# ritobanrc/firework

Measured on AMD Instinct MI355X. Metric: Mrays/s, cornell_box 512x512 @1024spp (scene resident in HBM; whole frame incl. tile gather), higher is better.
Workload: dtype f32; 1 GPU; C2_cornell_box 512x512 @1024spp; use_bvh=False, tiles=16x16, dealt diagonally over ranks, collective=none, rng=counter (pcg4d) keyed by (seed,pixel,sample,dimension), seed=0

## Files before the change

firework_amd/csrc/fw_device.h:

```cpp
#pragma once
#include <hip/hip_runtime.h>
#include <stdint.h>

#ifndef FW_AB
#define FW_AB 0
#endif

namespace fw {

constexpr int OBJ_Q = 6;

enum : uint32_t {
    OF_ROTATED = 1u << 0,
    OF_FLIP = 1u << 1,
    OF_RECT_FLIP = 1u << 2,
    OF_MESH_NORMALS = 1u << 3,
    OF_MESH_ATTR = 1u << 4,
    OF_CULL0 = 1u << 6,
    OF_GATE = 1u << 5,
};

constexpr uint32_t REF_LEAF = 0x80000000u, REF_DONE = 0xffffffffu;
constexpr int WIDE_NONE = 0, WIDE_F32 = 1, WIDE_Q8 = 2;
constexpr uint32_t WIDE_F32_DW = 28, WIDE_Q8_DW = 12;
// ... 22 lines not shown
    const uint32_t *tri_rank;
    const uint32_t *obj_rank;
    const float4 *obj_gate;
    const float4 *obj_cull;
    const float4 *obj_leaf;
    const float4 *mat;
    const float4 *tex;
    const uint8_t *images;
    uint32_t n_objects;
    uint32_t tlas_root;
    uint32_t has_medium;
    uint32_t has_perlin;
    uint32_t has_mesh;
    uint32_t prim_bits;
    const float4 *ref_tlas;
    const float4 *ref_blas;
    const uint32_t *obj_ref_blas;
    const uint32_t *wblas;
    const uint32_t *wtlas;
    const uint32_t *obj_wroot;
    uint32_t wtlas_root;
    float soft_shear;
    uint32_t n_hoisted;
    uint32_t hoisted[4];
    DEnv env;
};

constexpr uint32_t EX_TRACE_ZERO = 8u;
struct DExact {
    uint32_t mode;
    uint32_t n_frames;
    float frames[4][9];
    float shear;
    float far_c[3], far_r;
    float box_lo[3], box_hi[3];
    uint32_t *slots[2];
    uint32_t *count;
    uint32_t cap;
};

struct DCamera {
    float position[3], horizontal[3], vertical[3], lower_left[3], u[3], v[3];
    float lens_radius;
};

struct DFrame {
    uint32_t width, height;
    uint32_t n_pixels;
    const uint32_t *pixel_ids;
    uint32_t scatter_out;
    uint32_t seed32;
    uint32_t sample0;
    uint32_t spp_batch;
    float inv_width;
    float inv_n_pixels;
    uint32_t q_n_waves, q_shift;
    uint32_t skip_zero_deposits;
    uint32_t dep_pixel_major;
    uint32_t *dep_bits;
    uint32_t hit4;
    uint32_t pinhole0;
    float cam_pos[3];
    uint32_t chain_bits;
    float4 *atten;
    uint32_t atten_stride;
    DExact ex;
};

struct DPaths {
    float4 *ray_a;
    float2 *ray_b;
    float4 *state;
};

struct DQueue {
    uint32_t n_waves, cap;
    uint32_t cpw_shift;
    uint32_t *wcount;
};

struct DPark {
    float4 *ray_a; float2 *ray_b; float4 *meta;
    uint32_t stride;
    uint32_t *pcount;
    uint32_t *ptotal;
};

constexpr uint32_t B_RAY = 24, B_RAY_PINHOLE0 = 16, B_STATE = 16, B_STATE_CHAIN = 8, B_HIT = 8, B_HIT4 = 4, B_DEPOSIT = 16, B_PARK = 40, B_ACCUM = 16, B_ATTEN = 16;

constexpr uint32_t MISS = 0xffffffffu;
constexpr int MAX_SEGMENTS = 11;
constexpr int COUNT_STRIDE = 16;

struct DLights {
    const uint32_t *obj;
    uint32_t n;
    float p_pick;
};
struct DShadow {
    DLights lt;
    float4 *ray_a; float2 *ray_b;
    float4 *state;
    uint32_t *obj;
    uint32_t *wcount;
    const float *pb_in;
    float *pb_out;
    float4 *nee;
};
constexpr uint32_t SHADOW_SEED = 0x6e1a7c35u;

struct DEnvDist {
    const float *cdf_m, *cdf_c, *dens;
    float p_env;
    uint32_t w, h;
};

struct LaunchCfg {
    hipStream_t stream;
    DQueue q;
    int blocks_other;
    int tlas_depth, blas_depth;
    uint32_t n_mat, n_tex;
    bool lds_tables;
    bool has_mesh;
    bool simple_but_meshes;
    bool simple_set;
    int n_cus;
    uint32_t blas_pair_nodes, tlas_pair_nodes, max_tris, n_tris;
    bool no_lds_tris;
    uint32_t n_defer;
    bool lds_trees;
    int shade_mode;
    int exact_form;
    uint32_t ref_tlas_nodes, ref_blas_nodes, ref_tlas_depth, ref_blas_depth;
    int wblas_fmt, wtlas_fmt;
    uint32_t wblas_nodes, wtlas_nodes, wblas_depth, wtlas_depth;
    uint32_t debug_wide_levels;
    bool tlas_refill;
};
constexpr size_t LDS_TREE_LIMIT = 160 * 1024;
constexpr size_t LDS_TABLE_LIMIT = 16 * 1024;

void launch_raygen(const LaunchCfg &, const DCamera &, const DFrame &, DPaths out, float4 *sample_rad, uint32_t n_paths);
void launch_raygen_views(const LaunchCfg &, const DCamera *cams, uint32_t n_view, const DFrame &, DPaths out, float4 *sample_rad, uint32_t n_paths);
void launch_resolve_views(const LaunchCfg &, const DFrame &, uint32_t n_view, const float4 *accum, uint32_t total_spp, float gamma,
                          uint8_t *rgb8, float *gamma_rgb, float *linear_rgb);
void launch_view_ids(hipStream_t stream, const uint32_t *src, uint32_t n_view, uint32_t n, uint32_t *out);
void launch_raygen_rays(const LaunchCfg &, const float *rays, bool per_sample, uint32_t *err, const DFrame &, DPaths out, uint32_t n_paths);
void launch_ray_keys(hipStream_t stream, uint32_t base, uint32_t n, uint32_t *out);
void launch_extend(const LaunchCfg &, const DScene &, const DFrame &, DPaths in, float2 *hits, int segment, bool use_bvh, DPark park);
void launch_extend_exact(const LaunchCfg &, const DScene &, const DFrame &, const DPaths &in, float2 *hits, int segment, bool use_bvh);
void launch_shade(const LaunchCfg &, const DScene &, const DFrame &, DPaths in, DPaths out, const float2 *hits,
                  float4 *sample_rad, int segment);
void launch_shade_ls(const LaunchCfg &, const DScene &, const DFrame &, DPaths in, DPaths out, const float2 *hits,
                     float4 *sample_rad, int segment, const DShadow &);
void launch_shadow_resolve(const LaunchCfg &, const DScene &, const DShadow &, const float2 *hits, int segment);
void launch_shade_env(const LaunchCfg &, const DScene &, const DFrame &, DPaths in, DPaths out, const float2 *hits,
                      float4 *sample_rad, int segment, const DShadow &, const DEnvDist &);
void launch_shadow_resolve_env(const LaunchCfg &, const DScene &, const DShadow &, const float2 *hits, int segment);
int build_env_dist(hipStream_t stream, const DEnv &env, float *cdf_m, float *cdf_c, float *dens, float *p_out, double *scratch, double *total);
void launch_env_sample_test(hipStream_t stream, const DEnv &env, const DEnvDist &ed, uint32_t n, uint32_t seed32, float *out);
void launch_bounce(const LaunchCfg &, const DScene &, const DFrame &, DPaths in, DPaths out, float4 *sample_rad, int segment,
                   bool use_bvh);
void launch_queue_totals(const LaunchCfg &, uint32_t *totals, const uint32_t *ptotal);
void launch_trace_load(const LaunchCfg &, const DFrame &, const float *rays, DPaths out, uint32_t n, uint32_t key0, uint32_t *ids, uint32_t *slot_of);
void launch_trace_store(const LaunchCfg &, const DScene &, const DFrame &, const DPaths &in, const float2 *hits, const uint32_t *slot_of, uint32_t n,
                        float4 *out);
void launch_camera_rays(hipStream_t stream, int n_cus, const DCamera &, const DFrame &, uint32_t n, float *out);
void launch_aov_accumulate(hipStream_t stream, int n_cus, const DScene &, const DFrame &, const DPaths &in, const float2 *hits, const uint32_t *slot_of,
                           uint32_t n, uint32_t first, float4 *sum);
void launch_aov_finish(hipStream_t stream, int n_cus, uint32_t n, uint32_t spp, float4 *aov);
void launch_denoise(hipStream_t stream, int n_cus, uint32_t W, uint32_t H, uint32_t L, const float *color, const float4 *aov, const float4 *moments,
                    float4 *guide, float4 *ev0, float4 *ev1, float gamma, uint8_t *rgb8, float *gamma_rgb, float *linear_rgb);
void launch_scatter_tiles(hipStream_t stream, const uint32_t *ids, uint32_t n, const uint8_t *in8, const float *ing, const float *inl,
                          uint8_t *out8, float *outg, float *outl);
void launch_tile_order(hipStream_t stream, uint32_t width, uint32_t height, uint32_t *ids);
void launch_upload(hipStream_t stream, const void *pinned_src, void *dst, size_t bytes);
#if FW_AB
uint32_t take_error_word();
#endif
void preload_kernels();
void launch_count_deposits(const LaunchCfg &, const uint32_t *dep_bits, uint32_t *total);
void launch_selftest_arith(hipStream_t stream, uint32_t n, uint32_t seed, int mode, unsigned long long *out);
void launch_selftest_libm(hipStream_t stream, int fn, uint32_t n, const float *x, const float *y, float *out);
void launch_accumulate(const LaunchCfg &, const DFrame &, const float4 *sample_rad, float4 *accum);
void launch_resolve(const LaunchCfg &, const DFrame &, const float4 *accum, uint32_t total_spp, float gamma,
                    uint8_t *rgb8, float *gamma_rgb, float *linear_rgb);
constexpr uint32_t ADAPTIVE_MAX_BLOCKS = 1024;
void launch_accumulate_adaptive(const LaunchCfg &, const DFrame &, const float4 *sample_rad, float4 *accum, float4 *moments);
uint32_t adaptive_select_blocks(uint32_t n);
void launch_adaptive_select(hipStream_t stream, const uint32_t *ids, uint32_t n, const float4 *accum, float4 *moments, uint32_t n_samples, bool may_continue,
                            float tol, unsigned long long *mask, uint32_t *block_counts, uint32_t *out_ids, uint32_t *count);
void launch_resolve_adaptive(hipStream_t stream, int n_cus, uint32_t n, const float4 *accum, const float4 *moments, float gamma,
                             uint8_t *rgb8, float *gamma_rgb, float *linear_rgb);

constexpr int BLOCK = 256;

}
```

firework_amd/csrc/fw_kernels.hip:

```cpp
#include "../../include/firework_hip.h"
#include "fw_device.h"
#include "fw_libm.h"
#include <atomic>
#include <type_traits>

namespace fw {

struct V3 { float x, y, z; };
__device__ __forceinline__ V3 mk(float x, float y, float z) { return V3{x, y, z}; }
__device__ __forceinline__ V3 operator+(V3 a, V3 b) { return {a.x + b.x, a.y + b.y, a.z + b.z}; }
__device__ __forceinline__ V3 operator-(V3 a, V3 b) { return {a.x - b.x, a.y - b.y, a.z - b.z}; }
__device__ __forceinline__ V3 operator-(V3 a) { return {-a.x, -a.y, -a.z}; }
__device__ __forceinline__ V3 operator*(V3 a, V3 b) { return {a.x * b.x, a.y * b.y, a.z * b.z}; }
__device__ __forceinline__ V3 operator*(float s, V3 a) { return {s * a.x, s * a.y, s * a.z}; }
__device__ __forceinline__ V3 operator*(V3 a, float s) { return {a.x * s, a.y * s, a.z * s}; }
__device__ __forceinline__ float dot(V3 a, V3 b) { return fmaf(a.x, b.x, fmaf(a.y, b.y, a.z * b.z)); }
__device__ __forceinline__ V3 cross(V3 a, V3 b) {
    return {fmaf(a.y, b.z, -a.z * b.y), fmaf(a.z, b.x, -a.x * b.z), fmaf(a.x, b.y, -a.y * b.x)};
}
__device__ __forceinline__ float mag_sq(V3 a) { return dot(a, a); }
__device__ __forceinline__ float comp(V3 a, int i) { return i == 0 ? a.x : (i == 1 ? a.y : a.z); }
__device__ __forceinline__ V3 ld3(const float *p) { return {p[0], p[1], p[2]}; }

#ifndef FW_FAST_DIV
// ... 1189 lines not shown
                if (n_walk == 0u || (n_walk < n_busy && n_walk * WALK_NUM <= n_busy * WALK_DEN)) break;
                if (walking) {
                    TS_TICK(0);
                    cur = pair_step(sc.tlas, cur, wo, inv, relaxed(inv), box_tmin(TMIN, soft), TMAX, soft ? NO_CULL : cull_bound(have ? best_t : TMAX), st);
                }
            }
            if (busy && (cur & REF_LEAF) && cur != REF_DONE) {
                const uint32_t item = cur & NODE_MASK;
                cur = st.sp ? st.pop() : REF_DONE;
                Obj o = load_obj_for_hit(sc.obj, item);
                if (PARK && obj_kind(o) == 5u && !deferred) {
                    if (obj_gate_ok(sc, item, wo, inv)) { deferred = true; deferred_obj = item; }
                } else {
                    TS_TICK(2);
                    RngKey key{0, 0, 0};
                    if (sc.has_medium) key = key_of(f, path_id);
                    float t; uint32_t prim;
                    if (hit_object(sc, o, item, Ray{wo, wd}, TMIN, TMAX, blas_stack, key, segment, t, prim)) {
                        if ((!have || t < best_t || (t == best_t && sc.obj_rank[item] > sc.obj_rank[best_obj])) && obj_gate_ok(sc, item, wo, inv)) { have = true; best_t = t; best_obj = item; best_prim = prim; }
                    }
                }
            }

            const bool done = slot != IDLE && cur == REF_DONE;
            if (done && !deferred) qst(&hits[base + slot], pack_hit(best_t, best_obj, best_prim, sc.prim_bits));
            if (PARK) {
                const unsigned long long pmask = __ballot(done && deferred);
                if (pmask) {
                    const uint32_t prank = __builtin_amdgcn_mbcnt_hi((uint32_t)(pmask >> 32), __builtin_amdgcn_mbcnt_lo((uint32_t)pmask, 0u));
                    if (done && deferred) {
                        const uint32_t e = w * park.stride + park_n + prank;
                        qst(&park.ray_a[e], make_float4(wo.x, wo.y, wo.z, wd.x));
                        qst(&park.ray_b[e], make_float2(wd.y, wd.z));
                        qst(&park.meta[e], make_float4(__uint_as_float(base + slot), __uint_as_float(deferred_obj), best_t, pack_hit(best_t, best_obj, best_prim, sc.prim_bits).y));
                    }
                    park_n += (uint32_t)__popcll(pmask);
                }
            }
            if (done) slot = IDLE;
        }
        if (PARK && lane == 0) park.pcount[w] = park_n;
        TS_END();
        return;
    }

    float4 ra_n = make_float4(0, 0, 0, 0); float2 rb_n = make_float2(0, 0);
    if (lane < n) { ra_n = qld(&in.ray_a[base + lane]); rb_n = load_ray_b(in, base + lane, f, segment); }
    for (uint32_t c0 = 0; c0 < n; c0 += 64u) {
        const uint32_t j = c0 + lane;
        const uint32_t i = base + j;
        float4 ra = ra_n; float2 rb = rb_n;
        if (j + 64u < n) { ra_n = qld(&in.ray_a[i + 64u]); rb_n = load_ray_b(in, i + 64u, f, segment); }
        const bool active = j < n;
        bool deferred = false; uint32_t deferred_obj = 0;
        float best_t = TMAX; uint32_t best_obj = MISS, best_prim = 0;
        if (active) {
            Ray r = make_ray(ra, rb, f, segment);
            RngKey key{0, 0, 0};
            if (sc.has_medium) key = key_of(f, __float_as_uint(load_home(in, i, f, segment)));
            if (!skip_ray(f.ex, r))
                closest_hit<USE_BVH, USE_BVH, MESH, MEDIUM, SIMPLE>(sc, r, key, segment, my_stack, blas_stack, best_t, best_obj, best_prim, deferred, deferred_obj,
                                              USE_BVH && sc.has_mesh && soft_ray(f.ex, r.d, sc.soft_shear));
            if (!USE_BVH && f.hit4) reinterpret_cast<uint32_t *>(hits)[i] = __float_as_uint(pack_hit(best_t, best_obj, best_prim, sc.prim_bits).y);
            else if (!deferred) qst(&hits[i], pack_hit(best_t, best_obj, best_prim, sc.prim_bits));
        }
        if (USE_BVH && sc.has_mesh) {
            unsigned long long mask = __ballot(deferred);
            if (mask) {
                uint32_t rank = __builtin_amdgcn_mbcnt_hi((uint32_t)(mask >> 32), __builtin_amdgcn_mbcnt_lo((uint32_t)mask, 0u));
                if (deferred) {
                    uint32_t e = list_n + rank;
                    e_slot[e] = i; e_obj[e] = deferred_obj; e_t[e] = best_t; e_bobj[e] = best_obj; e_bprim[e] = best_prim;
                }
                list_n += (uint32_t)__popcll(mask);
                if (list_n >= BLAS_RUN_MIN) blas_run();
            }
        }
    }
    if (USE_BVH && list_n) blas_run();
    TS_END();
}
#ifndef FW_DEFER_WAVES
#define FW_DEFER_WAVES 7
#endif
#ifndef FW_DEFER_LDS_PAD
#define FW_DEFER_LDS_PAD 0
#endif
#ifndef FW_SCAN_WAVES
#define FW_SCAN_WAVES 6
#endif
#ifndef FW_SCAN_WAVES_PLAIN
#define FW_SCAN_WAVES_PLAIN 7
#endif
template <bool PARK, bool PLAIN = false, bool SIMPLE = false>
__global__ __launch_bounds__(WB) __attribute__((amdgpu_waves_per_eu(PLAIN ? FW_SCAN_WAVES_PLAIN : FW_SCAN_WAVES, 8))) void k_extend_scan(DScene sc, DFrame f, DPaths in, float2 *__restrict__ hits, DQueue q, int segment,
                                                    int tlas_levels, float4 *__restrict__ park_a, float2 *__restrict__ park_b, float4 *__restrict__ park_m,
                                                    uint32_t *__restrict__ park_count, uint32_t park_stride) {
    const uint32_t w = wave_index(), lane = threadIdx.x & 63u;
    if (w >= q.n_waves) return;
    const uint32_t n = q.wcount[(size_t)segment * q.n_waves + w];
    const uint32_t base = w * q.cap;
    uint32_t *blas_stack = lds_stack + threadIdx.x + (size_t)tlas_levels * WB;
    const float TMIN = 0.001f, TMAX = 2e9f;
    uint32_t park_n = 0;
    float4 ra_n = make_float4(0, 0, 0, 0); float2 rb_n = make_float2(0, 0);
    if (lane < n) { ra_n = qld(&in.ray_a[base + lane]); rb_n = load_ray_b(in, base + lane, f, segment); }
    for (uint32_t c0 = 0; c0 < n; c0 += 64u) {
        const uint32_t j = c0 + lane, i = base + j;
        const float4 ra = ra_n; const float2 rb = rb_n;
        if (j + 64u < n) { ra_n = qld(&in.ray_a[i + 64u]); rb_n = load_ray_b(in, i + 64u, f, segment); }
        const bool active = j < n;
        bool deferred = false, have = false; uint32_t deferred_obj = 0, best_obj = MISS, best_prim = 0; float best_t = TMAX;
        Ray r{mk(0, 0, 0), mk(0, 0, 1)};
        if (active) {
            r = make_ray(ra, rb, f, segment);
            RngKey key{0, 0, 0};
            if (sc.has_medium) key = key_of(f, __float_as_uint(load_home(in, i, f, segment)));
            const V3 inv = mk(fdiv(1.f, r.d.x), fdiv(1.f, r.d.y), fdiv(1.f, r.d.z));
            const bool soft = sc.has_mesh && soft_ray(f.ex, r.d, sc.soft_shear);
            const uint32_t n_obj = skip_ray(f.ex, r) ? 0u : sc.n_objects;
            for (uint32_t k = 0; k < n_obj; k++) {
                const float4 lo = sc.obj_leaf[2 * (size_t)k], hi = sc.obj_leaf[2 * (size_t)k + 1];
                float entry;
                if (!hit_aabb_entry(lo, hi, r.o, inv, relaxed(inv), box_tmin(TMIN, soft), TMAX, entry) || entry > (soft ? NO_CULL : cull_bound(have ? best_t : TMAX))) continue;
                Obj o = load_obj(sc.obj, k);
                if (PARK && obj_kind(o) == 5u) {
                    if (obj_gate_ok(sc, k, r.o, inv)) { deferred = true; deferred_obj |= 1u << k; }
                    continue;
                }
                float t; uint32_t prim;
                if (PLAIN ? hit_object<false, 0, false, SIMPLE>(sc, o, k, r, TMIN, TMAX, nullptr, key, segment, t, prim) : hit_object(sc, o, k, r, TMIN, TMAX, blas_stack, key, segment, t, prim)) {
                    if ((!have || t < best_t || (t == best_t && sc.obj_rank[k] > sc.obj_rank[best_obj])) && obj_gate_ok(sc, k, r.o, inv)) { have = true; best_t = t; best_obj = k; best_prim = prim; }
                }
            }
            if (!deferred) qst(&hits[i], pack_hit(best_t, best_obj, best_prim, sc.prim_bits));
        }
        if (PARK) {
            const unsigned long long pmask = __ballot(deferred);
            if (pmask) {
                const uint32_t prank = __builtin_amdgcn_mbcnt_hi((uint32_t)(pmask >> 32), __builtin_amdgcn_mbcnt_lo((uint32_t)pmask, 0u));
                if (deferred) {
                    const uint32_t e = w * park_stride + park_n + prank;
                    qst(&park_a[e], make_float4(r.o.x, r.o.y, r.o.z, r.d.x));
                    qst(&park_b[e], make_float2(r.d.y, r.d.z));
                    qst(&park_m[e], make_float4(__uint_as_float(i), __uint_as_float(PARK_MASK | deferred_obj), best_t, pack_hit(best_t, best_obj, best_prim, sc.prim_bits).y));
                }
                park_n += (uint32_t)__popcll(pmask);
            }
        }
    }
    if (PARK && lane == 0) park_count[w] = park_n;
}

constexpr uint32_t DEFER_FIELDS = 9;
extern __shared__ uint32_t lds_defer[];
template <bool SIMPLE>
__global__ __launch_bounds__(WB) __attribute__((amdgpu_waves_per_eu(FW_DEFER_WAVES, 8)))
void k_extend_linear_defer(DScene sc, DFrame f, DPaths in, float2 *__restrict__ hits, DQueue q, int segment, uint32_t n_def) {
    const uint32_t w = wave_index(), lane = threadIdx.x & 63u;
    if (w >= q.n_waves) return;
    const uint32_t n = q.wcount[(size_t)segment * q.n_waves + w], base = w * q.cap;
    const float TMIN = 0.001f, TMAX = 2e9f;
    const uint32_t n_first = sc.n_objects - n_def;
    uint32_t *const L0 = lds_defer, *const L1 = lds_defer + DEFER_FIELDS * 64u;
    uint32_t cnt0 = 0, cnt1 = 0;
    const RngKey nokey{0, 0, 0};
    auto write_final = [&](uint32_t slot, float t, uint32_t code) {
        if (f.hit4) reinterpret_cast<uint32_t *>(hits)[slot] = code; else qst(&hits[slot], make_float2(t, __uint_as_float(code)));
    };
    auto put = [&](uint32_t *L, uint32_t e, uint32_t sb, float t, uint32_t code, const Ray &r) {
        L[e] = sb; L[64u + e] = __float_as_uint(t); L[128u + e] = code;
        L[192u + e] = __float_as_uint(r.o.x); L[256u + e] = __float_as_uint(r.o.y); L[320u + e] = __float_as_uint(r.o.z);
        L[384u + e] = __float_as_uint(r.d.x); L[448u + e] = __float_as_uint(r.d.y); L[512u + e] = __float_as_uint(r.d.z);
    };
    auto get = [&](const uint32_t *L, uint32_t e, uint32_t &sb, float &t, uint32_t &code, Ray &r) {
        sb = L[e]; t = __uint_as_float(L[64u + e]); code = L[128u + e];
        r.o = mk(__uint_as_float(L[192u + e]), __uint_as_float(L[256u + e]), __uint_as_float(L[320u + e]));
        r.d = mk(__uint_as_float(L[384u + e]), __uint_as_float(L[448u + e]), __uint_as_float(L[512u + e]));
    };
    auto test = [&](uint32_t d, const Ray &r, float &t, uint32_t &code) {
        const uint32_t k = n_first + d;
        const Obj o = load_obj(sc.obj, k);
        float tt; uint32_t prim;
        if (hit_rect3d(o.q3, o.q4, to_object_space(o, r), TMIN, t, tt, prim)) { t = tt; code = (k << sc.prim_bits) | prim; }
    };
    auto append = [&](uint32_t *L, uint32_t &cnt, bool want, uint32_t sb, float t, uint32_t code, const Ray &r) {
        const unsigned long long m = __ballot(want);
        if (!m) return;
        const uint32_t rank = __builtin_amdgcn_mbcnt_hi((uint32_t)(m >> 32), __builtin_amdgcn_mbcnt_lo((uint32_t)m, 0u));
        if (want) put(L, cnt + rank, sb, t, code, r);
        cnt += (uint32_t)__popcll(m);
    };
    auto make_room = [&](uint32_t need0, uint32_t need1) {
        const bool r0 = cnt0 != 0u && cnt0 + need0 > 64u;
        const uint32_t pass_on = r0 ? (uint32_t)__popcll(__ballot(lane < cnt0 && (L0[lane] >> 31) != 0u)) : 0u;
#pragma nounroll
        for (int phase = 0; phase < 2; phase++) {
            const bool r1 = cnt1 != 0u && (phase == 0 ? cnt1 + pass_on > 64u : cnt1 + need1 > 64u);
            if (r1) {
                uint32_t sb = 0, code = MISS; float t = TMAX; Ray r{mk(0, 0, 0), mk(0, 0, 1)};
                if (lane < cnt1) { get(L1, lane, sb, t, code, r); test(1, r, t, code); write_final(sb, t, code); }
                cnt1 = 0;
            }
            if (phase == 0 && r0) {
                uint32_t sb = 0, code = MISS; float t = TMAX; Ray r{mk(0, 0, 0), mk(0, 0, 1)};
                const bool on = lane < cnt0;
                if (on) { get(L0, lane, sb, t, code, r); test(0, r, t, code); }
                cnt0 = 0;
                const bool more = on && (sb >> 31) != 0u;
                const uint32_t slot = sb & 0x7fffffffu;
                if (on && !more) write_final(slot, t, code);
                append(L1, cnt1, more, slot, t, code, r);
            }
        }
    };
    float4 ra_n = make_float4(0, 0, 0, 0); float2 rb_n = make_float2(0, 0);
    if (lane < n) { ra_n = qld(&in.ray_a[base + lane]); rb_n = load_ray_b(in, base + lane, f, segment); }
    for (uint32_t c0 = 0; c0 < n; c0 += 64u) {
        const uint32_t j = c0 + lane, i = base + j;
        const float4 ra = ra_n; const float2 rb = rb_n;
        if (j + 64u < n) { ra_n = qld(&in.ray_a[i + 64u]); rb_n = load_ray_b(in, i + 64u, f, segment); }
        const bool active = j < n;
        float best_t = TMAX; uint32_t best_obj = MISS, best_prim = 0;
        bool may0 = false, may1 = false;
        const Ray r = make_ray(ra, rb, f, segment);
        if (active) {
            const float4 *op = sc.obj;
            const Rcp rcx = make_rcp(r.d.x), rcy = make_rcp(r.d.y), rcz = make_rcp(r.d.z);
            for (uint32_t k = 0; k < n_first; k++, op += OBJ_Q) {
                const Obj o = load_obj(op, 0);
                float t; uint32_t prim = 0; bool h;
                const uint32_t kind = obj_kind(o);
                if (kind >= 1u && kind <= 3u && !(obj_flags(o) & OF_ROTATED) && o.q4.y == 0.f) {
                    const Ray ro{r.o - mk(o.q0.w, o.q1.w, o.q2.w), r.d};
                    if (kind == 1u) h = hit_rect_rcp<0>(o.q3.x, o.q3.y, o.q3.z, o.q3.w, o.q4.x, ro, rcz, TMIN, best_t, t);
                    else if (kind == 2u) h = hit_rect_rcp<1>(o.q3.x, o.q3.y, o.q3.z, o.q3.w, o.q4.x, ro, rcy, TMIN, best_t, t);
                    else h = hit_rect_rcp<2>(o.q3.x, o.q3.y, o.q3.z, o.q3.w, o.q4.x, ro, rcx, TMIN, best_t, t);
                } else h = hit_object<false, 0, false, SIMPLE>(sc, o, k, r, TMIN, best_t, nullptr, nokey, segment, t, prim);
                if (h) { best_t = t; best_obj = k; best_prim = prim; }
            }
            const V3 ainv = mk(__builtin_amdgcn_rcpf(r.d.x), __builtin_amdgcn_rcpf(r.d.y), __builtin_amdgcn_rcpf(r.d.z));
            const float eps = 1e-4f * (fabsf(r.o.x) + fabsf(r.o.y) + fabsf(r.o.z));
            for (uint32_t d = 0; d < n_def; d++) {
                const uint32_t k = n_first + d;
                const float4 lo = sc.obj_cull[2 * (size_t)k], hi = sc.obj_cull[2 * (size_t)k + 1];
                const float m = eps + 1e-4f * (fmaxf(fmaxf(fabsf(lo.x), fabsf(lo.y)), fabsf(lo.z)) + fmaxf(fmaxf(fabsf(hi.x), fabsf(hi.y)), fabsf(hi.z))) + 1e-6f;
                float t0 = (lo.x - m - r.o.x) * ainv.x, t1 = (hi.x + m - r.o.x) * ainv.x;
                float tn = fminf(t0, t1), tf = fmaxf(t0, t1);
                t0 = (lo.y - m - r.o.y) * ainv.y; t1 = (hi.y + m - r.o.y) * ainv.y;
                tn = fmaxf(tn, fminf(t0, t1)); tf = fminf(tf, fmaxf(t0, t1));
                t0 = (lo.z - m - r.o.z) * ainv.z; t1 = (hi.z + m - r.o.z) * ainv.z;
                tn = fmaxf(tn, fminf(t0, t1)); tf = fminf(tf, fmaxf(t0, t1));
                const bool maybe = !(tf < tn * (1.f - 1e-4f) - 1e-4f) && !(tf < 0.f) && !(tn * (1.f - 1e-4f) - 1e-4f > best_t);
                if (d == 0) may0 = maybe; else may1 = maybe;
            }
        }
        const uint32_t code = best_obj == MISS ? MISS : ((best_obj << sc.prim_bits) | best_prim);
        const bool c1 = may1 && !may0;
        make_room((uint32_t)__popcll(__ballot(may0)), (uint32_t)__popcll(__ballot(c1)));
        if (active && !may0 && !may1) write_final(i, best_t, code);
        append(L0, cnt0, may0, i | (may1 ? 0x80000000u : 0u), best_t, code, r);
        append(L1, cnt1, c1, i, best_t, code, r);
    }
    make_room(65u, 65u);
}

__global__ __launch_bounds__(WB) __attribute__((amdgpu_waves_per_eu(7, 8)))
void k_extend_linear(DScene sc, DFrame f, DPaths in, float2 *__restrict__ hits, DQueue q, int segment, int tlas_levels, int stack_levels) {
    extend_body<false, false, false>(sc, f, in, hits, q, segment, tlas_levels, stack_levels, DPark{});
}
__global__ __launch_bounds__(WB) __attribute__((amdgpu_waves_per_eu(7, 8)))
void k_extend_linear_nomesh(DScene sc, DFrame f, DPaths in, float2 *__restrict__ hits, DQueue q, int segment, int tlas_levels, int stack_levels) {
    extend_body<false, false, false, false>(sc, f, in, hits, q, segment, tlas_levels, stack_levels, DPark{});
}
__global__ __launch_bounds__(WB) __attribute__((amdgpu_waves_per_eu(7, 8)))
void k_extend_linear_plain(DScene sc, DFrame f, DPaths in, float2 *__restrict__ hits, DQueue q, int segment, int tlas_levels, int stack_levels) {
    extend_body<false, false, false, false, false>(sc, f, in, hits, q, segment, tlas_levels, stack_levels, DPark{});
}
template <bool MEDIUM>
__global__ __launch_bounds__(WB) __attribute__((amdgpu_waves_per_eu(7, 8)))
void k_extend_linear_simple(DScene sc, DFrame f, DPaths in, float2 *__restrict__ hits, DQueue q, int segment, int tlas_levels, int stack_levels) {
    extend_body<false, false, false, false, MEDIUM, true>(sc, f, in, hits, q, segment, tlas_levels, stack_levels, DPark{});
}
#if FW_AB
__global__ __launch_bounds__(WB) __attribute__((amdgpu_waves_per_eu(5, 8)))
void k_extend_bvh(DScene sc, DFrame f, DPaths in, float2 *__restrict__ hits, DQueue q, int segment, int tlas_levels, int stack_levels) {
    extend_body<true, false, false>(sc, f, in, hits, q, segment, tlas_levels, stack_levels, DPark{});
}
#endif
__global__ __launch_bounds__(WB) __attribute__((amdgpu_waves_per_eu(FW_TLAS_WAVES, 8)))
void k_extend_tlas(DScene sc, DFrame f, DPaths in, float2 *__restrict__ hits, DQueue q, int segment, int tlas_levels, int stack_levels) {
    extend_body<true, true, false>(sc, f, in, hits, q, segment, tlas_levels, stack_levels, DPark{});
}
__global__ __launch_bounds__(WB) __attribute__((amdgpu_waves_per_eu(FW_TLAS_WAVES, 8)))
void k_extend_tlas_park(DScene sc, DFrame f, DPaths in, float2 *__restrict__ hits, DQueue q, int segment, int tlas_levels, int stack_levels, DPark park) {
    extend_body<true, true, true>(sc, f, in, hits, q, segment, tlas_levels, stack_levels, park);
}

__global__ __launch_bounds__(WB) __attribute__((amdgpu_waves_per_eu(FW_BLAS_WAVES, 8)))
void k_blas(DScene sc, DPark park, float2 *__restrict__ hits, DQueue q) {
    const uint32_t w = wave_index(), lane = threadIdx.x & 63u;
    if (w >= q.n_waves) return;
    TS_BEGIN();
    const uint32_t n = park.pcount[w];
    if (lane == 0 && n) park.ptotal[w] += n;
    const uint32_t base = w * park.stride;
    const float TMIN = 0.001f, TMAX = 2e9f;
    float4 ca = make_float4(0, 0, 0, 0), na = ca, cm = ca, nm = ca; float2 cb = make_float2(0, 0), nb = cb;
    auto fetch = [&](uint32_t j, float4 &a, float2 &b, float4 &m) {
        if (j < n) { a = qld(&park.ray_a[base + j]); b = qld(&park.ray_b[base + j]); m = qld(&park.meta[base + j]); }
    };
    fetch(lane, ca, cb, cm); fetch(64u + lane, na, nb, nm);
    uint32_t cur_base = 0, q_next = 0;
    bool act = false, have = false;
    uint32_t slot = 0, obj = 0, tri_base = 0, bcode = MISS, mtri = 0, cur = REF_DONE;
    float bt = TMAX, mbest = TMAX;
    V3 ro = mk(0, 0, 0), inv = ro;
    bool soft = false;
    TriRay tr{mk(0, 0, 0), 0, 1, 2, 0.f, 0.f, 0.f};
    LdsStack st{lds_stack + threadIdx.x, 0};
    uint32_t more = 0, pidx = 0;
    auto start_walk = [&](uint32_t mesh_obj, float4 ra, float2 rb) {
        obj = mesh_obj;
        Obj o = load_obj(sc.obj, obj);
        Ray r = to_object_space(o, Ray{mk(ra.x, ra.y, ra.z), mk(ra.w, rb.x, rb.y)});
        ro = r.o; inv = mk(fdiv(1.f, r.d.x), fdiv(1.f, r.d.y), fdiv(1.f, r.d.z));
        soft = soft_direction(r.d.x, r.d.y, r.d.z, sc.soft_shear);
        tr = make_triray(r);
        tri_base = o.aux1; cur = o.aux0; st.sp = 0;
        have = false; mbest = TMAX; mtri = 0; act = true;
    };
    for (;;) {
        const unsigned long long idle_mask = __ballot(!act);
        const uint32_t n_idle = (uint32_t)__popcll(idle_mask);
        if (q_next < n) {
            if (n_idle >= BLAS_REFILL_MIN) {
                const uint32_t take = min(n_idle, min(n, cur_base + 64u) - q_next);
                const uint32_t rank = __builtin_amdgcn_mbcnt_hi((uint32_t)(idle_mask >> 32), __builtin_amdgcn_mbcnt_lo((uint32_t)idle_mask, 0u));
                const int sel = (int)((((q_next - cur_base) + rank) & 63u) << 2);
                auto bp = [&](float v) { return __int_as_float(__builtin_amdgcn_ds_bpermute(sel, __float_as_int(v))); };
                const float4 ra = make_float4(bp(ca.x), bp(ca.y), bp(ca.z), bp(ca.w));
                const float2 rb = make_float2(bp(cb.x), bp(cb.y));
                const float4 me = make_float4(bp(cm.x), bp(cm.y), bp(cm.z), bp(cm.w));
                if (!act && rank < take) {
                    slot = __float_as_uint(me.x); more = __float_as_uint(me.y); bt = me.z; bcode = __float_as_uint(me.w);
                    pidx = base + q_next + rank;
                    start_walk(park_next_mesh(more), ra, rb);
                }
                q_next += take;
                if (q_next == cur_base + 64u && q_next < n) { ca = na; cb = nb; cm = nm; cur_base += 64u; fetch(cur_base + 64u + lane, na, nb, nm); }
            }
        } else if (n_idle == 64u) break;

        const uint32_t n_act = (uint32_t)__popcll(__ballot(act));
        for (;;) {
            const bool walking = act && !(cur & REF_LEAF);
            const uint32_t n_walk = (uint32_t)__popcll(__ballot(walking));
            if (n_walk == 0u || (n_walk < n_act && n_walk * BLAS_WALK_NUM <= n_act * BLAS_WALK_DEN)) break;
            if (walking) {
                TS_TICK(4);
                cur = pair_step(sc.blas, cur, ro, inv, relaxed(inv), box_tmin(TMIN, soft), TMAX, soft ? NO_CULL : cull_bound(have ? fminf(mbest, bt) : bt), st);
            }
        }
        if (act && (cur & REF_LEAF)) {
            if (cur != REF_DONE) {
                const uint32_t item = cur & NODE_MASK;
                cur = st.sp ? st.pop() : REF_DONE;
                TS_TICK(6);
                const float4 *tp = sc.tri + 3 * (size_t)(tri_base + item);
                float4 a = tp[0], b = tp[1], c = tp[2];
                float t, b0, b1, b2;
                if (hit_triangle(mk(a.x, a.y, a.z), mk(b.x, b.y, b.z), mk(c.x, c.y, c.z), tr, TMIN, TMAX, t, b0, b1, b2)) {
                    if ((!have || t < mbest || (t == mbest && sc.tri_rank[tri_base + item] > sc.tri_rank[tri_base + mtri])) &&
                        tri_gate_ok(sc, tri_base + item, mk(a.x, a.y, a.z), mk(b.x, b.y, b.z), mk(c.x, c.y, c.z), ro, inv, TMIN, TMAX)) { have = true; mbest = t; mtri = item; }
                }
            }
            if (cur == REF_DONE) {
                const uint32_t bobj = bcode == MISS ? MISS : (bcode >> sc.prim_bits);
                if (have && (bobj == MISS || mbest < bt || (mbest == bt && sc.obj_rank[obj] > sc.obj_rank[bobj]))) { bt = mbest; bcode = (obj << sc.prim_bits) | mtri; }
                if (more) start_walk(park_next_mesh(more), qld(&park.ray_a[pidx]), qld(&park.ray_b[pidx]));
                else { qst(&hits[slot], make_float2(bt, __uint_as_float(bcode))); act = false; }
            }
        }
    }
    TS_END();
}

constexpr int LDS_WAVES = 16;
constexpr uint32_t LDS_UNIT = 512;
__host__ __device__ inline uint32_t lds_unit(uint32_t queue_slots) { const uint32_t u = (queue_slots / 4u) & ~63u; return u < 128u ? 128u : (u > LDS_UNIT ? LDS_UNIT : u); }
template <bool LDS_TRIS>
__global__ __launch_bounds__(LDS_WAVES * 64) void k_blas_lds(DScene sc, DPark park, float2 *__restrict__ hits, DQueue q,
                                                             uint32_t n_nodes, uint32_t n_tris, uint32_t levels) {
    extern __shared__ float4 lds_nodes[];
    const uint32_t lane = threadIdx.x & 63u, wib = threadIdx.x >> 6;
    for (uint32_t k = threadIdx.x; k < n_nodes * 4u; k += LDS_WAVES * 64) lds_nodes[k] = sc.blas[k];
    float4 *lds_tris = lds_nodes + (size_t)n_nodes * 4u;
    if (LDS_TRIS) for (uint32_t k = threadIdx.x; k < n_tris * 3u; k += LDS_WAVES * 64) lds_tris[k] = sc.tri[k];
    uint16_t *stacks = reinterpret_cast<uint16_t *>(lds_tris + (LDS_TRIS ? (size_t)n_tris * 3u : 0u));
    uint32_t *ctr = reinterpret_cast<uint32_t *>(stacks + (size_t)LDS_WAVES * levels * 64u);
    const uint32_t n_k = (q.n_waves + gridDim.x - 1u - blockIdx.x) / gridDim.x;
    uint32_t *lds_cnt = ctr + 4;
    for (uint32_t k = threadIdx.x; k < n_k; k += LDS_WAVES * 64) lds_cnt[k] = park.pcount[blockIdx.x + k * gridDim.x];
    if (threadIdx.x == 0) *ctr = 0u;
    __syncthreads();
    BlockStream bs;
// ... 1141 lines not shown
        if (f.skip_zero_deposits) {
            const uint32_t b = f.dep_pixel_major ? dep_bit_of(f, path_id) : path_id;
            atomicOr(&f.dep_bits[b >> 5], 1u << (b & 31u));
        }
        PH_ADD(6);
    }
    return alive;
}

extern __shared__ float4 lds_tables[];

template <int LDS_TAB, int MODE, bool CHAIN>
#ifndef FW_SHADE_WAVES
#define FW_SHADE_WAVES 5
#endif
#ifndef FW_SHADE_PIPE
#define FW_SHADE_PIPE 0
#endif
#ifndef FW_SHADE_STATIC_STORES
#define FW_SHADE_STATIC_STORES FW_SHADE_PIPE
#endif
__attribute__((amdgpu_waves_per_eu(FW_SHADE_WAVES, 8)))
__global__ __launch_bounds__(WB) void k_shade(DScene sc, DFrame f, DPaths in, DPaths out, const float2 *__restrict__ hits,
                                                 float4 *__restrict__ sample_rad, DQueue q, int segment,
                                                 uint32_t n_mat, uint32_t n_tex) {
    const uint32_t w = wave_index(), lane = threadIdx.x & 63u;
    const float4 *objp = sc.obj, *matp = sc.mat, *texp = sc.tex;
    __shared__ uint16_t shade_list[128];
    if (sc.has_perlin && MODE != 1 && !CHAIN) { stage_perm(); if (!LDS_TAB) __syncthreads(); }
    if (LDS_TAB) {
        const uint32_t no = LDS_TAB == 1 ? sc.n_objects * OBJ_Q : 0u, nm = 2 * n_mat, nt = 2 * n_tex;
        if (LDS_TAB == 1) for (uint32_t k = threadIdx.x; k < no; k += WB) lds_tables[k] = sc.obj[k];
        for (uint32_t k = threadIdx.x; k < nm; k += WB) lds_tables[no + k] = sc.mat[k];
        for (uint32_t k = threadIdx.x; k < nt; k += WB) lds_tables[no + nm + k] = sc.tex[k];
        __syncthreads();
        if (LDS_TAB == 1) objp = lds_tables;
        matp = lds_tables + no; texp = lds_tables + no + nm;
    }
    if (w >= q.n_waves) return;
    const uint32_t n = q.wcount[(size_t)segment * q.n_waves + w];
    const uint32_t base = w * q.cap;
    uint32_t out_n = 0;
    uint32_t list_n = 0;
    PH_DECL;
    auto compact = [&](bool alive, const Ray &nr, V3 nbeta, uint32_t nchain, uint32_t path_id, uint32_t c0 = 0xffffffffu) {
        const unsigned long long mask = __ballot(alive);
        const uint32_t rank = __builtin_amdgcn_mbcnt_hi((uint32_t)(mask >> 32), __builtin_amdgcn_mbcnt_lo((uint32_t)mask, 0u));
#if FW_SHADE_STATIC_STORES
        if (c0 != 0xffffffffu) {
#if FW_SHADE_STATIC_STORES == 2
            const uint32_t dst = base + (alive ? out_n + rank : q.cap - 1u);
#else
            const uint32_t dst = base + (alive ? out_n + rank : min(c0 + 64u + lane, q.cap - 1u));
#endif
            qst(&out.ray_a[dst], make_float4(nr.o.x, nr.o.y, nr.o.z, nr.d.x));
            qst(&out.ray_b[dst], make_float2(nr.d.y, nr.d.z));
            if (CHAIN) qst(&reinterpret_cast<float2 *>(out.state)[dst], make_float2(__uint_as_float(nchain), __uint_as_float(path_id)));
            else qst(&out.state[dst], make_float4(nbeta.x, nbeta.y, nbeta.z, __uint_as_float(path_id)));
        } else
#endif
        if (alive) {
            const uint32_t dst = base + out_n + rank;
            qst(&out.ray_a[dst], make_float4(nr.o.x, nr.o.y, nr.o.z, nr.d.x));
            qst(&out.ray_b[dst], make_float2(nr.d.y, nr.d.z));
            if (CHAIN) qst(&reinterpret_cast<float2 *>(out.state)[dst], make_float2(__uint_as_float(nchain), __uint_as_float(path_id)));
            else qst(&out.state[dst], make_float4(nbeta.x, nbeta.y, nbeta.z, __uint_as_float(path_id)));
        }
        if (f.ex.mode)
            flag_exact(f.ex, alive && needs_exact(f.ex, nr.o.x, nr.o.y, nr.o.z, nr.d.x, nr.d.y, nr.d.z), base + out_n + rank, segment + 1);
        out_n += (uint32_t)__popcll(mask);
    };
    auto load_st = [&](uint32_t idx) { return CHAIN ? load_state_chain(in, idx, segment) : load_state(in, idx, segment); };
    auto load_hit = [&](uint32_t idx) { return f.hit4 ? make_float2(0.f, __uint_as_float(reinterpret_cast<const uint32_t *>(hits)[idx])) : qld(&hits[idx]); };
    auto run_list = [&](uint32_t take) {
        bool alive = false;
        Ray nr{mk(0, 0, 0), mk(0, 0, 0)}; V3 nbeta = mk(0, 0, 0); uint32_t path_id = 0, nchain = 0;
        if (lane < take) {
            const uint32_t i = base + shade_list[list_n - take + lane];
            const float4 ra = qld(&in.ray_a[i]), st = load_st(i); const float2 rb = load_ray_b(in, i, f, segment), hr = load_hit(i);
            path_id = __float_as_uint(st.w);
            alive = shade_path<false, CHAIN>(sc, f, objp, matp, texp, make_ray(ra, rb, f, segment), mk(st.x, st.y, st.z), __float_as_uint(st.x), path_id, hr.x, __float_as_uint(hr.y), segment, sample_rad, nr, nbeta, nchain PH_PASS);
        }
        list_n -= take;
        compact(alive, nr, nbeta, nchain, path_id);
    };
    float4 ra_n = make_float4(0, 0, 0, 0), st_n = ra_n; float2 rb_n = make_float2(0, 0), hr_n = rb_n;
#if FW_SHADE_PIPE
    auto prefetch = [&](uint32_t jn) {
        const uint32_t in_ = base + jn;
        ra_n = qld(&in.ray_a[in_]);
        rb_n = qld(&in.ray_b[short_rays(f, segment) ? base : in_]);
        if (CHAIN) { const float2 v = qld(&reinterpret_cast<const float2 *>(in.state)[segment == 0 ? base : in_]); st_n = make_float4(v.x, 0.f, 0.f, v.y); }
        else st_n = qld(&in.state[segment == 0 ? base : in_]);
        hr_n = load_hit(in_);
    };
    auto fix_implicit = [&](float4 &st_, float2 &rb_, uint32_t slot) {
        if (segment == 0) st_ = CHAIN ? make_float4(0.f, 0.f, 0.f, __uint_as_float(slot)) : make_float4(1.f, 1.f, 1.f, __uint_as_float(slot));
        if (short_rays(f, segment)) rb_ = make_float2(0.f, 0.f);
    };
    if (n) {
        prefetch(min(lane, n - 1u));
        const uint32_t d0 = base + lane;
        qst(&out.ray_a[d0], make_float4(0.f, 0.f, 0.f, 0.f));
        qst(&out.ray_b[d0], make_float2(0.f, 0.f));
        if (CHAIN) qst(&reinterpret_cast<float2 *>(out.state)[d0], make_float2(0.f, 0.f)); else qst(&out.state[d0], make_float4(0.f, 0.f, 0.f, 0.f));
    }
#else
    if (lane < n) { ra_n = qld(&in.ray_a[base + lane]); rb_n = load_ray_b(in, base + lane, f, segment); st_n = load_st(base + lane); hr_n = load_hit(base + lane); }
#endif
    for (uint32_t c0 = 0; c0 < n; c0 += 64u) {
        const uint32_t j = c0 + lane;
        const uint32_t i = base + j;
        float4 ra = ra_n, st = st_n; float2 rb = rb_n, hr = hr_n;
#if FW_SHADE_PIPE
        fix_implicit(st, rb, i);
        const RngKey key_ = key_of(f, __float_as_uint(st.w));
        prefetch(min(j + 64u, n - 1u));
        const RngKey *pre_key = &key_;
#else
        if (j + 64u < n) { ra_n = qld(&in.ray_a[i + 64u]); rb_n = load_ray_b(in, i + 64u, f, segment); st_n = load_st(i + 64u); hr_n = load_hit(i + 64u); }
        const RngKey *pre_key = nullptr;
#endif
        bool alive = false, later = false;
        Ray nr{mk(0, 0, 0), mk(0, 0, 0)}; V3 nbeta = mk(0, 0, 0); uint32_t path_id = 0, nchain = 0;
        if (j < n) {
            PH_T0;
            Ray r = make_ray(ra, rb, f, segment);
            V3 beta = mk(st.x, st.y, st.z);
            path_id = __float_as_uint(st.w);
            const uint32_t hit_code = __float_as_uint(hr.y);
#ifdef FW_ABL_SHADE_COPY
            alive = hit_code != MISS && segment < 10; nr = r; nbeta = beta; nchain = __float_as_uint(st.x) + (pre_key ? pre_key->pixel & 1u : 0u);
#else
            if (MODE == 2 && expensive_shading(sc, objp, matp, hit_code)) later = true;
            else alive = shade_path<MODE != 0, CHAIN>(sc, f, objp, matp, texp, r, beta, __float_as_uint(st.x), path_id, hr.x, hit_code, segment, sample_rad, nr, nbeta, nchain PH_PASS, pre_key);
#endif
            PH_ADD(0);
        }
        { PH_T0; compact(alive, nr, nbeta, nchain, path_id, c0); PH_ADD(7); }
        if (MODE == 2) {
            const unsigned long long lm = __ballot(later);
            if (lm) {
                const uint32_t lr = __builtin_amdgcn_mbcnt_hi((uint32_t)(lm >> 32), __builtin_amdgcn_mbcnt_lo((uint32_t)lm, 0u));
                if (later) shade_list[list_n + lr] = (uint16_t)j;
                list_n += (uint32_t)__popcll(lm);
                if (list_n >= 64u) run_list(64u);
            }
        }
    }
    if (MODE == 2) while (list_n) run_list(min(list_n, 64u));
    if (lane == 0) q.wcount[(size_t)(segment + 1) * q.n_waves + w] = out_n;
    PH_FLUSH(1);
}
template <int LDS_TAB, int MODE>
__attribute__((amdgpu_waves_per_eu(FW_SHADE_WAVES, 8)))
__global__ __launch_bounds__(WB) void k_shade_ls(DScene sc, DFrame f, DPaths in, DPaths out, const float2 *__restrict__ hits,
                                                    float4 *__restrict__ sample_rad, DQueue q, int segment,
                                                    uint32_t n_mat, uint32_t n_tex, DShadow sh) {
    static_assert(MODE == 0 || MODE == 1, "in line only");
    const uint32_t w = wave_index(), lane = threadIdx.x & 63u;
    const float4 *objp = sc.obj, *matp = sc.mat, *texp = sc.tex;
    if (sc.has_perlin && MODE != 1) { stage_perm(); if (!LDS_TAB) __syncthreads(); }
    if (LDS_TAB) {
        const uint32_t no = LDS_TAB == 1 ? sc.n_objects * OBJ_Q : 0u, nm = 2 * n_mat, nt = 2 * n_tex;
        if (LDS_TAB == 1) for (uint32_t k = threadIdx.x; k < no; k += WB) lds_tables[k] = sc.obj[k];
        for (uint32_t k = threadIdx.x; k < nm; k += WB) lds_tables[no + k] = sc.mat[k];
        for (uint32_t k = threadIdx.x; k < nt; k += WB) lds_tables[no + nm + k] = sc.tex[k];
        __syncthreads();
        if (LDS_TAB == 1) objp = lds_tables;
        matp = lds_tables + no; texp = lds_tables + no + nm;
    }
    if (w >= q.n_waves) return;
    const uint32_t n = q.wcount[(size_t)segment * q.n_waves + w];
    const uint32_t base = w * q.cap;
    uint32_t out_n = 0, sh_n = 0;
    PH_DECL;
    float4 ra_n = make_float4(0, 0, 0, 0), st_n = ra_n; float2 rb_n = make_float2(0, 0), hr_n = rb_n; float pb_n = 0.f;
    auto fetch = [&](uint32_t i) {
        ra_n = qld(&in.ray_a[i]); rb_n = load_ray_b(in, i, f, segment); st_n = load_state(in, i, segment); hr_n = qld(&hits[i]);
        pb_n = segment > 0 ? sh.pb_in[i] : 0.f;
    };
    if (lane < n) fetch(base + lane);
    for (uint32_t c0 = 0; c0 < n; c0 += 64u) {
        const uint32_t j = c0 + lane, i = base + j;
        float4 ra = ra_n, st = st_n; float2 rb = rb_n, hr = hr_n;
        LsIO ls{pb_n, 0.f, false, Ray{mk(0, 0, 0), mk(0, 0, 0)}, 0u, mk(0, 0, 0)};
        if (j + 64u < n) fetch(i + 64u);
        bool alive = false;
        Ray nr{mk(0, 0, 0), mk(0, 0, 0)}; V3 nbeta = mk(0, 0, 0); uint32_t path_id = 0, nchain = 0;
        if (j < n) {
            path_id = __float_as_uint(st.w);
            alive = shade_path<MODE != 0, false, true>(sc, f, objp, matp, texp, make_ray(ra, rb, f, segment), mk(st.x, st.y, st.z), 0u, path_id, hr.x,
                                                       __float_as_uint(hr.y), segment, sample_rad, nr, nbeta, nchain PH_PASS, nullptr, &sh, &ls);
        }
        const unsigned long long mask = __ballot(alive);
        const uint32_t rank = __builtin_amdgcn_mbcnt_hi((uint32_t)(mask >> 32), __builtin_amdgcn_mbcnt_lo((uint32_t)mask, 0u));
        if (alive) {
            const uint32_t dst = base + out_n + rank;
            qst(&out.ray_a[dst], make_float4(nr.o.x, nr.o.y, nr.o.z, nr.d.x));
            qst(&out.ray_b[dst], make_float2(nr.d.y, nr.d.z));
            qst(&out.state[dst], make_float4(nbeta.x, nbeta.y, nbeta.z, __uint_as_float(path_id)));
            sh.pb_out[dst] = ls.pb_out;
        }
        if (f.ex.mode) flag_exact(f.ex, alive && needs_exact(f.ex, nr.o.x, nr.o.y, nr.o.z, nr.d.x, nr.d.y, nr.d.z), base + out_n + rank, segment + 1);
        out_n += (uint32_t)__popcll(mask);
        const unsigned long long sm = __ballot(ls.shadow);
        if (sm) {
            const uint32_t sr = __builtin_amdgcn_mbcnt_hi((uint32_t)(sm >> 32), __builtin_amdgcn_mbcnt_lo((uint32_t)sm, 0u));
            if (ls.shadow) {
                const uint32_t d = base + sh_n + sr;
                sh.ray_a[d] = make_float4(ls.sray.o.x, ls.sray.o.y, ls.sray.o.z, ls.sray.d.x);
                sh.ray_b[d] = make_float2(ls.sray.d.y, ls.sray.d.z);
                sh.state[d] = make_float4(ls.pending.x, ls.pending.y, ls.pending.z, __uint_as_float(path_id));
                sh.obj[d] = ls.sobj;
            }
            sh_n += (uint32_t)__popcll(sm);
        }
    }
    if (lane == 0) { q.wcount[(size_t)(segment + 1) * q.n_waves + w] = out_n; sh.wcount[(size_t)(segment + 1) * q.n_waves + w] = sh_n; }
}
template <int LDS_TAB>
__attribute__((amdgpu_waves_per_eu(FW_SHADE_WAVES, 8)))
__global__ __launch_bounds__(WB) void k_shade_env(DScene sc, DFrame f, DPaths in, DPaths out, const float2 *__restrict__ hits,
                                                     float4 *__restrict__ sample_rad, DQueue q, int segment,
                                                     uint32_t n_mat, uint32_t n_tex, DShadow sh, DEnvDist ed) {
    const uint32_t w = wave_index(), lane = threadIdx.x & 63u;
    const float4 *objp = sc.obj, *matp = sc.mat, *texp = sc.tex;
    if (sc.has_perlin) { stage_perm(); if (!LDS_TAB) __syncthreads(); }
    if (LDS_TAB) {
        const uint32_t no = LDS_TAB == 1 ? sc.n_objects * OBJ_Q : 0u, nm = 2 * n_mat, nt = 2 * n_tex;
        if (LDS_TAB == 1) for (uint32_t k = threadIdx.x; k < no; k += WB) lds_tables[k] = sc.obj[k];
        for (uint32_t k = threadIdx.x; k < nm; k += WB) lds_tables[no + k] = sc.mat[k];
        for (uint32_t k = threadIdx.x; k < nt; k += WB) lds_tables[no + nm + k] = sc.tex[k];
        __syncthreads();
        if (LDS_TAB == 1) objp = lds_tables;
        matp = lds_tables + no; texp = lds_tables + no + nm;
    }
    if (w >= q.n_waves) return;
    const uint32_t n = q.wcount[(size_t)segment * q.n_waves + w];
    const uint32_t base = w * q.cap;
    uint32_t out_n = 0, sh_n = 0;
    PH_DECL;
    float4 ra_n = make_float4(0, 0, 0, 0), st_n = ra_n; float2 rb_n = make_float2(0, 0), hr_n = rb_n; float pb_n = 0.f;
    auto fetch = [&](uint32_t i) {
        ra_n = qld(&in.ray_a[i]); rb_n = load_ray_b(in, i, f, segment); st_n = load_state(in, i, segment); hr_n = qld(&hits[i]);
        pb_n = segment > 0 ? sh.pb_in[i] : 0.f;
    };
    if (lane < n) fetch(base + lane);
    for (uint32_t c0 = 0; c0 < n; c0 += 64u) {
        const uint32_t j = c0 + lane, i = base + j;
        float4 ra = ra_n, st = st_n; float2 rb = rb_n, hr = hr_n;
        LsIO ls{pb_n, 0.f, false, Ray{mk(0, 0, 0), mk(0, 0, 0)}, 0u, mk(0, 0, 0)};
        if (j + 64u < n) fetch(i + 64u);
        bool alive = false;
        Ray nr{mk(0, 0, 0), mk(0, 0, 0)}; V3 nbeta = mk(0, 0, 0); uint32_t path_id = 0, nchain = 0;
        if (j < n) {
            path_id = __float_as_uint(st.w);
            alive = shade_path<false, false, true, true>(sc, f, objp, matp, texp, make_ray(ra, rb, f, segment), mk(st.x, st.y, st.z), 0u, path_id, hr.x,
                                                            __float_as_uint(hr.y), segment, sample_rad, nr, nbeta, nchain PH_PASS, nullptr, &sh, &ls, &ed);
        }
        const unsigned long long mask = __ballot(alive);
        const uint32_t rank = __builtin_amdgcn_mbcnt_hi((uint32_t)(mask >> 32), __builtin_amdgcn_mbcnt_lo((uint32_t)mask, 0u));
        if (alive) {
            const uint32_t dst = base + out_n + rank;
            qst(&out.ray_a[dst], make_float4(nr.o.x, nr.o.y, nr.o.z, nr.d.x));
            qst(&out.ray_b[dst], make_float2(nr.d.y, nr.d.z));
            qst(&out.state[dst], make_float4(nbeta.x, nbeta.y, nbeta.z, __uint_as_float(path_id)));
            sh.pb_out[dst] = ls.pb_out;
        }
        if (f.ex.mode) flag_exact(f.ex, alive && needs_exact(f.ex, nr.o.x, nr.o.y, nr.o.z, nr.d.x, nr.d.y, nr.d.z), base + out_n + rank, segment + 1);
        out_n += (uint32_t)__popcll(mask);
        const unsigned long long sm = __ballot(ls.shadow);
        if (sm) {
            const uint32_t sr = __builtin_amdgcn_mbcnt_hi((uint32_t)(sm >> 32), __builtin_amdgcn_mbcnt_lo((uint32_t)sm, 0u));
            if (ls.shadow) {
                const uint32_t d = base + sh_n + sr;
                sh.ray_a[d] = make_float4(ls.sray.o.x, ls.sray.o.y, ls.sray.o.z, ls.sray.d.x);
                sh.ray_b[d] = make_float2(ls.sray.d.y, ls.sray.d.z);
                sh.state[d] = make_float4(ls.pending.x, ls.pending.y, ls.pending.z, __uint_as_float(path_id));
                sh.obj[d] = ls.sobj;
            }
            sh_n += (uint32_t)__popcll(sm);
        }
    }
    if (lane == 0) { q.wcount[(size_t)(segment + 1) * q.n_waves + w] = out_n; sh.wcount[(size_t)(segment + 1) * q.n_waves + w] = sh_n; }
}
__global__ __launch_bounds__(WB) void k_shadow_resolve(DShadow sh, const float2 *__restrict__ hits, DQueue q, int segment, uint32_t prim_bits) {
    const uint32_t w = wave_index(), lane = threadIdx.x & 63u;
    if (w >= q.n_waves) return;
    const uint32_t n = sh.wcount[(size_t)(segment + 1) * q.n_waves + w], base = w * q.cap;
    for (uint32_t j = lane; j < n; j += 64u) {
        const uint32_t i = base + j, code = __float_as_uint(hits[i].y);
        if (code == MISS || (code >> prim_bits) != sh.obj[i]) continue;
        const float4 p = sh.state[i];
        float4 &e = sh.nee[__float_as_uint(p.w)];
        e = make_float4(e.x + p.x, e.y + p.y, e.z + p.z, 0.f);
    }
}
__global__ __launch_bounds__(WB) void k_shadow_resolve_env(DShadow sh, const float2 *__restrict__ hits, DQueue q, int segment, uint32_t prim_bits) {
    const uint32_t w = wave_index(), lane = threadIdx.x & 63u;
    if (w >= q.n_waves) return;
    const uint32_t n = sh.wcount[(size_t)(segment + 1) * q.n_waves + w], base = w * q.cap;
    for (uint32_t j = lane; j < n; j += 64u) {
        const uint32_t i = base + j, code = __float_as_uint(hits[i].y);
        if ((code == MISS ? MISS : code >> prim_bits) != sh.obj[i]) continue;
        const float4 p = sh.state[i];
// ... 522 lines not shown
void launch_trace_store(const LaunchCfg &c, const DScene &sc, const DFrame &f, const DPaths &in, const float2 *hits, const uint32_t *slot_of, uint32_t n,
                        float4 *out) {
    const uint32_t blocks = (uint32_t)std::max<uint64_t>(1, std::min<uint64_t>(((uint64_t)n + BLOCK - 1) / BLOCK, (uint64_t)c.n_cus * 32u));
    hipLaunchKernelGGL(k_trace_store, dim3(blocks), dim3(BLOCK), 0, c.stream, sc, f, in, hits, slot_of, n, out);
}
void launch_camera_rays(hipStream_t stream, int n_cus, const DCamera &cam, const DFrame &f, uint32_t n, float *out) {
    const uint32_t blocks = (uint32_t)std::max<uint64_t>(1, std::min<uint64_t>(((uint64_t)n + 63u) / 64u, (uint64_t)n_cus * 64u));
    hipLaunchKernelGGL(k_camera_rays, dim3(blocks), dim3(WB), 0, stream, cam, f, n, out);
}

void launch_raygen(const LaunchCfg &c, const DCamera &cam, const DFrame &f, DPaths out, float4 *sample_rad, uint32_t n_paths) {
    hipLaunchKernelGGL(k_raygen, wave_grid(c), dim3(WB), 0, c.stream, cam, f, out, sample_rad, c.q, n_paths);
}
void launch_raygen_views(const LaunchCfg &c, const DCamera *cams, uint32_t n_view, const DFrame &f, DPaths out, float4 *sample_rad, uint32_t n_paths) {
    hipLaunchKernelGGL(k_raygen_views, wave_grid(c), dim3(WB), 0, c.stream, cams, n_view, f, out, sample_rad, c.q, n_paths);
}
void launch_raygen_rays(const LaunchCfg &c, const float *rays, bool per_sample, uint32_t *err, const DFrame &f, DPaths out, uint32_t n_paths) {
    hipLaunchKernelGGL(k_raygen_rays, wave_grid(c), dim3(WB), 0, c.stream, rays, per_sample ? 1u : 0u, err, f, out, c.q, n_paths);
}
void launch_ray_keys(hipStream_t stream, uint32_t base, uint32_t n, uint32_t *out) {
    hipLaunchKernelGGL(k_ray_keys, dim3(std::min<uint32_t>((n + BLOCK - 1) / BLOCK, 4096u)), dim3(BLOCK), 0, stream, base, n, out);
}
void launch_resolve_views(const LaunchCfg &c, const DFrame &f, uint32_t n_view, const float4 *accum, uint32_t total_spp, float gamma,
                          uint8_t *rgb8, float *gamma_rgb, float *linear_rgb) {
    hipLaunchKernelGGL(k_resolve_views, dim3(c.blocks_other), dim3(BLOCK), 0, c.stream, f, n_view, accum, total_spp, gamma, rgb8, gamma_rgb, linear_rgb);
}
void launch_view_ids(hipStream_t stream, const uint32_t *src, uint32_t n_view, uint32_t n, uint32_t *out) {
    hipLaunchKernelGGL(k_view_ids, dim3(std::min<uint32_t>((n + BLOCK - 1) / BLOCK, 4096u)), dim3(BLOCK), 0, stream, src, n_view, n, out);
}
static bool lds_attr_needed(int which) {
    static std::atomic<unsigned char> done[4][64];
    int dev = 0;
    if (hipGetDevice(&dev) != hipSuccess || dev < 0 || dev >= 64) return true;
    return done[which][dev].exchange(1) == 0;
}
static size_t lds_walk_bytes(size_t tree_bytes, uint32_t waves, uint32_t levels, uint32_t n_queues, uint32_t grid) {
    return tree_bytes + (size_t)waves * levels * 64 * 2 + 16 + 4 * (size_t)((n_queues + grid - 1) / grid);
}
void launch_extend(const LaunchCfg &c, const DScene &sc, const DFrame &f, DPaths in, float2 *hits, int segment, bool use_bvh, DPark park) {
    int tl = use_bvh ? c.tlas_depth + 1 : 0;
    int levels = tl + c.blas_depth + 1;
    size_t lds = (size_t)levels * WB * sizeof(uint32_t) + (use_bvh && c.has_mesh ? 5 * DEFER_CAP * sizeof(uint32_t) : 0);
    dim3 eg = wave_grid(c);
    const dim3 sg = eg;
    auto walk_grid = [&](uint32_t waves) { return std::min<uint32_t>((uint32_t)c.n_cus, (c.q.n_waves + waves - 1) / waves); };
    if (use_bvh && c.tlas_refill && c.has_mesh) {
        if (sc.n_objects <= TLAS_SCAN_MAX && !sc.has_medium && c.simple_but_meshes) hipLaunchKernelGGL((k_extend_scan<true, true, true>), eg, dim3(WB), (size_t)levels * WB * sizeof(uint32_t), c.stream, sc, f, in, hits, c.q, segment, tl, park.ray_a, park.ray_b, park.meta, park.pcount, park.stride);
        else if (sc.n_objects <= TLAS_SCAN_MAX && !sc.has_medium) hipLaunchKernelGGL((k_extend_scan<true, true>), eg, dim3(WB), (size_t)levels * WB * sizeof(uint32_t), c.stream, sc, f, in, hits, c.q, segment, tl, park.ray_a, park.ray_b, park.meta, park.pcount, park.stride);
        else if (sc.n_objects <= TLAS_SCAN_MAX) hipLaunchKernelGGL(k_extend_scan<true>, eg, dim3(WB), (size_t)levels * WB * sizeof(uint32_t), c.stream, sc, f, in, hits, c.q, segment, tl, park.ray_a, park.ray_b, park.meta, park.pcount, park.stride);
        else hipLaunchKernelGGL(k_extend_tlas_park, sg, dim3(WB), (size_t)levels * WB * sizeof(uint32_t), c.stream, sc, f, in, hits, c.q, segment, tl, levels, park);
        if (c.lds_trees && c.wblas_fmt != WIDE_NONE && sc.wblas && c.max_tris < 0x7fffu) {
            const uint32_t wl = c.debug_wide_levels ? c.debug_wide_levels : 3u * c.wblas_depth + 2u;
            const size_t tree = (size_t)c.wblas_nodes * (c.wblas_fmt == WIDE_F32 ? WIDE_F32_DW : WIDE_Q8_DW) * 4, tris = (size_t)c.n_tris * 48;
            uint32_t waves = 0; bool lds_tris = false;
            if (!c.no_lds_tris && lds_walk_bytes(tree + tris, 16, wl, c.q.n_waves, walk_grid(16)) <= LDS_TREE_LIMIT) { waves = 16; lds_tris = true; }
            else for (uint32_t w : {16u, 12u, 8u}) if (lds_walk_bytes(tree, w, wl, c.q.n_waves, walk_grid(w)) <= LDS_TREE_LIMIT) { waves = w; break; }
            if (waves) {
                if (lds_attr_needed(2)) {
                    (void)hipFuncSetAttribute(reinterpret_cast<const void *>(k_blas_wide<WIDE_F32, false>), hipFuncAttributeMaxDynamicSharedMemorySize, (int)LDS_TREE_LIMIT);
                    (void)hipFuncSetAttribute(reinterpret_cast<const void *>(k_blas_wide<WIDE_F32, true>), hipFuncAttributeMaxDynamicSharedMemorySize, (int)LDS_TREE_LIMIT);
                    (void)hipFuncSetAttribute(reinterpret_cast<const void *>(k_blas_wide<WIDE_Q8, false>), hipFuncAttributeMaxDynamicSharedMemorySize, (int)LDS_TREE_LIMIT);
                    (void)hipFuncSetAttribute(reinterpret_cast<const void *>(k_blas_wide<WIDE_Q8, true>), hipFuncAttributeMaxDynamicSharedMemorySize, (int)LDS_TREE_LIMIT);
                }
                const dim3 lg(walk_grid(waves));
                const size_t bytes = lds_walk_bytes(tree + (lds_tris ? tris : 0), waves, wl, c.q.n_waves, lg.x);
#define FW_BLAS_WIDE(F, T) hipLaunchKernelGGL((k_blas_wide<F, T>), lg, dim3(waves * 64), bytes, c.stream, sc, park, hits, c.q, c.wblas_nodes, c.n_tris, wl)
                if (c.wblas_fmt == WIDE_F32) { if (lds_tris) FW_BLAS_WIDE(WIDE_F32, true); else FW_BLAS_WIDE(WIDE_F32, false); }
                else { if (lds_tris) FW_BLAS_WIDE(WIDE_Q8, true); else FW_BLAS_WIDE(WIDE_Q8, false); }
#undef FW_BLAS_WIDE
                return;
            }
        }
        const uint32_t bl = (uint32_t)c.blas_depth + 1u;
        const size_t lds_blas = lds_walk_bytes((size_t)c.blas_pair_nodes * 64, LDS_WAVES, bl, c.q.n_waves, walk_grid(LDS_WAVES)), lds_tris = (size_t)c.n_tris * 48;
        if (c.lds_trees && c.blas_pair_nodes > 0 && c.blas_pair_nodes < 32768u && c.max_tris < 32768u && lds_blas <= LDS_TREE_LIMIT) {
            if (lds_attr_needed(0)) {
                (void)hipFuncSetAttribute(reinterpret_cast<const void *>(k_blas_lds<false>), hipFuncAttributeMaxDynamicSharedMemorySize, (int)LDS_TREE_LIMIT);
                (void)hipFuncSetAttribute(reinterpret_cast<const void *>(k_blas_lds<true>), hipFuncAttributeMaxDynamicSharedMemorySize, (int)LDS_TREE_LIMIT);
            }
            const dim3 lg(walk_grid(LDS_WAVES));
            if (lds_blas + lds_tris <= LDS_TREE_LIMIT && !c.no_lds_tris)
                hipLaunchKernelGGL(k_blas_lds<true>, lg, dim3(LDS_WAVES * 64), lds_blas + lds_tris, c.stream, sc, park, hits, c.q, c.blas_pair_nodes, c.n_tris, bl);
            else
                hipLaunchKernelGGL(k_blas_lds<false>, lg, dim3(LDS_WAVES * 64), lds_blas, c.stream, sc, park, hits, c.q, c.blas_pair_nodes, c.n_tris, bl);
        }
        else hipLaunchKernelGGL(k_blas, sg, dim3(WB), (size_t)(c.blas_depth + 1) * WB * sizeof(uint32_t), c.stream, sc, park, hits, c.q);
    }
    else if (use_bvh && c.tlas_refill) {
        if (c.lds_trees && !c.has_mesh && sc.n_objects > TLAS_SCAN_MAX && c.wtlas_fmt == WIDE_F32 && sc.wtlas && sc.n_objects < 0x7fffu) {
            const uint32_t wl = c.debug_wide_levels ? c.debug_wide_levels : 3u * c.wtlas_depth + 2u;
            const size_t tree = (size_t)c.wtlas_nodes * WIDE_F32_DW * 4;
            uint32_t waves = 0;
            for (uint32_t w : {16u, 12u, 8u}) if (lds_walk_bytes(tree, w, wl, c.q.n_waves, walk_grid(w)) <= LDS_TREE_LIMIT) { waves = w; break; }
            if (waves) {
                if (lds_attr_needed(3)) {
                    (void)hipFuncSetAttribute(reinterpret_cast<const void *>(k_extend_tlas_wide<true>), hipFuncAttributeMaxDynamicSharedMemorySize, (int)LDS_TREE_LIMIT);
                    (void)hipFuncSetAttribute(reinterpret_cast<const void *>(k_extend_tlas_wide<false>), hipFuncAttributeMaxDynamicSharedMemorySize, (int)LDS_TREE_LIMIT);
                    (void)hipFuncSetAttribute(reinterpret_cast<const void *>((k_extend_tlas_wide<true, true>)), hipFuncAttributeMaxDynamicSharedMemorySize, (int)LDS_TREE_LIMIT);
                    (void)hipFuncSetAttribute(reinterpret_cast<const void *>((k_extend_tlas_wide<false, true>)), hipFuncAttributeMaxDynamicSharedMemorySize, (int)LDS_TREE_LIMIT);
                }
                const dim3 lg(walk_grid(waves));
                if (!sc.has_medium && c.simple_set) hipLaunchKernelGGL((k_extend_tlas_wide<false, true>), lg, dim3(waves * 64), lds_walk_bytes(tree, waves, wl, c.q.n_waves, lg.x), c.stream, sc, f, in, hits, c.q, segment, c.wtlas_nodes, wl);
                else if (sc.has_medium && c.simple_set) hipLaunchKernelGGL((k_extend_tlas_wide<true, true>), lg, dim3(waves * 64), lds_walk_bytes(tree, waves, wl, c.q.n_waves, lg.x), c.stream, sc, f, in, hits, c.q, segment, c.wtlas_nodes, wl);
                else if (sc.has_medium) hipLaunchKernelGGL(k_extend_tlas_wide<true>, lg, dim3(waves * 64), lds_walk_bytes(tree, waves, wl, c.q.n_waves, lg.x), c.stream, sc, f, in, hits, c.q, segment, c.wtlas_nodes, wl);
                else hipLaunchKernelGGL(k_extend_tlas_wide<false>, lg, dim3(waves * 64), lds_walk_bytes(tree, waves, wl, c.q.n_waves, lg.x), c.stream, sc, f, in, hits, c.q, segment, c.wtlas_nodes, wl);
                return;
            }
        }
        const size_t lds_tlas = lds_walk_bytes((size_t)c.tlas_pair_nodes * 64, LDS_WAVES, (uint32_t)tl, c.q.n_waves, walk_grid(LDS_WAVES));
        if (c.lds_trees && !c.has_mesh && sc.n_objects > TLAS_SCAN_MAX && c.tlas_pair_nodes < 32768u && sc.n_objects < 32768u && lds_tlas <= LDS_TREE_LIMIT) {
            if (lds_attr_needed(1)) (void)hipFuncSetAttribute(reinterpret_cast<const void *>(k_extend_tlas_lds), hipFuncAttributeMaxDynamicSharedMemorySize, (int)LDS_TREE_LIMIT);
            hipLaunchKernelGGL(k_extend_tlas_lds, dim3(walk_grid(LDS_WAVES)), dim3(LDS_WAVES * 64), lds_tlas, c.stream,
                               sc, f, in, hits, c.q, segment, c.tlas_pair_nodes, (uint32_t)tl);
        }
        else if (sc.n_objects <= TLAS_SCAN_MAX) hipLaunchKernelGGL(k_extend_scan<false>, eg, dim3(WB), lds, c.stream, sc, f, in, hits, c.q, segment, tl, (float4 *)nullptr, (float2 *)nullptr, (float4 *)nullptr, (uint32_t *)nullptr, 0u);
        else hipLaunchKernelGGL(k_extend_tlas, sg, dim3(WB), lds, c.stream, sc, f, in, hits, c.q, segment, tl, levels);
    }
#if FW_AB
    else if (use_bvh) hipLaunchKernelGGL(k_extend_bvh, eg, dim3(WB), lds, c.stream, sc, f, in, hits, c.q, segment, tl, levels);
#endif
    else if (c.n_defer && c.simple_set) hipLaunchKernelGGL(k_extend_linear_defer<true>, eg, dim3(WB), (size_t)2 * 64 * DEFER_FIELDS * 4 + FW_DEFER_LDS_PAD, c.stream, sc, f, in, hits, c.q, segment, c.n_defer);
    else if (c.n_defer) hipLaunchKernelGGL(k_extend_linear_defer<false>, eg, dim3(WB), (size_t)2 * 64 * DEFER_FIELDS * 4 + FW_DEFER_LDS_PAD, c.stream, sc, f, in, hits, c.q, segment, c.n_defer);
    else if (c.simple_set && !sc.has_medium) hipLaunchKernelGGL(k_extend_linear_simple<false>, eg, dim3(WB), lds, c.stream, sc, f, in, hits, c.q, segment, tl, levels);
    else if (c.simple_set) hipLaunchKernelGGL(k_extend_linear_simple<true>, eg, dim3(WB), lds, c.stream, sc, f, in, hits, c.q, segment, tl, levels);
    else if (!c.has_mesh && !sc.has_medium) hipLaunchKernelGGL(k_extend_linear_plain, eg, dim3(WB), lds, c.stream, sc, f, in, hits, c.q, segment, tl, levels);
    else if (!c.has_mesh) hipLaunchKernelGGL(k_extend_linear_nomesh, eg, dim3(WB), lds, c.stream, sc, f, in, hits, c.q, segment, tl, levels);
    else hipLaunchKernelGGL(k_extend_linear, eg, dim3(WB), lds, c.stream, sc, f, in, hits, c.q, segment, tl, levels);
}
void launch_extend_exact(const LaunchCfg &c, const DScene &sc, const DFrame &f, const DPaths &in, float2 *hits, int segment, bool use_bvh) {
    const uint32_t tl = std::max<uint32_t>(std::min<uint32_t>(c.ref_tlas_depth + 2u, EXACT_LEVELS), (EXACT_STACK + 2u * EXACT_DEFER) / EXACT_WB);
    const uint32_t bl = std::max<uint32_t>(std::min<uint32_t>(c.ref_blas_depth + 2u, EXACT_LEVELS), EXACT_STACK / EXACT_WB);
    const size_t lds = (size_t)(tl + bl) * EXACT_WB * 4;
    hipLaunchKernelGGL(k_extend_exact, dim3((uint32_t)c.n_cus * 8u), dim3(EXACT_WB), lds, c.stream, sc, f, in, hits, segment, use_bvh ? 1 : 0, tl, c.exact_form);
}
void launch_shade(const LaunchCfg &c, const DScene &sc, const DFrame &f, DPaths in, DPaths out, const float2 *hits,
                  float4 *sample_rad, int segment) {
    size_t tab = ((size_t)sc.n_objects * OBJ_Q + 2 * (size_t)c.n_mat + 2 * (size_t)c.n_tex) * sizeof(float4);
    const size_t tab_mt = (2 * (size_t)c.n_mat + 2 * (size_t)c.n_tex) * sizeof(float4);
    const int lt = (c.lds_tables && tab <= LDS_TABLE_LIMIT) ? 1 : ((c.lds_tables && tab_mt <= LDS_TABLE_LIMIT) ? 2 : 0);
    const size_t lds = lt == 1 ? tab : (lt == 2 ? tab_mt : 0);
    const int mode = c.shade_mode;
#define FW_SHADE(L, M, C) hipLaunchKernelGGL((k_shade<L, M, C>), wave_grid(c), dim3(WB), lds, c.stream, sc, f, in, out, hits, sample_rad, c.q, segment, c.n_mat, c.n_tex)
#define FW_SHADE_C(L, M) do { if (f.chain_bits) FW_SHADE(L, M, true); else FW_SHADE(L, M, false); } while (0)
#if FW_AB
#define FW_SHADE_L(L) do { if (mode == 2) FW_SHADE(L, 2, false); else if (mode == 1) FW_SHADE_C(L, 1); else FW_SHADE_C(L, 0); } while (0)
#else
#define FW_SHADE_L(L) do { if (mode == 1) FW_SHADE_C(L, 1); else FW_SHADE_C(L, 0); } while (0)
#endif
    if (lt == 1) FW_SHADE_L(1); else if (lt == 2) FW_SHADE_L(2); else FW_SHADE_L(0);
#undef FW_SHADE_L
#undef FW_SHADE_C
#undef FW_SHADE
}
void launch_shade_ls(const LaunchCfg &c, const DScene &sc, const DFrame &f, DPaths in, DPaths out, const float2 *hits,
                     float4 *sample_rad, int segment, const DShadow &sh) {
    const size_t tab = ((size_t)sc.n_objects * OBJ_Q + 2 * (size_t)c.n_mat + 2 * (size_t)c.n_tex) * sizeof(float4);
    const size_t tab_mt = (2 * (size_t)c.n_mat + 2 * (size_t)c.n_tex) * sizeof(float4);
    const int lt = (c.lds_tables && tab <= LDS_TABLE_LIMIT) ? 1 : ((c.lds_tables && tab_mt <= LDS_TABLE_LIMIT) ? 2 : 0);
    const size_t lds = lt == 1 ? tab : (lt == 2 ? tab_mt : 0);
#define FW_SHADE_LS(L, M) hipLaunchKernelGGL((k_shade_ls<L, M>), wave_grid(c), dim3(WB), lds, c.stream, sc, f, in, out, hits, sample_rad, c.q, segment, c.n_mat, c.n_tex, sh)
#define FW_SHADE_LS_M(L) do { if (c.shade_mode == 1) FW_SHADE_LS(L, 1); else FW_SHADE_LS(L, 0); } while (0)
    if (lt == 1) FW_SHADE_LS_M(1); else if (lt == 2) FW_SHADE_LS_M(2); else FW_SHADE_LS_M(0);
#undef FW_SHADE_LS_M
#undef FW_SHADE_LS
}
void launch_shadow_resolve(const LaunchCfg &c, const DScene &sc, const DShadow &sh, const float2 *hits, int segment) {
    hipLaunchKernelGGL(k_shadow_resolve, wave_grid(c), dim3(WB), 0, c.stream, sh, hits, c.q, segment, sc.prim_bits);
}
void launch_shade_env(const LaunchCfg &c, const DScene &sc, const DFrame &f, DPaths in, DPaths out, const float2 *hits,
                      float4 *sample_rad, int segment, const DShadow &sh, const DEnvDist &ed) {
    const size_t tab = ((size_t)sc.n_objects * OBJ_Q + 2 * (size_t)c.n_mat + 2 * (size_t)c.n_tex) * sizeof(float4);
    const size_t tab_mt = (2 * (size_t)c.n_mat + 2 * (size_t)c.n_tex) * sizeof(float4);
    const int lt = (c.lds_tables && tab <= LDS_TABLE_LIMIT) ? 1 : ((c.lds_tables && tab_mt <= LDS_TABLE_LIMIT) ? 2 : 0);
    const size_t lds = lt == 1 ? tab : (lt == 2 ? tab_mt : 0);
#define FW_SHADE_ENV(L) hipLaunchKernelGGL((k_shade_env<L>), wave_grid(c), dim3(WB), lds, c.stream, sc, f, in, out, hits, sample_rad, c.q, segment, c.n_mat, c.n_tex, sh, ed)
    if (lt == 1) FW_SHADE_ENV(1); else if (lt == 2) FW_SHADE_ENV(2); else FW_SHADE_ENV(0);
#undef FW_SHADE_ENV
}
void launch_shadow_resolve_env(const LaunchCfg &c, const DScene &sc, const DShadow &sh, const float2 *hits, int segment) {
    hipLaunchKernelGGL(k_shadow_resolve_env, wave_grid(c), dim3(WB), 0, c.stream, sh, hits, c.q, segment, sc.prim_bits);
}
int build_env_dist(hipStream_t stream, const DEnv &env, float *cdf_m, float *cdf_c, float *dens, float *p_out, double *scratch, double *total) {
    const size_t n = (size_t)env.hdr_w * env.hdr_h;
    hipLaunchKernelGGL(k_env_rows, dim3(env.hdr_h), dim3(ENV_BUILD_THREADS), 0, stream, env, cdf_c, scratch);
    hipLaunchKernelGGL(k_env_marg, dim3(1), dim3(ENV_BUILD_THREADS), 0, stream, env.hdr_h, cdf_m, scratch);
    hipLaunchKernelGGL(k_env_dens, dim3((unsigned)((n + ENV_BUILD_THREADS - 1) / ENV_BUILD_THREADS)), dim3(ENV_BUILD_THREADS), 0, stream, env, dens, p_out,
                       (const double *)scratch);
    if (hipGetLastError() != hipSuccess) return FW_ERR_HIP;
    if (hipMemcpyAsync(total, scratch + env.hdr_h, sizeof(double), hipMemcpyDeviceToHost, stream) != hipSuccess) return FW_ERR_HIP;
    if (hipStreamSynchronize(stream) != hipSuccess) return FW_ERR_HIP;
    return FW_OK;
}
void launch_env_sample_test(hipStream_t stream, const DEnv &env, const DEnvDist &ed, uint32_t n, uint32_t seed32, float *out) {
    hipLaunchKernelGGL(k_env_sample_test, dim3((n + WB - 1) / WB), dim3(WB), 0, stream, env, ed, n, seed32, out);
}
#if FW_AB
void launch_bounce(const LaunchCfg &c, const DScene &sc, const DFrame &f, DPaths in, DPaths out, float4 *sample_rad,
                   int segment, bool use_bvh) {
    size_t tab = ((size_t)sc.n_objects * OBJ_Q + 2 * (size_t)c.n_mat + 2 * (size_t)c.n_tex) * sizeof(float4);
    const bool lds_tab = c.lds_tables && tab <= LDS_TABLE_LIMIT;
    if (!lds_tab) tab = 0;
    int tl = use_bvh ? c.tlas_depth + 1 : 0;
    int levels = tl + c.blas_depth + 1;
    size_t lds = tab + (size_t)levels * WB * sizeof(uint32_t);
    uint32_t tq = (uint32_t)(tab / sizeof(float4));
    dim3 g = wave_grid(c);
#define FW_BOUNCE(B, T) hipLaunchKernelGGL((k_bounce<B, T>), g, dim3(WB), lds, c.stream, sc, f, in, out, sample_rad, c.q, segment, tl, c.n_mat, c.n_tex, tq)
    if (use_bvh) { if (lds_tab) FW_BOUNCE(true, true); else FW_BOUNCE(true, false); }
    else { if (lds_tab) FW_BOUNCE(false, true); else FW_BOUNCE(false, false); }
#undef FW_BOUNCE
}
#endif
void preload_kernels() {
    hipFuncAttributes a;
#define FW_TOUCH(k) (void)hipFuncGetAttributes(&a, reinterpret_cast<const void *>(k))
    FW_TOUCH(k_raygen); FW_TOUCH(k_extend_linear); FW_TOUCH(k_extend_linear_nomesh); FW_TOUCH(k_extend_linear_plain); FW_TOUCH(k_extend_linear_defer<true>); FW_TOUCH(k_extend_linear_defer<false>); FW_TOUCH(k_extend_linear_simple<true>); FW_TOUCH(k_extend_linear_simple<false>); FW_TOUCH(k_extend_scan<true>); FW_TOUCH((k_extend_scan<true, true>)); FW_TOUCH((k_extend_scan<true, true, true>)); FW_TOUCH(k_extend_scan<false>);
    FW_TOUCH(k_extend_tlas); FW_TOUCH(k_extend_tlas_park); FW_TOUCH(k_blas); FW_TOUCH(k_blas_lds<true>); FW_TOUCH(k_blas_lds<false>); FW_TOUCH(k_extend_tlas_lds);
    FW_TOUCH((k_blas_wide<WIDE_F32, true>)); FW_TOUCH((k_blas_wide<WIDE_F32, false>)); FW_TOUCH((k_blas_wide<WIDE_Q8, true>)); FW_TOUCH((k_blas_wide<WIDE_Q8, false>));
    FW_TOUCH(k_extend_tlas_wide<true>); FW_TOUCH(k_extend_tlas_wide<false>); FW_TOUCH((k_extend_tlas_wide<true, true>)); FW_TOUCH((k_extend_tlas_wide<false, true>)); FW_TOUCH(k_extend_exact); FW_TOUCH(k_queue_totals); FW_TOUCH(k_count_deposits); FW_TOUCH(k_accumulate); FW_TOUCH(k_tile_order);
    FW_TOUCH(k_resolve); FW_TOUCH(k_raygen_views); FW_TOUCH(k_resolve_views); FW_TOUCH(k_view_ids); FW_TOUCH(k_raygen_rays); FW_TOUCH(k_ray_keys); FW_TOUCH(k_accumulate_adaptive); FW_TOUCH(k_adaptive_select); FW_TOUCH(k_adaptive_compact); FW_TOUCH(k_resolve_adaptive); FW_TOUCH(k_scatter_tiles); FW_TOUCH(k_trace_load); FW_TOUCH(k_trace_store); FW_TOUCH(k_camera_rays);
    FW_TOUCH((k_shade<0, 0, false>)); FW_TOUCH((k_shade<0, 0, true>)); FW_TOUCH((k_shade<0, 1, false>)); FW_TOUCH((k_shade<0, 1, true>));
    FW_TOUCH((k_shade<1, 0, false>)); FW_TOUCH((k_shade<1, 0, true>)); FW_TOUCH((k_shade<1, 1, false>)); FW_TOUCH((k_shade<1, 1, true>));
    FW_TOUCH((k_shade<2, 0, false>)); FW_TOUCH((k_shade<2, 0, true>)); FW_TOUCH((k_shade<2, 1, false>)); FW_TOUCH((k_shade<2, 1, true>));
#undef FW_TOUCH
    (void)hipGetLastError();
}
#if FW_AB
uint32_t take_error_word() {
    uint32_t v = 0, zero = 0;
    if (hipMemcpyFromSymbol(&v, HIP_SYMBOL(g_err_word), 4) != hipSuccess) { (void)hipGetLastError(); return 0; }
    if (v) (void)hipMemcpyToSymbol(HIP_SYMBOL(g_err_word), &zero, 4);
    return v;
}
#endif
#ifdef FW_PHASE_STATS
extern "C" int fw_debug_phase_stats(unsigned long long *out, int n) {
    static unsigned long long zero[2 * 3 * PH_N];
    if (n < 2 * 3 * PH_N) return -1;
    if (hipMemcpyFromSymbol(out, HIP_SYMBOL(g_phase), sizeof zero) != hipSuccess) return -1;
    return hipMemcpyToSymbol(HIP_SYMBOL(g_phase), zero, sizeof zero) == hipSuccess ? 2 * 3 * PH_N : -1;
}
#endif
#ifdef FW_TRAV_STATS
extern "C" int fw_debug_trav_stats(unsigned long long out[8]) {
    unsigned long long zero[8] = {0, 0, 0, 0, 0, 0, 0, 0};
    if (hipMemcpyFromSymbol(out, HIP_SYMBOL(g_trav), sizeof zero) != hipSuccess) return -1;
    return hipMemcpyToSymbol(HIP_SYMBOL(g_trav), zero, sizeof zero) == hipSuccess ? 0 : -1;
}
#endif
void launch_queue_totals(const LaunchCfg &c, uint32_t *totals, const uint32_t *ptotal) {
    hipLaunchKernelGGL(k_queue_totals, dim3(32, MAX_SEGMENTS + 1), dim3(BLOCK), 0, c.stream, c.q, totals, ptotal);
}
void launch_count_deposits(const LaunchCfg &c, const uint32_t *dep_bits, uint32_t *total) {
    hipLaunchKernelGGL(k_count_deposits, dim3(1024), dim3(BLOCK), 0, c.stream, dep_bits, (c.q.n_waves * c.q.cap + 31u) / 32u, total);
}
void launch_accumulate(const LaunchCfg &c, const DFrame &f, const float4 *sample_rad, float4 *accum) {
    uint32_t blocks = (uint32_t)std::max<uint64_t>(1, std::min<uint64_t>(((uint64_t)f.n_pixels + WB - 1) / WB, 65536));
    hipLaunchKernelGGL(k_accumulate, dim3(blocks), dim3(WB), 0, c.stream, f, sample_rad, accum);
}
void launch_resolve(const LaunchCfg &c, const DFrame &f, const float4 *accum, uint32_t total_spp, float gamma,
                    uint8_t *rgb8, float *gamma_rgb, float *linear_rgb) {
    hipLaunchKernelGGL(k_resolve, dim3(c.blocks_other), dim3(BLOCK), 0, c.stream, f, accum, total_spp, gamma, rgb8, gamma_rgb, linear_rgb);
}
void launch_accumulate_adaptive(const LaunchCfg &c, const DFrame &f, const float4 *sample_rad, float4 *accum, float4 *moments) {
    uint32_t blocks = (uint32_t)std::max<uint64_t>(1, std::min<uint64_t>(((uint64_t)f.n_pixels + WB - 1) / WB, 65536));
    hipLaunchKernelGGL(k_accumulate_adaptive, dim3(blocks), dim3(WB), 0, c.stream, f, sample_rad, accum, moments);
}
void launch_resolve_adaptive(hipStream_t stream, int n_cus, uint32_t n, const float4 *accum, const float4 *moments, float gamma,
                             uint8_t *rgb8, float *gamma_rgb, float *linear_rgb) {
    const uint32_t blocks = (uint32_t)std::max<uint64_t>(1, std::min<uint64_t>(((uint64_t)n + BLOCK - 1) / BLOCK, (uint64_t)n_cus * 8));
    hipLaunchKernelGGL(k_resolve_adaptive, dim3(blocks), dim3(BLOCK), 0, stream, n, accum, moments, gamma, rgb8, gamma_rgb, linear_rgb);
}
uint32_t adaptive_select_blocks(uint32_t n) { return (uint32_t)std::max<uint64_t>(1, std::min<uint64_t>(((uint64_t)n + BLOCK - 1) / BLOCK, ADAPTIVE_MAX_BLOCKS)); }
void launch_adaptive_select(hipStream_t stream, const uint32_t *ids, uint32_t n, const float4 *accum, float4 *moments, uint32_t n_samples, bool may_continue,
                            float tol, unsigned long long *mask, uint32_t *block_counts, uint32_t *out_ids, uint32_t *count) {
    const uint32_t blocks = adaptive_select_blocks(n), per_block = (n + blocks - 1) / blocks, per = (per_block + BLOCK - 1) / BLOCK * BLOCK;
    hipLaunchKernelGGL(k_adaptive_select, dim3(blocks), dim3(BLOCK), 0, stream, ids, n, per, accum, moments, n_samples, may_continue ? 1u : 0u, tol, mask, block_counts);
    hipLaunchKernelGGL(k_adaptive_compact, dim3(blocks), dim3(BLOCK), 0, stream, ids, n, per, (const unsigned long long *)mask, (const uint32_t *)block_counts, out_ids, count);
}

__device__ __forceinline__ float clamp01_keep_nan(float x) { return x < 0.f ? 0.f : (x > 1.f ? 1.f : x); }
__device__ __forceinline__ float len_plain(float x, float y, float z) { return fsqrt((x * x + y * y) + z * z); }

__global__ __launch_bounds__(BLOCK) void k_aov_accumulate(DScene sc, DFrame f, DPaths in, const float2 *__restrict__ hits, const uint32_t *__restrict__ slot_of,
                                                          uint32_t n, uint32_t first, float4 *__restrict__ sum) {
    if (sc.has_perlin) stage_perm();
    __syncthreads();
    for (uint32_t i = blockIdx.x * BLOCK + threadIdx.x; i < n; i += gridDim.x * BLOCK) {
        const uint32_t slot = slot_of[i];
        uint32_t code = MISS;
        float t = 0.f;
        if (slot != MISS) {
            if (f.hit4) code = reinterpret_cast<const uint32_t *>(hits)[slot];
            else { const float2 h = hits[slot]; t = h.x; code = __float_as_uint(h.y); }
        }
        float4 *s = sum + 3 * (size_t)(first + i);
        if (code == MISS) {
            V3 c = mk(0.f, 0.f, 0.f);
            if (slot != MISS) {
                const float4 ra = in.ray_a[slot];
                const float2 rb = in.ray_b[slot];
                const float l = len_plain(ra.w, rb.x, rb.y);
                c = env_sample(sc.env, mk(fdiv(ra.w, l), fdiv(rb.x, l), fdiv(rb.y, l)));
            }
            float4 a = s[0];
            a.x += clamp01_keep_nan(c.x); a.y += clamp01_keep_nan(c.y); a.z += clamp01_keep_nan(c.z);
// ... 192 lines not shown
```

firework_amd/csrc/fw_runtime.cpp:

```cpp
#include "../../include/firework_hip.h"
#include "fw_device.h"
#include "fw_build.h"

#include <algorithm>
#include <atomic>
#include <exception>
#include <chrono>
#include <cmath>
#include <cstdio>
#include <cstdlib>
#include <cstring>
#include <limits>
#include <mutex>
#include <new>
#include <string>
#include <thread>
#include <vector>

namespace {

thread_local std::string g_last_error;

int fail(int status, const std::string &msg) { g_last_error = msg; return status; }

struct Options {
    bool bvh_median = false;
    bool no_exact = false, exact_all = false;
    int exact_form = 0;
    bool no_defer = false, no_hit4 = false, no_hoist = false, no_lds_tables = false, no_lds_trees = false, no_lds_tris = false, no_short_rays = false,
         no_tile_order = false, no_zero_skip = false, dep_pixel_major = false, dep_slot_major = false, trace = false, no_chain = false,
         exact_product = false;
    int streams = 0;
    int graph = -1;
    int phase_lock = -1;
    int soft_shear_log2 = 5, exact_shear_log2 = 10; double exact_far_x = 256.0;
    double wide_node_cost = 0.0005;
    int wide = -1;
    int build = -1;
    long waves = 0;
    long long paths_per_batch = 0;
    std::string dump_path;
#if FW_AB
    bool fused = false, tlas_refill_off = false, shade_list = false, no_shade_defer = false, stagger = false;
    int debug_wide_levels = 0;
#endif
};
const char *const OPTION_NAMES[] = {"BVH", "NO_EXACT", "EXACT_ALL", "EXACT_FORM", "NO_DEFER", "NO_HIT4", "NO_HOIST", "NO_LDS_TABLES", "NO_LDS_TREES", "NO_LDS_TRIS",
                                    "NO_SHORT_RAYS", "NO_TILE_ORDER", "NO_ZERO_SKIP", "DEP_PIXEL_MAJOR", "DEP_SLOT_MAJOR", "NO_CHAIN", "EXACT_PRODUCT", "PHASE_LOCK", "GRAPH", "SOFT_SHEAR_LOG2", "EXACT_SHEAR_LOG2", "EXACT_FAR_X", "WIDE_NODE_COST", "TRACE", "STREAMS", "WIDE", "BUILD", "WAVES",
                                    "PATHS_PER_BATCH", "DUMP_PATH",
#if FW_AB
                                    "FUSED", "TLAS_REFILL", "SHADE_LIST", "NO_SHADE_DEFER", "STAGGER", "DEBUG_WIDE_LEVELS",
#endif
                                    nullptr};
bool option_apply(Options &o, const char *name, const char *v) {
    const std::string n = name;
    auto on = [&] { return v != nullptr; };
    auto num = [&] { return v ? atoll(v) : 0ll; };
    if (n == "BVH") o.bvh_median = v && std::strcmp(v, "median") == 0;
    else if (n == "NO_EXACT") o.no_exact = on();
    else if (n == "EXACT_ALL") o.exact_all = num() != 0;
    else if (n == "EXACT_FORM") o.exact_form = v ? (std::strcmp(v, "lane") == 0 ? 1 : (std::strcmp(v, "wave") == 0 ? 2 : 0)) : 0;
    else if (n == "NO_DEFER") o.no_defer = on();
    else if (n == "NO_HIT4") o.no_hit4 = on();
    else if (n == "NO_HOIST") o.no_hoist = on();
    else if (n == "NO_LDS_TABLES") o.no_lds_tables = on();
    else if (n == "NO_LDS_TREES") o.no_lds_trees = on();
    else if (n == "NO_LDS_TRIS") o.no_lds_tris = on();
    else if (n == "NO_SHORT_RAYS") o.no_short_rays = on();
    else if (n == "NO_TILE_ORDER") o.no_tile_order = on();
    else if (n == "NO_ZERO_SKIP") o.no_zero_skip = on();
    else if (n == "DEP_PIXEL_MAJOR") o.dep_pixel_major = on();
    else if (n == "DEP_SLOT_MAJOR") o.dep_slot_major = on();
    else if (n == "NO_CHAIN") o.no_chain = on();
    else if (n == "EXACT_PRODUCT") o.exact_product = v && atoi(v) != 0;
    else if (n == "PHASE_LOCK") o.phase_lock = v ? (atoi(v) != 0 ? 1 : 0) : -1;
    else if (n == "GRAPH") o.graph = v ? (atoi(v) != 0 ? 1 : 0) : -1;
    else if (n == "SOFT_SHEAR_LOG2") o.soft_shear_log2 = v ? (int)num() : 5;
    else if (n == "EXACT_SHEAR_LOG2") o.exact_shear_log2 = v ? (int)num() : 10;
    else if (n == "EXACT_FAR_X") o.exact_far_x = v ? atof(v) : 256.0;
    else if (n == "WIDE_NODE_COST") o.wide_node_cost = v ? atof(v) : 0.0005;
    else if (n == "TRACE") o.trace = on();
    else if (n == "STREAMS") o.streams = (int)std::max<long long>(0, num());
    else if (n == "WIDE") o.wide = !v ? -1 : (std::strcmp(v, "0") == 0 ? 0 : (std::strcmp(v, "f32") == 0 ? 1 : (std::strcmp(v, "q8") == 0 ? 2 : -1)));
    else if (n == "BUILD") {
        if (v && std::strcmp(v, "host") != 0 && std::strcmp(v, "device") != 0) return false;
        o.build = !v ? -1 : (std::strcmp(v, "device") == 0 ? 1 : 0);
    }
    else if (n == "WAVES") o.waves = (long)std::max<long long>(0, num());
    else if (n == "PATHS_PER_BATCH") o.paths_per_batch = std::max<long long>(0, num());
    else if (n == "DUMP_PATH") o.dump_path = v ? v : "";
#if FW_AB
    else if (n == "FUSED") o.fused = num() != 0;
    else if (n == "TLAS_REFILL") o.tlas_refill_off = v && atoi(v) == 0;
    else if (n == "SHADE_LIST") o.shade_list = on();
    else if (n == "NO_SHADE_DEFER") o.no_shade_defer = on();
    else if (n == "STAGGER") o.stagger = on();
    else if (n == "DEBUG_WIDE_LEVELS") o.debug_wide_levels = (int)std::max<long long>(0, num());
#endif
    else return false;
    return true;
}
Options options_from_env() {
    Options o;
    for (int k = 0; OPTION_NAMES[k]; k++) { const std::string e = std::string("FIREWORK_") + OPTION_NAMES[k]; if (const char *v = getenv(e.c_str())) option_apply(o, OPTION_NAMES[k], v); }
    return o;
}
std::mutex g_opt_mu;
Options g_opt = options_from_env();
Options options() { std::lock_guard<std::mutex> g(g_opt_mu); return g_opt; }

#define HIPCHK(expr)                                                                                           \
    do {                                                                                                       \
        hipError_t e_ = (expr);                                                                                \
        if (e_ != hipSuccess) {                                                                                \
            char buf_[512];                                                                                    \
            snprintf(buf_, sizeof buf_, "%s failed: %s (%s:%d)", #expr, hipGetErrorString(e_), __FILE__, __LINE__); \
            return fail(e_ == hipErrorOutOfMemory ? FW_ERR_OOM : FW_ERR_HIP, buf_);                            \
        }                                                                                                      \
    } while (0)

struct V3 { float x, y, z; float operator[](int i) const { return i == 0 ? x : (i == 1 ? y : z); } };
inline V3 operator+(V3 a, V3 b) { return {a.x + b.x, a.y + b.y, a.z + b.z}; }
inline V3 operator-(V3 a, V3 b) { return {a.x - b.x, a.y - b.y, a.z - b.z}; }
inline V3 operator*(float s, V3 a) { return {s * a.x, s * a.y, s * a.z}; }
inline V3 operator*(V3 a, float s) { return {a.x * s, a.y * s, a.z * s}; }
inline float dot(V3 a, V3 b) { return std::fmaf(a.x, b.x, std::fmaf(a.y, b.y, a.z * b.z)); }
inline V3 cross(V3 a, V3 b) { return {std::fmaf(a.y, b.z, -a.z * b.y), std::fmaf(a.z, b.x, -a.x * b.z), std::fmaf(a.x, b.y, -a.y * b.x)}; }
inline V3 normalized(V3 a) { float m = std::sqrt(dot(a, a)); return {a.x / m, a.y / m, a.z / m}; }
inline V3 vmin(V3 a, V3 b) { return {std::fmin(a.x, b.x), std::fmin(a.y, b.y), std::fmin(a.z, b.z)}; }
inline V3 vmax(V3 a, V3 b) { return {std::fmax(a.x, b.x), std::fmax(a.y, b.y), std::fmax(a.z, b.z)}; }
inline V3 tov(const fw_vec3 &v) { return {v.x, v.y, v.z}; }

struct Box { V3 mn, mx; };
inline Box box_union(const Box &a, const Box &b) { return {vmin(a.mn, b.mn), vmax(a.mx, b.mx)}; }
inline V3 box_center(const Box &b) { return 0.5f * b.mn + 0.5f * b.mx; }

inline float bits_f(uint32_t u) { float f; std::memcpy(&f, &u, 4); return f; }

void rotor_rows(const fw_rotor3 &r, float rows[3][3]) {
    float s2 = r.s * r.s, bxy2 = r.xy * r.xy, bxz2 = r.xz * r.xz, byz2 = r.yz * r.yz;
    float s_bxy = r.s * r.xy, s_bxz = r.s * r.xz, s_byz = r.s * r.yz;
    float bxz_byz = r.xz * r.yz, bxy_byz = r.xy * r.yz, bxy_bxz = r.xy * r.xz;
    float c0[3] = {s2 - bxy2 - bxz2 + byz2, -2.f * (bxz_byz + s_bxy), 2.f * (bxy_byz - s_bxz)};
    float c1[3] = {2.f * (s_bxy - bxz_byz), s2 - bxy2 + bxz2 - byz2, -2.f * (s_byz + bxy_bxz)};
    float c2[3] = {2.f * (s_bxz + bxy_byz), 2.f * (s_byz - bxy_bxz), s2 + bxy2 - bxz2 - byz2};
    for (int i = 0; i < 3; i++) { rows[i][0] = c0[i]; rows[i][1] = c1[i]; rows[i][2] = c2[i]; }
}
inline V3 mat_mul(const float rows[3][3], V3 v) {
    return {rows[0][0] * v.x + rows[0][1] * v.y + rows[0][2] * v.z,
            rows[1][0] * v.x + rows[1][1] * v.y + rows[1][2] * v.z,
            rows[2][0] * v.x + rows[2][1] * v.y + rows[2][2] * v.z};
}

struct FlatBvh {
    std::vector<float> nodes;
    uint32_t depth = 0;
    uint32_t count() const { return (uint32_t)(nodes.size() / 8); }
};
struct NanError {};

struct BuildPool {
    std::atomic<int> free_threads;
    explicit BuildPool(int n) : free_threads(n) {}
    int take(int want) {
        int got = 0;
        while (got < want) { int f = free_threads.load(); if (f <= 0) break; if (free_threads.compare_exchange_weak(f, f - 1)) got++; }
        return got;
    }
    void give(int n) { free_threads.fetch_add(n); }
};
inline int host_build_threads() {
    static const int n = [] { const char *e = getenv("FIREWORK_BUILD_THREADS"); int v = e ? atoi(e) : (int)std::thread::hardware_concurrency(); return std::max(1, std::min(v, 64)); }();
    return n;
}
constexpr size_t PAR_SUBTREE_MIN = 4096, PAR_PASS_MIN = 1 << 15;

template <class F> void par_parts(size_t n, int parts, F f) {
    if (parts <= 1) { f((size_t)0, n, 0); return; }
    std::vector<std::thread> th;
    th.reserve((size_t)parts - 1);
    for (int k = 1; k < parts; k++) th.emplace_back([&, k] { f(n * (size_t)k / (size_t)parts, n * (size_t)(k + 1) / (size_t)parts, k); });
    f((size_t)0, n / (size_t)parts, 0);
    for (auto &t : th) t.join();
}
template <class Cmp> void par_stable_sort(uint32_t *b, size_t n, Cmp cmp, BuildPool &pool) {
    int helpers = n >= PAR_PASS_MIN ? pool.take(15) : 0;
    int parts = 1; while (parts * 2 <= helpers + 1) parts *= 2;
    pool.give(helpers - (parts - 1)); helpers = parts - 1;
    if (parts == 1) { std::stable_sort(b, b + n, cmp); return; }
    auto cut = [&](int k) { return n * (size_t)k / (size_t)parts; };
    par_parts(n, parts, [&](size_t lo, size_t hi, int) { std::stable_sort(b + lo, b + hi, cmp); });
    for (int width = 1; width < parts; width *= 2) {
        const int pairs = parts / (2 * width);
        par_parts((size_t)pairs, pairs, [&](size_t lo, size_t hi, int) {
            for (size_t q = lo; q < hi; q++) std::inplace_merge(b + cut((int)q * 2 * width), b + cut((int)q * 2 * width + width), b + cut((int)(q + 1) * 2 * width), cmp);
        });
    }
    pool.give(helpers);
}
inline uint32_t append_tree(FlatBvh &out, const FlatBvh &t) {
    const uint32_t off = out.count();
    out.nodes.insert(out.nodes.end(), t.nodes.begin(), t.nodes.end());
    for (uint32_t i = 0; i < t.count(); i++) {
        float *p = &out.nodes[(size_t)(off + i) * 8];
        uint32_t A; std::memcpy(&A, p + 3, 4);
        if ((A >> 30) == 0u) { A += off; std::memcpy(p + 3, &A, 4); }
    }
    out.depth = std::max(out.depth, t.depth);
    return off;
}
template <class Build> uint32_t build_children(FlatBvh &out, size_t n, size_t half, BuildPool &pool, Build build, Box &lb, Box &rb) {
    if (n >= PAR_SUBTREE_MIN && pool.take(1) == 1) {
        FlatBvh L, R;
        std::exception_ptr ep;
        std::thread th([&] { try { build(L, (size_t)0, half, lb); } catch (...) { ep = std::current_exception(); } });
        try { build(R, half, n - half, rb); } catch (...) { th.join(); pool.give(1); throw; }
        th.join(); pool.give(1);
        if (ep) std::rethrow_exception(ep);
        append_tree(out, L);
        return append_tree(out, R);
    }
    build(out, (size_t)0, half, lb);
    const uint32_t before = out.count();
    build(out, half, n - half, rb);
    return before;
}

struct Centers { std::vector<float> c[3]; };
inline Centers centers_of(const std::vector<Box> &boxes, BuildPool &pool) {
// ... 1503 lines not shown
    if (O.paths_per_batch > 0) return (uint32_t)std::min<long long>(O.paths_per_batch, 0x7fffffffll);
    size_t free_b = 0, total_b = 0;
    uint64_t budget = 1ull << 28;
    if (hipMemGetInfo(&free_b, &total_b) == hipSuccess && free_b + arena_bytes > 0) budget = std::min<uint64_t>(budget, (uint64_t)((free_b + arena_bytes) / 2) / 288u);
    return (uint32_t)std::max<uint64_t>(budget, 1u << 16);
}

void set_walk_cfg(fw::LaunchCfg &cfg, const fw_scene *sc, const Options &O, const fw::DQueue &q, bool use_bvh, bool tlas_refill) {
    cfg.q = q;
    cfg.tlas_depth = (int)sc->tlas_depth; cfg.blas_depth = (int)sc->blas_depth;
    cfg.n_mat = sc->n_mat; cfg.n_tex = sc->n_tex;
    cfg.lds_tables = !O.no_lds_tables;
    cfg.has_mesh = sc->d.has_mesh != 0;
    cfg.simple_set = sc->simple_set; cfg.simple_but_meshes = sc->simple_but_meshes;
#ifdef FW_NO_SIMPLE
    cfg.simple_set = cfg.simple_but_meshes = false;
#endif
    cfg.tlas_refill = tlas_refill;
    cfg.n_cus = sc->n_cus;
    cfg.blas_pair_nodes = sc->blas_pair_nodes; cfg.tlas_pair_nodes = sc->tlas_pair_nodes; cfg.max_tris = sc->max_tris; cfg.n_tris = sc->n_tris;
    cfg.no_lds_tris = O.no_lds_tris;
    cfg.n_defer = (!use_bvh && !O.no_defer) ? sc->n_defer : 0u;
    cfg.lds_trees = !O.no_lds_trees;
    cfg.wblas_fmt = sc->wblas_fmt; cfg.wtlas_fmt = sc->wtlas_fmt; cfg.wblas_nodes = sc->wblas_nodes; cfg.wtlas_nodes = sc->wtlas_nodes;
    cfg.wblas_depth = sc->wblas_depth; cfg.wtlas_depth = sc->wtlas_depth;
    cfg.exact_form = O.exact_form;
    cfg.debug_wide_levels = 0;
#if FW_AB
    cfg.debug_wide_levels = (uint32_t)O.debug_wide_levels;
#endif
    cfg.ref_tlas_nodes = sc->tlas_nodes; cfg.ref_blas_nodes = sc->blas_nodes; cfg.ref_tlas_depth = sc->ref_tlas_depth; cfg.ref_blas_depth = sc->ref_blas_depth;
}

static bool light_sampling(const fw_scene *sc, const fw_render_params *p) {
    return (p->flags & FW_FLAG_LIGHT_SAMPLING) != 0 && sc->n_lights > 0 && sc->ls_vertices;
}
static int build_env_table(const fw::DEnv &env, DevBuf &buf, float *p_out, double &total, hipEvent_t after = nullptr) {
    const size_t n = (size_t)env.hdr_w * env.hdr_h;
    if (int rc = buf.alloc((env.hdr_h + 2 * n) * 4)) return rc;
    DevBuf scratch;
    if (int rc = scratch.alloc((2 * (size_t)env.hdr_h + 1) * 8)) return rc;
    float *base = (float *)buf.p;
    if (after && hipStreamWaitEvent(nullptr, after, 0) != hipSuccess) { scratch.release(); return fail(FW_ERR_HIP, "hipStreamWaitEvent failed"); }
    const int rc = fw::build_env_dist(nullptr, env, base, base + env.hdr_h, base + env.hdr_h + n, p_out, (double *)scratch.p, &total);
    scratch.release();
    return rc ? fail(rc, "environment table build failed") : FW_OK;
}
static fw::DEnvDist env_dist_of(const DevBuf &buf, const fw::DEnv &env, float p_env) {
    const float *base = (const float *)buf.p;
    const size_t n = (size_t)env.hdr_w * env.hdr_h;
    return fw::DEnvDist{base, base + env.hdr_h, base + env.hdr_h + n, p_env, env.hdr_w, env.hdr_h};
}
static int ensure_env_dist(fw_scene *sc, const fw_render_params *p, const Workspace *ws) {
    if (!(p->flags & FW_FLAG_ENV_SAMPLING) || sc->d.env.kind != FW_ENV_HDR || !sc->ls_vertices || sc->env_state != 0) return FW_OK;
    if ((uint64_t)sc->d.env.hdr_w * sc->d.env.hdr_h > 0xffffffffull) { sc->env_state = 2; return FW_OK; }
    const auto t0 = std::chrono::steady_clock::now();
    double total = 0;
    if (int rc = build_env_table(sc->d.env, sc->env_dist, nullptr, total, ws->ev_upload)) return rc;
    sc->env_state = total > 0 ? 1 : 2;
    sc->env_build_ms = std::chrono::duration<double, std::milli>(std::chrono::steady_clock::now() - t0).count();
    if (options().trace) fprintf(stderr, "[firework] environment table: %u x %u texels, total weight %.6g, %.2f ms\n", sc->d.env.hdr_w, sc->d.env.hdr_h, total, sc->env_build_ms);
    return FW_OK;
}
static bool env_sampling(const fw_scene *sc, const fw_render_params *p) {
    return (p->flags & FW_FLAG_ENV_SAMPLING) != 0 && sc->env_state == 1 && sc->ls_vertices;
}
struct BatchBudget { int n_lanes; bool exact_product; uint32_t budget; };
BatchBudget batch_budget(const fw_scene *sc, const fw_render_params *p, const Options &O, size_t arena_bytes) {
    int n_lanes = 2;
    if (O.streams >= 1) n_lanes = std::min(O.streams, (int)Workspace::MAX_LANES);
    n_lanes = (int)std::min<uint32_t>((uint32_t)n_lanes, p->samples);
    const bool exact_product = O.exact_product && (sc->chain_bits == 0 || O.no_chain);
    const bool ls = light_sampling(sc, p) || env_sampling(sc, p);
    const uint32_t budget = p->paths_per_batch ? p->paths_per_batch : default_paths_per_batch(O, arena_bytes) / (uint32_t)n_lanes / (exact_product || ls ? 2u : 1u);
    return BatchBudget{n_lanes, exact_product, budget};
}

struct AdaptiveRound { const uint32_t *ids; uint32_t n; float4 *accum, *moments; };

struct ViewGroup { const fw::DCamera *cams; uint32_t n; };

struct RayInput { const float *rays; uint32_t n; bool per_sample; const uint32_t *keys; uint32_t key_base; bool on_device; };

int render_impl(fw_scene *sc, const fw_render_params *p, uint8_t *rgb8, float *gamma_rgb, float *linear_rgb, fw_stats *stats,
                uint32_t first_sample = 0, float *user_accum = nullptr, const AdaptiveRound *rd = nullptr, const ViewGroup *vg = nullptr,
                const RayInput *ri = nullptr) {
    if (!sc || !p) return fail(FW_ERR_BAD_ARG, "null argument");
    if (p->width == 0 || p->height == 0 || p->samples == 0) return fail(FW_ERR_BAD_ARG, "width, height and samples must be > 0");
    if (!(p->gamma > 0.f)) return fail(FW_ERR_BAD_ARG, "gamma must be > 0");
    if (p->rng_mode != FW_RNG_CTR) return fail(FW_ERR_UNSUPPORTED, "the HIP path implements FW_RNG_CTR only (FW_RNG_LCG is a sequential stream)");
    uint64_t full = (uint64_t)p->width * p->height;
    if (full > 0xffffffffull) return fail(FW_ERR_UNSUPPORTED, "image too large");
    const uint32_t n_view = rd ? rd->n : ri ? ri->n : (p->pixel_ids ? p->n_pixels : (uint32_t)full);
    if (n_view == 0) return fail(FW_ERR_BAD_ARG, "no pixels to render");
    if ((uint64_t)first_sample + p->samples > 0xffffffffull) return fail(FW_ERR_BAD_ARG, "first_sample + samples overflows");
    if (p->pixel_ids) for (uint32_t i = 0; i < n_view; i++) if (p->pixel_ids[i] >= full) return fail(FW_ERR_BAD_ARG, "pixel id out of range");
    if (vg && (uint64_t)n_view * vg->n >= (1ull << 30)) return fail(FW_ERR_UNSUPPORTED, "too many pixels in one view group");
    const uint32_t n_pix = vg ? n_view * vg->n : n_view;
    const auto wall0 = std::chrono::steady_clock::now();
    HIPCHK(hipSetDevice(sc->device));
    hipStream_t stream = (hipStream_t)p->stream;
    Workspace *ws = workspace_for(sc->device);
    if (!ws) return fail(FW_ERR_OOM, "no workspace for this device");
    std::unique_lock<std::mutex> ws_guard(ws->mu, std::defer_lock);
    if (!rd) ws_guard.lock();
    { const int irc = init_device_locked(ws, sc->device); if (irc) return irc; }
    if (int erc = ensure_env_dist(sc, p, ws)) return erc;
    const Options O = options();

    const BatchBudget bb = batch_budget(sc, p, O, ws->arena.bytes);
    int n_lanes = bb.n_lanes;
    const bool ls_lights = light_sampling(sc, p), es = env_sampling(sc, p);
    const bool ls = ls_lights || es;
    const bool exact_product = bb.exact_product && !ls;
    const uint32_t budget = bb.budget;
    uint32_t spp_b = std::max<uint32_t>(1u, budget / n_pix);
    spp_b = std::min(spp_b, (p->samples + (uint32_t)n_lanes - 1) / (uint32_t)n_lanes);
    if (ri) spp_b = std::min(spp_b, (1u << 21) - 1u);
    uint64_t paths64 = (uint64_t)n_pix * spp_b;
    if (paths64 > 0x7fffffffull) return fail(FW_ERR_UNSUPPORTED, "too many paths per batch");
    uint32_t max_paths = (uint32_t)paths64;
    uint32_t n_batches = (p->samples + spp_b - 1) / spp_b;
    spp_b = (p->samples + n_batches - 1) / n_batches;
    max_paths = n_pix * spp_b;
    n_lanes = (int)std::min<uint32_t>((uint32_t)n_lanes, n_batches);
    if (vg && spp_b >= (1u << 21)) return fail(FW_ERR_UNSUPPORTED, "too many samples per batch for a view group");

    fw::DQueue q{};
    const uint32_t unit = (uint32_t)sc->n_cus * 4u * (p->use_bvh ? 20u : 28u);
    const uint64_t chunks = ((uint64_t)max_paths + 63u) / 64u;
    uint32_t want_waves = unit * (uint32_t)std::min<uint64_t>(3u, std::max<uint64_t>(1u, chunks / ((uint64_t)unit * 16u)));
    if (!p->use_bvh && n_lanes > 1) want_waves = chunks >= (1u << 20) ? unit : (uint32_t)sc->n_cus * 48u;
    if (O.waves > 0) want_waves = (uint32_t)O.waves;
    q.n_waves = std::max(4u, std::min(want_waves, (max_paths + 511u) / 512u));
    q.n_waves = (q.n_waves + 7u) & ~7u;
    uint32_t chunks_per_wave = (max_paths + q.n_waves * 64u - 1) / (q.n_waves * 64u);
    q.cpw_shift = 0;
    while ((1u << q.cpw_shift) < chunks_per_wave) q.cpw_shift++;
    q.cap = 64u << q.cpw_shift;
    uint64_t cap64 = (uint64_t)q.cap * q.n_waves;
    if (cap64 > 0x7fffffffull) return fail(FW_ERR_UNSUPPORTED, "too many path slots");
    uint32_t cap = (uint32_t)cap64;

#if FW_AB
    const bool fused_req = O.fused && !ls && !(p->use_bvh && sc->d.has_mesh);
    const bool tlas_refill = !O.tlas_refill_off;
#else
    const bool fused_req = false, tlas_refill = true;
#endif
    const uint32_t exact_mode = fused_req ? 0u : ((sc->ex.mode & 1u) | (p->use_bvh ? (sc->ex.mode & 6u) | (ri ? fw::EX_TRACE_ZERO : 0u)
                                                                                   : ((sc->ex.mode & 4u) && sc->d.has_mesh ? 4u : 0u)));
    const bool park_meshes = p->use_bvh && sc->d.has_mesh != 0 && tlas_refill;
    const bool stage_rays = ri && ri->per_sample && !ri->on_device;
    int rc = FW_OK;
    auto need = [&](DevBuf &b, size_t n) { if (!rc) rc = b.alloc(n); };
    auto layout = [&](uint8_t *arena_base) -> size_t {
        size_t off = 0;
        auto put = [&](void *&dst, size_t n) { dst = arena_base ? arena_base + off : nullptr; off += (n + 255) & ~(size_t)255; };
        for (int l = 0; l < n_lanes; l++) {
            Workspace::Lane &L = ws->lanes[l];
            for (int k = 0; k < 2; k++) { put(L.ray_a[k], (size_t)cap * 16); put(L.ray_b[k], (size_t)cap * 8); put(L.state[k], (size_t)cap * 16); }
            put(L.hits, (size_t)cap * 8);
            put(L.sample_rad, (size_t)cap * 16);
            put(L.dep_bits, ((size_t)cap + 31) / 32 * 4);
            if (exact_product && !fused_req) put(L.atten, (size_t)cap * (fw::MAX_SEGMENTS - 1) * fw::B_ATTEN); else L.atten = nullptr;
            if (exact_mode) put(L.exact_slots, 2 * (size_t)max_paths * 4 + 64);
            put(L.wcount, (size_t)(fw::MAX_SEGMENTS + 1) * q.n_waves * 4);
            if (stage_rays) put(L.rays, (size_t)max_paths * 24); else L.rays = nullptr;
            if (ls) {
                put(L.s_ray_a, (size_t)cap * 16); put(L.s_ray_b, (size_t)cap * 8); put(L.s_state, (size_t)cap * 16); put(L.s_obj, (size_t)cap * 4);
                put(L.s_hits, (size_t)cap * 8); put(L.s_wcount, (size_t)(fw::MAX_SEGMENTS + 1) * q.n_waves * 4);
                put(L.pb[0], (size_t)cap * 4); put(L.pb[1], (size_t)cap * 4); put(L.nee, (size_t)cap * 16);
            }
            if (park_meshes) {
                const size_t pcap = (size_t)(q.cap + 64u) * q.n_waves;
                put(L.park_a, pcap * 16); put(L.park_b, pcap * 8); put(L.park_m, pcap * 16); put(L.pcount, (size_t)q.n_waves * 8);
            }
        }
        return off;
    };
    {
        size_t want = (layout(nullptr) + ((size_t)1 << 30) - 1) & ~(((size_t)1 << 30) - 1);
        if (want > ws->arena.bytes && ws->arena.bytes) want = std::max(want, (ws->arena.bytes + ws->arena.bytes / 4 + ((size_t)1 << 30) - 1) & ~(((size_t)1 << 30) - 1));
        const auto ta = std::chrono::steady_clock::now();
        const bool grow = want > ws->arena.bytes;
        if (!rc && grow) rc = arena_reserve_locked(ws, sc->device, want);
        if ((rd || ri) && grow) { ws->fg.key = 0; ws->fg.seen = 0; }
        if (O.trace && grow) fprintf(stderr, "[firework] render: path arena grown to %.1f GiB in %.2f ms\n", (double)want / (double)(1 << 30),
                                     std::chrono::duration<double, std::milli>(std::chrono::steady_clock::now() - ta).count());
        if (!rc) layout((uint8_t *)ws->arena.p);
    }
    for (int l = 0; l < n_lanes && !rc; l++)
        if (!ws->lanes[l].stream && n_lanes > 1) HIPCHK(hipStreamCreateWithFlags(&ws->lanes[l].stream, hipStreamNonBlocking));
    if (!rd) need(ws->accum, (size_t)n_pix * 16);
    need(ws->totals, (size_t)n_batches * fw::COUNT_STRIDE * 4);
    if (p->pixel_ids) need(ws->pixel_ids, (size_t)n_view * 4);
    const bool own_order = !p->pixel_ids && !user_accum && !rd && !ri && n_view >= 1024 && !O.no_tile_order;
    if (own_order) { const void *before = ws->tile_ids.p; need(ws->tile_ids, (size_t)n_view * 4); if (ws->tile_ids.p != before) ws->tile_w = ws->tile_h = 0; }
    if (vg) { need(ws->view_ids, (size_t)n_pix * 4); need(ws->view_cams, (size_t)vg->n * sizeof(fw::DCamera)); }
    const bool ray_table = ri && (ri->keys || ri->key_base != 0);
    if (ri) {
        need(ws->ray_err, 256);
        if (ray_table) need(ws->ray_keys, (size_t)n_pix * 4);
        if (!ri->per_sample && !ri->on_device) need(ws->ray_fixed, (size_t)n_pix * 24);
        const size_t host_bytes = ri->on_device ? 0 : ri->per_sample ? (size_t)n_lanes * max_paths * 24 : (size_t)n_pix * 24;
        if (!rc && ws->ray_host_bytes < host_bytes) {
            if (ws->ray_host) (void)hipHostFree(ws->ray_host);
            ws->ray_host = nullptr; ws->ray_host_bytes = 0;
            if (hipHostMalloc(&ws->ray_host, host_bytes, hipHostMallocDefault) != hipSuccess) return fail(FW_ERR_OOM, "pinned ray staging allocation failed");
            ws->ray_host_bytes = host_bytes;
        }
    }
    uint8_t *d_rgb8 = rgb8; float *d_gamma = gamma_rgb, *d_linear = linear_rgb;
    if (!p->outputs_on_device) {
        if (rgb8) { need(ws->out_rgb8, (size_t)n_pix * 3); d_rgb8 = (uint8_t *)ws->out_rgb8.p; }
        if (gamma_rgb) { need(ws->out_gamma, (size_t)n_pix * 12); d_gamma = (float *)ws->out_gamma.p; }
        if (linear_rgb) { need(ws->out_linear, (size_t)n_pix * 12); d_linear = (float *)ws->out_linear.p; }
    }
    if (rc) return rc;
    while (ws->events.size() < 3 + 2 * (size_t)n_batches) {
         hipEvent_t e; HIPCHK(hipEventCreateWithFlags(&e, ws->events.size() < 2 ? hipEventDefault : hipEventDisableTiming)); ws->events.push_back(e); }

    if (ws->ev_upload) HIPCHK(hipStreamWaitEvent(stream, ws->ev_upload, 0));
    if (p->pixel_ids) HIPCHK(hipMemcpyAsync(ws->pixel_ids.p, p->pixel_ids, (size_t)n_view * 4, hipMemcpyHostToDevice, stream));
    if (own_order && (ws->tile_w != p->width || ws->tile_h != p->height)) {
        ws->tile_w = ws->tile_h = 0;
        fw::launch_tile_order(stream, p->width, p->height, (uint32_t *)ws->tile_ids.p);
        ws->tile_w = p->width; ws->tile_h = p->height;
    }
    if (vg) {
        fw::launch_view_ids(stream, p->pixel_ids ? (const uint32_t *)ws->pixel_ids.p : (own_order ? (const uint32_t *)ws->tile_ids.p : nullptr), n_view, n_pix,
                            (uint32_t *)ws->view_ids.p);
        HIPCHK(hipMemcpyAsync(ws->view_cams.p, vg->cams, (size_t)vg->n * sizeof(fw::DCamera), hipMemcpyHostToDevice, stream));
    }
    if (ri) {
        HIPCHK(hipMemsetAsync(ws->ray_err.p, 0, 4, stream));
        if (ri->keys) HIPCHK(hipMemcpyAsync(ws->ray_keys.p, ri->keys, (size_t)n_pix * 4, ri->on_device ? hipMemcpyDeviceToDevice : hipMemcpyHostToDevice, stream));
        else if (ray_table) fw::launch_ray_keys(stream, ri->key_base, n_pix, (uint32_t *)ws->ray_keys.p);
        if (!ri->per_sample && !ri->on_device) {
            std::memcpy(ws->ray_host, ri->rays, (size_t)n_pix * 24);
            HIPCHK(hipMemcpyAsync(ws->ray_fixed.p, ws->ray_host, (size_t)n_pix * 24, hipMemcpyHostToDevice, stream));
        }
    }
    if (user_accum)
        HIPCHK(hipMemcpyAsync(ws->accum.p, user_accum, (size_t)n_pix * 16, p->outputs_on_device ? hipMemcpyDeviceToDevice : hipMemcpyHostToDevice, stream));
    else if (!rd) HIPCHK(hipMemsetAsync(ws->accum.p, 0, (size_t)n_pix * 16, stream));
    HIPCHK(hipMemsetAsync(ws->totals.p, 0, (size_t)n_batches * fw::COUNT_STRIDE * 4, stream));

    fw::LaunchCfg cfg{};
    set_walk_cfg(cfg, sc, O, q, p->use_bvh != 0, tlas_refill);
    int max_blocks = sc->n_cus * 8;
    cfg.blocks_other = (int)std::max<uint64_t>(1, std::min<uint64_t>(((uint64_t)n_pix + fw::BLOCK - 1) / fw::BLOCK, (uint64_t)max_blocks));
    cfg.shade_mode = !sc->has_expensive ? 1 : 0;
#if FW_AB
    if (O.no_shade_defer) cfg.shade_mode = 0; else if (sc->has_expensive && O.shade_list && q.cap <= 65536u) cfg.shade_mode = 2;
#endif

    fw::DCamera cam = vg ? vg->cams[0] : ri ? fw::DCamera{} : make_camera(p->camera, p->width, p->height);
    fw::DFrame fr{};
    fr.width = p->width; fr.height = p->height; fr.n_pixels = n_pix; fr.inv_n_pixels = 1.0f / (float)n_pix; fr.inv_width = 1.0f / (float)p->width;
    fr.pixel_ids = rd ? rd->ids : vg ? (const uint32_t *)ws->view_ids.p : ri ? (ray_table ? (const uint32_t *)ws->ray_keys.p : nullptr)
                 : (p->pixel_ids ? (const uint32_t *)ws->pixel_ids.p : (own_order ? (const uint32_t *)ws->tile_ids.p : nullptr));
    fr.scatter_out = own_order ? 1u : 0u;
    fr.seed32 = (uint32_t)p->seed ^ ((uint32_t)(p->seed >> 32) * 0x9E3779B9u);
    fr.q_n_waves = q.n_waves; fr.q_shift = q.cpw_shift;
    fr.cam_pos[0] = cam.position[0]; fr.cam_pos[1] = cam.position[1]; fr.cam_pos[2] = cam.position[2];
    auto not_negative_zero = [](float x) { uint32_t b; std::memcpy(&b, &x, 4); return b != 0x80000000u; };
    bool one_position = true;
    if (vg) for (uint32_t v = 1; v < vg->n; v++) one_position = one_position && vg->cams[v].lens_radius == 0.f && std::memcmp(vg->cams[v].position, cam.position, sizeof cam.position) == 0;
    fr.pinhole0 = (!ri && one_position && cam.lens_radius == 0.f && not_negative_zero(cam.position[0]) && not_negative_zero(cam.position[1]) && not_negative_zero(cam.position[2]) &&
                   !O.no_short_rays) ? 1u : 0u;
    fr.hit4 = (!p->use_bvh && sc->simple_shapes && !exact_mode && !O.no_hit4 && !fused_req && !ls) ? 1u : 0u;
    const fw::DEnv &env = sc->d.env;
    fr.dep_pixel_major = (((n_pix <= 65536u && !O.dep_slot_major) || O.dep_pixel_major) && spp_b < (1u << 21)) ? 1u : 0u;
    fr.ex = sc->ex; fr.ex.mode = exact_mode;
    fr.chain_bits = (O.no_chain || fused_req || cfg.shade_mode == 2 || ls) ? 0u : sc->chain_bits;
    fr.skip_zero_deposits = (env.kind == 0 && env.color[0] == 0.f && env.color[1] == 0.f && env.color[2] == 0.f && !O.no_zero_skip && !ls) ? 1u : 0u;

    const bool timing = (p->flags & FW_FLAG_TIME_KERNELS) != 0;
    const bool count_deposits = (p->flags & FW_FLAG_COUNT_DEPOSITS) != 0 && fr.skip_zero_deposits != 0;
    const size_t per_batch_launches = 1 + 3 * fw::MAX_SEGMENTS + 2 + (ls ? 2 * (fw::MAX_SEGMENTS - 1) : 0);
    std::vector<std::vector<int>> ev_class(n_lanes);
    std::vector<size_t> ev_next(n_lanes, 0);
    if (timing) for (int l = 0; l < n_lanes; l++) {
        size_t want = 1 + per_batch_launches * ((n_batches + n_lanes - 1) / n_lanes);
        auto &ev = ws->lanes[l].events;
        while (ev.size() < want) { hipEvent_t e; HIPCHK(hipEventCreate(&e)); ev.push_back(e); }
    }
    const bool use_bvh = p->use_bvh != 0;
    const bool fused = fused_req;
#if FW_AB
    const bool stagger = n_lanes > 1 && O.stagger;
#else
    const bool stagger = false;
#endif

    const char *dump_file = O.dump_path.c_str();
    const bool dump_one = *dump_file && n_pix == 1 && p->samples == 1 && !fused;
    std::vector<float> dump_rec(dump_one ? (size_t)fw::MAX_SEGMENTS * 16 : 0, 0.f);

    HIPCHK(hipEventRecord(ws->events[0], stream));
    hipStream_t origin = stream;
    bool graph_replayed = false;
    auto fork_lanes = [&]() -> int {
        if (n_lanes > 1) {
            HIPCHK(hipEventRecord(ws->events[2], origin));
            for (int l = 0; l < n_lanes; l++) HIPCHK(hipStreamWaitEvent(ws->lanes[l].stream, ws->events[2], 0));
        }
        return FW_OK;
    };
    struct BatchCtx { fw::DFrame fr; fw::LaunchCfg cfg; fw::DPaths buf[2]; float2 *hits; float4 *srad; fw::DPark park; uint32_t *totals; uint32_t n_paths; int cur; int lane; hipStream_t ls;
                      fw::DShadow sh; fw::DEnvDist ed; };
    constexpr uint64_t PHASE_LOCK_MIN_CHUNKS = 3u << 19;
    const bool phase_lock = n_lanes == 2 && !fused && (O.phase_lock == 1 || (O.phase_lock < 0 && !p->use_bvh && cfg.n_defer > 0 && chunks >= PHASE_LOCK_MIN_CHUNKS));
    std::vector<hipEvent_t> &pe = ws->phase_events;
    while (phase_lock && pe.size() < 2 * (size_t)fw::MAX_SEGMENTS) { hipEvent_t e; HIPCHK(hipEventCreateWithFlags(&e, hipEventDisableTiming)); pe.push_back(e); }
    float4 *const accum = rd ? rd->accum : (float4 *)ws->accum.p;
    auto begin_batch = [&](uint32_t b, BatchCtx &c) -> int {
        const int l = (int)(b % (uint32_t)n_lanes);
        Workspace::Lane &L = ws->lanes[l];
        c.lane = l; c.ls = n_lanes > 1 ? L.stream : origin;
        c.cfg = cfg; c.cfg.stream = c.ls; c.cfg.q.wcount = (uint32_t *)L.wcount;
        c.fr = fr;
        if (timing && ev_next[l] == 0) (void)hipEventRecord(L.events[0], c.ls);
        c.fr.sample0 = first_sample + b * spp_b;
        c.fr.dep_bits = (uint32_t *)L.dep_bits;
        c.fr.atten = (c.fr.chain_bits == 0 && exact_product && !fused_req) ? (float4 *)L.atten : nullptr; c.fr.atten_stride = cap;
        if (c.fr.skip_zero_deposits) HIPCHK(hipMemsetAsync(c.fr.dep_bits, 0, ((size_t)cap + 31) / 32 * 4, c.ls));
        if (exact_mode) {
            c.fr.ex.slots[0] = (uint32_t *)L.exact_slots; c.fr.ex.slots[1] = c.fr.ex.slots[0] + max_paths;
            c.fr.ex.count = c.fr.ex.slots[1] + max_paths; c.fr.ex.cap = max_paths;
            HIPCHK(hipMemsetAsync(c.fr.ex.count, 0, 64, c.ls));
        }
        c.fr.spp_batch = std::min(spp_b, p->samples - b * spp_b);
        c.n_paths = n_pix * c.fr.spp_batch;
        c.totals = (uint32_t *)ws->totals.p + (size_t)b * fw::COUNT_STRIDE;
        for (int k = 0; k < 2; k++) c.buf[k] = {(float4 *)L.ray_a[k], (float2 *)L.ray_b[k], (float4 *)L.state[k]};
        c.hits = (float2 *)L.hits;
        c.srad = (float4 *)L.sample_rad;
        c.park = fw::DPark{(float4 *)L.park_a, (float2 *)L.park_b, (float4 *)L.park_m, q.cap + 64u, (uint32_t *)L.pcount,
                           park_meshes ? (uint32_t *)L.pcount + q.n_waves : nullptr};
        if (park_meshes) HIPCHK(hipMemsetAsync(c.park.ptotal, 0, (size_t)q.n_waves * 4, c.ls));
        c.sh = fw::DShadow{}; c.ed = fw::DEnvDist{};
        if (ls) {
            const float p_env = es ? (ls_lights ? 0.5f : 1.f) : 0.f;
            c.sh.lt = ls_lights ? fw::DLights{(const uint32_t *)sc->lights.p, sc->n_lights, es ? (1.f - p_env) / (float)sc->n_lights : 1.f / (float)sc->n_lights}
                                : fw::DLights{(const uint32_t *)sc->lights.p, 0u, 0.f};
            if (es) c.ed = env_dist_of(sc->env_dist, sc->d.env, p_env);
            c.sh.ray_a = (float4 *)L.s_ray_a; c.sh.ray_b = (float2 *)L.s_ray_b; c.sh.state = (float4 *)L.s_state; c.sh.obj = (uint32_t *)L.s_obj;
            c.sh.wcount = (uint32_t *)L.s_wcount; c.sh.nee = (float4 *)L.nee;
            HIPCHK(hipMemsetAsync(c.sh.nee, 0, (size_t)cap * 16, c.ls));
        }
        c.cur = 0;
        return FW_OK;
    };
    auto timed = [&](BatchCtx &c, int cls, auto &&launch) {
        launch();
        if (timing) { (void)hipEventRecord(ws->lanes[c.lane].events[1 + ev_next[c.lane]], c.ls); ev_next[c.lane]++; ev_class[c.lane].push_back(cls); }
    };
    auto segment = [&](uint32_t b, BatchCtx &c, int seg, int which, int group_size) -> int {
#if FW_AB
        if (fused) { timed(c, 2, [&] { fw::launch_bounce(c.cfg, sc->d, c.fr, c.buf[c.cur], c.buf[c.cur ^ 1], c.srad, seg, use_bvh); }); c.cur ^= 1; return FW_OK; }
#endif
        if (stagger && seg == 0 && b > 0) HIPCHK(hipStreamWaitEvent(c.ls, ws->events[3 + n_batches + b - 1], 0));
        if (phase_lock && group_size == 2) {
            if (which == 1) HIPCHK(hipStreamWaitEvent(c.ls, pe[(size_t)seg], 0));
            else if (seg > 0) HIPCHK(hipStreamWaitEvent(c.ls, pe[(size_t)fw::MAX_SEGMENTS + (size_t)seg - 1], 0));
        }
        timed(c, 1, [&] { fw::launch_extend(c.cfg, sc->d, c.fr, c.buf[c.cur], c.hits, seg, use_bvh, c.park); });
        if (phase_lock && group_size == 2) HIPCHK(hipEventRecord(pe[(size_t)which * fw::MAX_SEGMENTS + (size_t)seg], c.ls));
        if (stagger && seg == 0) HIPCHK(hipEventRecord(ws->events[3 + n_batches + b], c.ls));
        if (exact_mode) timed(c, 1, [&] { fw::launch_extend_exact(c.cfg, sc->d, c.fr, c.buf[c.cur], c.hits, seg, use_bvh); });
        if (dump_one) {
            float *r = &dump_rec[(size_t)seg * 16];
            uint32_t alive = 0;
            HIPCHK(hipMemcpyAsync(&alive, c.cfg.q.wcount + (size_t)seg * q.n_waves, 4, hipMemcpyDeviceToHost, c.ls));
            HIPCHK(hipMemcpyAsync(r, c.buf[c.cur].ray_a, 16, hipMemcpyDeviceToHost, c.ls));
            HIPCHK(hipMemcpyAsync(r + 4, c.buf[c.cur].ray_b, 8, hipMemcpyDeviceToHost, c.ls));
            HIPCHK(hipMemcpyAsync(r + 6, c.buf[c.cur].state, 16, hipMemcpyDeviceToHost, c.ls));
            HIPCHK(hipMemcpyAsync(r + 10, c.hits, 8, hipMemcpyDeviceToHost, c.ls));
            HIPCHK(hipStreamSynchronize(c.ls));
            r[12] = (float)alive;
        }
        if (ls) {
            Workspace::Lane &L = ws->lanes[c.lane];
            c.sh.pb_in = (const float *)L.pb[c.cur]; c.sh.pb_out = (float *)L.pb[c.cur ^ 1];
            if (es) timed(c, 2, [&] { fw::launch_shade_env(c.cfg, sc->d, c.fr, c.buf[c.cur], c.buf[c.cur ^ 1], c.hits, c.srad, seg, c.sh, c.ed); });
            else timed(c, 2, [&] { fw::launch_shade_ls(c.cfg, sc->d, c.fr, c.buf[c.cur], c.buf[c.cur ^ 1], c.hits, c.srad, seg, c.sh); });
            if (seg < fw::MAX_SEGMENTS - 1) {
                fw::LaunchCfg scfg = c.cfg; scfg.q.wcount = c.sh.wcount;
                fw::DFrame sfr = c.fr; sfr.seed32 ^= fw::SHADOW_SEED; sfr.ex.mode = 0;
                const fw::DPaths sp{c.sh.ray_a, c.sh.ray_b, c.sh.state};
                timed(c, 1, [&] { fw::launch_extend(scfg, sc->d, sfr, sp, (float2 *)L.s_hits, seg + 1, use_bvh, c.park); });
                if (es) timed(c, 2, [&] { fw::launch_shadow_resolve_env(scfg, sc->d, c.sh, (const float2 *)L.s_hits, seg); });
                else timed(c, 2, [&] { fw::launch_shadow_resolve(scfg, sc->d, c.sh, (const float2 *)L.s_hits, seg); });
            }
        } else
        timed(c, 2, [&] { fw::launch_shade(c.cfg, sc->d, c.fr, c.buf[c.cur], c.buf[c.cur ^ 1], c.hits, c.srad, seg); });
        c.cur ^= 1;
        return FW_OK;
    };
    auto end_batch = [&](uint32_t b, BatchCtx &c) -> int {
        timed(c, 3, [&] { fw::launch_queue_totals(c.cfg, c.totals, c.park.ptotal); });
        if (count_deposits) fw::launch_count_deposits(c.cfg, c.fr.dep_bits, c.totals + 12);
        if (n_lanes > 1 && b > 0) HIPCHK(hipStreamWaitEvent(c.ls, ws->events[3 + b - 1], 0));
        if (rd) timed(c, 3, [&] { fw::launch_accumulate_adaptive(c.cfg, c.fr, c.srad, accum, rd->moments); });
        else timed(c, 3, [&] { fw::launch_accumulate(c.cfg, c.fr, c.srad, accum); });
        if (n_lanes > 1) HIPCHK(hipEventRecord(ws->events[3 + b], c.ls));
        return FW_OK;
    };
    auto batch_rays = [&](uint32_t b, const BatchCtx &c, const float *&src) -> int {
        if (!ri->per_sample) { src = ri->on_device ? ri->rays : (const float *)ws->ray_fixed.p; return FW_OK; }
        const size_t first = (size_t)b * spp_b * n_pix * 6, bytes = (size_t)c.n_paths * 24;
        if (ri->on_device) { src = ri->rays + first; return FW_OK; }
        HIPCHK(hipStreamSynchronize(c.ls));
        uint8_t *slab = (uint8_t *)ws->ray_host + (size_t)c.lane * max_paths * 24;
        std::memcpy(slab, ri->rays + first, bytes);
        HIPCHK(hipMemcpyAsync(ws->lanes[c.lane].rays, slab, bytes, hipMemcpyHostToDevice, c.ls));
        src = (const float *)ws->lanes[c.lane].rays;
        return FW_OK;
    };
    auto enqueue_frame = [&]() -> int {
    if (int frc = fork_lanes()) return frc;
    for (uint32_t b0 = 0; b0 < n_batches; b0 += (uint32_t)n_lanes) {
        const int group = (int)std::min<uint32_t>((uint32_t)n_lanes, n_batches - b0);
        BatchCtx ctx[Workspace::MAX_LANES];
        for (int g = 0; g < group; g++) {
            if (int brc = begin_batch(b0 + (uint32_t)g, ctx[g])) return brc;
            if (ri) {
                const float *src = nullptr;
                if (int src_rc = batch_rays(b0 + (uint32_t)g, ctx[g], src)) return src_rc;
                timed(ctx[g], 0, [&] { fw::launch_raygen_rays(ctx[g].cfg, src, ri->per_sample, (uint32_t *)ws->ray_err.p, ctx[g].fr, ctx[g].buf[0], ctx[g].n_paths); });
            }
            else if (vg) timed(ctx[g], 0, [&] { fw::launch_raygen_views(ctx[g].cfg, (const fw::DCamera *)ws->view_cams.p, n_view, ctx[g].fr, ctx[g].buf[0], ctx[g].srad, ctx[g].n_paths); });
            else timed(ctx[g], 0, [&] { fw::launch_raygen(ctx[g].cfg, cam, ctx[g].fr, ctx[g].buf[0], ctx[g].srad, ctx[g].n_paths); });
        }
        for (int seg = 0; seg < fw::MAX_SEGMENTS; seg++)
            for (int g = 0; g < group; g++)
                if (int src = segment(b0 + (uint32_t)g, ctx[g], seg, g, group)) return src;
        for (int g = 0; g < group; g++)
            if (int erc = end_batch(b0 + (uint32_t)g, ctx[g])) return erc;
        fr = ctx[group - 1].fr;
    }
    if (n_lanes > 1) HIPCHK(hipStreamWaitEvent(origin, ws->events[3 + n_batches - 1], 0));
    return FW_OK;
    };
    {
        Workspace::FrameGraph &fg = ws->fg;
        constexpr uint64_t GRAPH_MAX_CHUNKS = 1u << 19;
        const bool graph_ok = O.graph != 0 && !rd && !vg && !ri && !ls && !fg.broken && !timing && !dump_one && !phase_lock && !stagger && (O.graph == 1 || chunks < GRAPH_MAX_CHUNKS);
        uint64_t key = 0;
        if (graph_ok) {
            uint64_t h = 1469598103934665603ull;
            auto mix = [&](const void *ptr, size_t n) { const unsigned char *b = (const unsigned char *)ptr; for (size_t i = 0; i < n; i++) { h ^= b[i]; h *= 1099511628211ull; } };
            fw::LaunchCfg kc = cfg; kc.stream = nullptr;
            mix(&cam, sizeof cam); mix(&fr, sizeof fr); mix(&kc, sizeof kc); mix(&sc->d, sizeof sc->d); mix(&q, sizeof q);
            const uint64_t scalars[] = {n_batches, (uint64_t)n_lanes, spp_b, first_sample, p->samples, n_pix, max_paths, cap, exact_mode, (uint64_t)park_meshes, (uint64_t)phase_lock,
                                        (uint64_t)count_deposits, (uint64_t)exact_product, (uint64_t)use_bvh, (uint64_t)fused, (uint64_t)stagger, (uint64_t)(uintptr_t)accum, (uint64_t)(uintptr_t)ws->totals.p,
                                        (uint64_t)(uintptr_t)ws->arena.p, (uint64_t)ws->arena.bytes};
            mix(scalars, sizeof scalars);
            for (int l = 0; l < n_lanes; l++) { const Workspace::Lane &L = ws->lanes[l]; const void *ptrs[] = {L.ray_a[0], L.ray_a[1], L.ray_b[0], L.ray_b[1], L.state[0], L.state[1], L.hits, L.sample_rad, L.wcount, L.park_a, L.park_b, L.park_m, L.pcount, L.dep_bits, L.exact_slots, L.atten}; mix(ptrs, sizeof ptrs); }
            key = h | 1ull;
        }
        bool done = false;
        if (graph_ok && fg.exec && fg.key == key) {
            HIPCHK(hipGraphLaunch(fg.exec, stream));
            fr = fg.fr_after; done = true; graph_replayed = true;
        } else if (graph_ok && fg.seen == key) {
            if (!fg.origin && hipStreamCreateWithFlags(&fg.origin, hipStreamNonBlocking) != hipSuccess) { fg.origin = nullptr; fg.broken = true; }
            if (!fg.broken && hipStreamBeginCapture(fg.origin, hipStreamCaptureModeRelaxed) == hipSuccess) {
                origin = fg.origin;
                if (O.trace) fprintf(stderr, "[firework] GRAPH: capturing (%u batches, %d lanes, phase lock %d)\n", n_batches, n_lanes, (int)phase_lock);
                const int crc = enqueue_frame();
                origin = stream;
                hipGraph_t g = nullptr;
                const hipError_t ee = hipStreamEndCapture(fg.origin, &g);
                if (O.trace) fprintf(stderr, "[firework] GRAPH: capture ended: enqueue %d, end %s\n", crc, hipGetErrorString(ee));
                if (fg.exec) { (void)hipGraphExecDestroy(fg.exec); fg.exec = nullptr; fg.key = 0; }
                if (crc == FW_OK && ee == hipSuccess && g && hipGraphInstantiate(&fg.exec, g, nullptr, nullptr, 0) == hipSuccess) {
                    fg.key = key; fg.fr_after = fr;
                    (void)hipGraphDestroy(g);
                    if (O.trace) fprintf(stderr, "[firework] GRAPH: instantiated\n");
                    HIPCHK(hipGraphLaunch(fg.exec, stream));
                    if (O.trace) fprintf(stderr, "[firework] GRAPH: launched\n");
                    graph_replayed = true;
                    done = true;
                } else {
                    if (g) (void)hipGraphDestroy(g);
                    fg.exec = nullptr; fg.broken = true; (void)hipGetLastError();
                    if (O.trace) fprintf(stderr, "[firework] GRAPH: capture failed (%d, %s): frames run as plain launches from here on\n", crc, hipGetErrorString(ee));
                }
            } else { fg.broken = true; (void)hipGetLastError(); }
        }
        if (graph_ok) fg.seen = key;
        if (!done) { if (int frc = enqueue_frame()) return frc; }
    }
    cfg.stream = stream;
    if (vg) fw::launch_resolve_views(cfg, fr, n_view, (const float4 *)ws->accum.p, p->samples, p->gamma, d_rgb8, d_gamma, d_linear);
    else if (!rd) fw::launch_resolve(cfg, fr, (const float4 *)ws->accum.p, first_sample + p->samples, p->gamma, d_rgb8, d_gamma, d_linear);
    if (user_accum) HIPCHK(hipMemcpyAsync(user_accum, ws->accum.p, (size_t)n_pix * 16, p->outputs_on_device ? hipMemcpyDeviceToDevice : hipMemcpyDeviceToHost, stream));
    HIPCHK(hipEventRecord(ws->events[1], stream));
    HIPCHK(hipGetLastError());

    if (dump_one) {
        if (FILE *fp = fopen(dump_file, "wb")) {
            uint32_t hdr[8] = {0x46574450u, fr.pinhole0, fr.hit4, sc->d.prim_bits, 0, 0, 0, cfg.n_defer};
            std::memcpy(&hdr[4], fr.cam_pos, 12);
            fwrite(hdr, 4, 8, fp); fwrite(dump_rec.data(), 4, dump_rec.size(), fp); fclose(fp);
        }
    }
    const bool trace = O.trace;
    const auto tq0 = std::chrono::steady_clock::now();
    auto since = [](std::chrono::steady_clock::time_point t) { return std::chrono::duration<double, std::milli>(std::chrono::steady_clock::now() - t).count(); };
    const size_t n_counts = (size_t)n_batches * fw::COUNT_STRIDE;
    const size_t off_c = 0, off_8 = (n_counts * 4 + 255) & ~(size_t)255;
    const size_t off_g = off_8 + ((!p->outputs_on_device && rgb8 ? (size_t)n_pix * 3 : 0) + 255 & ~(size_t)255);
    const size_t off_l = off_g + ((!p->outputs_on_device && gamma_rgb ? (size_t)n_pix * 12 : 0) + 255 & ~(size_t)255);
    const size_t off_e = off_l + ((!p->outputs_on_device && linear_rgb ? (size_t)n_pix * 12 : 0) + 255 & ~(size_t)255);
    const size_t host_need = off_e + 256;
    if (ws->host_out_bytes < host_need) {
        if (ws->host_out) (void)hipHostFree(ws->host_out);
        ws->host_out = nullptr; ws->host_out_bytes = 0;
        if (hipHostMalloc(&ws->host_out, host_need + host_need / 4, hipHostMallocDefault) != hipSuccess) return fail(FW_ERR_OOM, "pinned output staging allocation failed");
        ws->host_out_bytes = host_need + host_need / 4;
    }
    uint8_t *ho = (uint8_t *)ws->host_out;
    const uint32_t *h_counts = (const uint32_t *)(ho + off_c);
    HIPCHK(hipMemcpyAsync(ho + off_c, ws->totals.p, n_counts * 4, hipMemcpyDeviceToHost, stream));
    const double t_counts = since(tq0);
    if (!p->outputs_on_device) {
        if (rgb8) HIPCHK(hipMemcpyAsync(ho + off_8, d_rgb8, (size_t)n_pix * 3, hipMemcpyDeviceToHost, stream));
        if (gamma_rgb) HIPCHK(hipMemcpyAsync(ho + off_g, d_gamma, (size_t)n_pix * 12, hipMemcpyDeviceToHost, stream));
        if (linear_rgb) HIPCHK(hipMemcpyAsync(ho + off_l, d_linear, (size_t)n_pix * 12, hipMemcpyDeviceToHost, stream));
    }
    if (ri) HIPCHK(hipMemcpyAsync(ho + off_e, ws->ray_err.p, 4, hipMemcpyDeviceToHost, stream));
    const double t_outs = since(tq0);
    if (!ws->ev_d2h) HIPCHK(hipEventCreate(&ws->ev_d2h));
    HIPCHK(hipEventRecord(ws->ev_d2h, stream));
    HIPCHK(hipStreamSynchronize(stream));
    if (!p->outputs_on_device) {
        if (rgb8) std::memcpy(rgb8, ho + off_8, (size_t)n_pix * 3);
        if (gamma_rgb) std::memcpy(gamma_rgb, ho + off_g, (size_t)n_pix * 12);
        if (linear_rgb) std::memcpy(linear_rgb, ho + off_l, (size_t)n_pix * 12);
    }
#if FW_AB
    if (const uint32_t ew = fw::take_error_word())
        return fail(FW_ERR_HIP, std::string("device error word: ") + ((ew & 1u) ? "LDS traversal stack overflow (a push beyond the levels the launch reserved) " : "") +
                                    ((ew & 2u) ? "a walk kernel's wave made no progress for 2^24 rounds (left its loop) " : ""));
#endif
    if (ri && *(const uint32_t *)(ho + off_e)) return fail(FW_ERR_BAD_ARG, "a ray has a non-finite component or an all-zero direction");
    if (trace) fprintf(stderr, "[firework] render: enqueue %.2f ms | counters copy queued +%.2f | output copies queued +%.2f | sync + host memcpy returned +%.2f\n",
                       std::chrono::duration<double, std::milli>(tq0 - wall0).count(), t_counts, t_outs, since(tq0));
    const auto wall1 = std::chrono::steady_clock::now();

    if (stats) {
        std::memset(stats, 0, sizeof *stats);
        stats->samples = (uint64_t)n_pix * p->samples;
        uint64_t deposits = 0;
        for (uint32_t b = 0; b < n_batches; b++) {
            for (int s = 0; s < fw::MAX_SEGMENTS; s++) { uint64_t c = h_counts[(size_t)b * fw::COUNT_STRIDE + s]; stats->rays_per_depth[s] += c; stats->rays += c; }
            stats->parked_rays += h_counts[(size_t)b * fw::COUNT_STRIDE + fw::MAX_SEGMENTS];
            deposits += h_counts[(size_t)b * fw::COUNT_STRIDE + 12];
        }
        stats->deposits = count_deposits ? deposits : stats->samples;
        {
            const uint64_t *R = stats->rays_per_depth;
            const uint64_t S = stats->samples, ray0 = fr.pinhole0 ? fw::B_RAY_PINHOLE0 : fw::B_RAY, b_hit = fr.hit4 ? fw::B_HIT4 : fw::B_HIT;
            uint64_t rd_ray = R[0] * ray0, later = 0, survivors = 0;
            for (int s = 1; s < fw::MAX_SEGMENTS; s++) { rd_ray += R[s] * fw::B_RAY; later += R[s]; survivors += R[s]; }
            stats->bytes_raygen = S * ray0 + (fr.pixel_ids ? S * 4 : 0) + (ri ? S * 24 : 0);
            const uint64_t medium = sc->d.has_medium ? later * 4 : 0;
            const uint64_t b_state = fr.chain_bits ? fw::B_STATE_CHAIN : fw::B_STATE;
            const uint64_t shade_in = rd_ray + later * b_state, shade_out = survivors * (fw::B_RAY + b_state + (fr.atten ? fw::B_ATTEN : 0u)) + stats->deposits * fw::B_DEPOSIT;
            if (fused) { stats->bytes_extend = 0; stats->bytes_shade = shade_in + shade_out; }
            else {
                stats->bytes_extend = rd_ray + medium + stats->rays * b_hit + stats->parked_rays * 2 * fw::B_PARK;
                stats->bytes_shade = shade_in + stats->rays * b_hit + shade_out;
            }
            stats->bytes_accumulate = (fr.skip_zero_deposits ? stats->deposits * fw::B_DEPOSIT + S / 8 : S * fw::B_DEPOSIT) + (uint64_t)n_batches * n_pix * 2 * fw::B_ACCUM * (rd ? 2u : 1u);
        }
        stats->ms_wall = std::chrono::duration<double, std::milli>(wall1 - wall0).count();
        float ms_copy = 0.f;
        HIPCHK(hipEventElapsedTime(&ms_copy, ws->events[1], ws->ev_d2h));
        stats->ms_d2h = ms_copy;
        stats->algorithmic_bytes = 160 * stats->rays + 24 * stats->samples;
        float ms = 0.f;
        HIPCHK(hipEventElapsedTime(&ms, ws->events[0], ws->events[1]));
        stats->ms_render = ms;
        if (timing) {
            double acc[4] = {0, 0, 0, 0};
            for (int l = 0; l < n_lanes; l++)
                for (size_t i = 0; i < ev_class[l].size(); i++) {
                    float t = 0.f;
                    HIPCHK(hipEventElapsedTime(&t, ws->lanes[l].events[i], ws->lanes[l].events[i + 1]));
                    acc[ev_class[l][i]] += t;
                }
            stats->ms_raygen = acc[0]; stats->ms_extend = acc[1]; stats->ms_shade = acc[2]; stats->ms_accumulate = acc[3];
        }
        stats->n_extend_launches = fused ? 0 : n_batches * fw::MAX_SEGMENTS; stats->n_shade_launches = n_batches * fw::MAX_SEGMENTS;
        stats->n_batches = n_batches; stats->tlas_nodes = sc->tlas_nodes; stats->blas_nodes = sc->blas_nodes;
        stats->reserved = ((sc->tlas_depth & 0x7fffu) << 16) | (sc->blas_depth & 0xffffu) | (graph_replayed ? 0x80000000u : 0u);
    }
    return FW_OK;
}

constexpr uint32_t ADAPTIVE_MAX_ROUNDS = 32;
int adaptive_impl(fw_scene *sc, const fw_render_params *p, float tol, uint32_t min_samples, float *accum, float *moments, uint8_t *rgb8,
                  float *gamma_rgb, float *linear_rgb, uint32_t *round_pixels, fw_stats *stats) {
    if (!sc || !p) return fail(FW_ERR_BAD_ARG, "null argument");
    if (p->pixel_ids) return fail(FW_ERR_BAD_ARG, "fw_render_adaptive renders whole frames: pixel_ids must be NULL");
    if (min_samples < 2) return fail(FW_ERR_BAD_ARG, "min_samples must be >= 2 (the rule needs a variance)");
    if (p->samples < min_samples) return fail(FW_ERR_BAD_ARG, "samples (the cap) must be >= min_samples");
    if (p->samples > (1u << 24)) return fail(FW_ERR_BAD_ARG, "samples must be <= 2^24 (the count is exact as a float)");
    if (!std::isfinite(tol) || !(tol > 0.f)) return fail(FW_ERR_BAD_ARG, "tolerance must be finite and > 0");
    if (p->width == 0 || p->height == 0) return fail(FW_ERR_BAD_ARG, "width and height must be > 0");
    if (!(p->gamma > 0.f)) return fail(FW_ERR_BAD_ARG, "gamma must be > 0");
    if (p->rng_mode != FW_RNG_CTR) return fail(FW_ERR_UNSUPPORTED, "the HIP path implements FW_RNG_CTR only (FW_RNG_LCG is a sequential stream)");
    const uint64_t full = (uint64_t)p->width * p->height;
    if (full > 0xffffffffull) return fail(FW_ERR_UNSUPPORTED, "image too large");
    const uint32_t n = (uint32_t)full;
    const auto wall0 = std::chrono::steady_clock::now();
    HIPCHK(hipSetDevice(sc->device));
    hipStream_t stream = (hipStream_t)p->stream;
    Workspace *ws = workspace_for(sc->device);
    if (!ws) return fail(FW_ERR_OOM, "no workspace for this device");
    std::lock_guard<std::mutex> ws_guard(ws->mu);
    { const int irc = init_device_locked(ws, sc->device); if (irc) return irc; }
    const Options O = options();
    int rc = FW_OK;
    auto need = [&](DevBuf &b, size_t bytes) { if (!rc) rc = b.alloc(bytes); };
    need(ws->ad_accum, (size_t)n * 16); need(ws->ad_moments, (size_t)n * 16);
    need(ws->ad_ids[0], (size_t)n * 4); need(ws->ad_ids[1], (size_t)n * 4);
    need(ws->ad_mask, ((size_t)n + 63) / 64 * 8); need(ws->ad_counts, ((size_t)fw::ADAPTIVE_MAX_BLOCKS + 1) * 4);
    uint8_t *d_rgb8 = rgb8; float *d_gamma = gamma_rgb, *d_linear = linear_rgb;
    if (!p->outputs_on_device) {
        if (rgb8) { need(ws->out_rgb8, (size_t)n * 3); d_rgb8 = (uint8_t *)ws->out_rgb8.p; }
        if (gamma_rgb) { need(ws->out_gamma, (size_t)n * 12); d_gamma = (float *)ws->out_gamma.p; }
        if (linear_rgb) { need(ws->out_linear, (size_t)n * 12); d_linear = (float *)ws->out_linear.p; }
    }
    if (rc) return rc;
    if (!ws->ad_count_host) HIPCHK(hipHostMalloc((void **)&ws->ad_count_host, 4, hipHostMallocDefault));
    for (hipEvent_t &e : ws->ad_ev) if (!e) HIPCHK(hipEventCreate(&e));
    float4 *d_accum = (float4 *)ws->ad_accum.p, *d_moments = (float4 *)ws->ad_moments.p;
    uint32_t *d_count = (uint32_t *)ws->ad_counts.p + fw::ADAPTIVE_MAX_BLOCKS;

    if (ws->ev_upload) HIPCHK(hipStreamWaitEvent(stream, ws->ev_upload, 0));
    HIPCHK(hipEventRecord(ws->ad_ev[0], stream));
    HIPCHK(hipMemsetAsync(d_accum, 0, (size_t)n * 16, stream));
    HIPCHK(hipMemsetAsync(d_moments, 0, (size_t)n * 16, stream));
    const uint32_t *cur = nullptr;
    if (n >= 1024 && !O.no_tile_order) { fw::launch_tile_order(stream, p->width, p->height, (uint32_t *)ws->ad_ids[0].p); cur = (const uint32_t *)ws->ad_ids[0].p; }

    fw_stats total{};
    uint32_t rounds[ADAPTIVE_MAX_ROUNDS] = {};
    uint32_t n_rounds = 0, active = n, done = 0;
    double ms_classes[4] = {0, 0, 0, 0};
    while (active > 0) {
        if (n_rounds >= ADAPTIVE_MAX_ROUNDS) return fail(FW_ERR_HIP, "adaptive render: more rounds than the schedule allows");
        const uint32_t target = n_rounds == 0 ? min_samples : std::min<uint32_t>(2u * done, p->samples);
        fw_render_params rp = *p;
        rp.samples = target - done; rp.pixel_ids = nullptr; rp.n_pixels = 0;
        const AdaptiveRound rd{cur, active, d_accum, d_moments};
        fw_stats rs{};
        if (int rrc = render_impl(sc, &rp, nullptr, nullptr, nullptr, &rs, done, nullptr, &rd)) return rrc;
        rounds[n_rounds++] = active;
        total.samples += rs.samples; total.rays += rs.rays; total.deposits += rs.deposits; total.parked_rays += rs.parked_rays;
        for (int d = 0; d < FW_MAX_SEGMENTS; d++) total.rays_per_depth[d] += rs.rays_per_depth[d];
        total.algorithmic_bytes += rs.algorithmic_bytes;
        total.bytes_raygen += rs.bytes_raygen; total.bytes_extend += rs.bytes_extend; total.bytes_shade += rs.bytes_shade; total.bytes_accumulate += rs.bytes_accumulate;
        total.n_batches += rs.n_batches; total.n_extend_launches += rs.n_extend_launches; total.n_shade_launches += rs.n_shade_launches;
        total.tlas_nodes = rs.tlas_nodes; total.blas_nodes = rs.blas_nodes; total.reserved = rs.reserved;
        ms_classes[0] += rs.ms_raygen; ms_classes[1] += rs.ms_extend; ms_classes[2] += rs.ms_shade; ms_classes[3] += rs.ms_accumulate;
        done = target;
        uint32_t *next = (uint32_t *)ws->ad_ids[cur == (const uint32_t *)ws->ad_ids[0].p ? 1 : 0].p;
        fw::launch_adaptive_select(stream, cur, active, d_accum, d_moments, done, done < p->samples, tol, (unsigned long long *)ws->ad_mask.p,
                                   (uint32_t *)ws->ad_counts.p, next, d_count);
        HIPCHK(hipMemcpyAsync(ws->ad_count_host, d_count, 4, hipMemcpyDeviceToHost, stream));
        HIPCHK(hipStreamSynchronize(stream));
        if (*ws->ad_count_host > active) return fail(FW_ERR_HIP, "adaptive render: survivor count out of range");
        active = *ws->ad_count_host;
        cur = next;
    }
    fw::launch_resolve_adaptive(stream, sc->n_cus, n, d_accum, d_moments, p->gamma, d_rgb8, d_gamma, d_linear);
    HIPCHK(hipEventRecord(ws->ad_ev[1], stream));
    const hipMemcpyKind kind = p->outputs_on_device ? hipMemcpyDeviceToDevice : hipMemcpyDeviceToHost;
    if (accum) HIPCHK(hipMemcpyAsync(accum, d_accum, (size_t)n * 16, kind, stream));
    if (moments) HIPCHK(hipMemcpyAsync(moments, d_moments, (size_t)n * 16, kind, stream));
    if (!p->outputs_on_device) {
        if (rgb8) HIPCHK(hipMemcpyAsync(rgb8, d_rgb8, (size_t)n * 3, kind, stream));
        if (gamma_rgb) HIPCHK(hipMemcpyAsync(gamma_rgb, d_gamma, (size_t)n * 12, kind, stream));
        if (linear_rgb) HIPCHK(hipMemcpyAsync(linear_rgb, d_linear, (size_t)n * 12, kind, stream));
    }
    if (round_pixels && p->outputs_on_device) HIPCHK(hipMemcpyAsync(round_pixels, rounds, sizeof rounds, hipMemcpyHostToDevice, stream));
    if (!ws->ev_d2h) HIPCHK(hipEventCreate(&ws->ev_d2h));
    HIPCHK(hipEventRecord(ws->ev_d2h, stream));
    HIPCHK(hipStreamSynchronize(stream));
    HIPCHK(hipGetLastError());
    if (round_pixels && !p->outputs_on_device) std::memcpy(round_pixels, rounds, sizeof rounds);
    if (stats) {
        *stats = total;
        float ms = 0.f;
        HIPCHK(hipEventElapsedTime(&ms, ws->ad_ev[0], ws->ad_ev[1]));
        stats->ms_render = ms;
        HIPCHK(hipEventElapsedTime(&ms, ws->ad_ev[1], ws->ev_d2h));
        stats->ms_d2h = p->outputs_on_device ? 0.0 : ms;
        if (p->flags & FW_FLAG_TIME_KERNELS) { stats->ms_raygen = ms_classes[0]; stats->ms_extend = ms_classes[1]; stats->ms_shade = ms_classes[2]; stats->ms_accumulate = ms_classes[3]; }
        stats->ms_wall = std::chrono::duration<double, std::milli>(std::chrono::steady_clock::now() - wall0).count();
    }
    return FW_OK;
}

constexpr uint64_t VIEW_GROUP_MAX_PIXELS = 1ull << 24;
int views_impl(fw_scene *sc, const fw_render_params *p, const fw_camera_settings *cameras, uint32_t n_views, uint8_t *rgb8, float *gamma_rgb,
               float *linear_rgb, fw_stats *stats) {
    if (!sc || !p || !cameras) return fail(FW_ERR_BAD_ARG, "null argument");
    if (n_views == 0) return fail(FW_ERR_BAD_ARG, "n_views must be > 0");
    if (p->width == 0 || p->height == 0 || p->samples == 0) return fail(FW_ERR_BAD_ARG, "width, height and samples must be > 0");
    if (!(p->gamma > 0.f)) return fail(FW_ERR_BAD_ARG, "gamma must be > 0");
    const uint64_t full = (uint64_t)p->width * p->height;
    if (p->pixel_ids && p->n_pixels == 0) return fail(FW_ERR_BAD_ARG, "no pixels to render");
    if (p->pixel_ids) for (uint32_t i = 0; i < p->n_pixels; i++) if (p->pixel_ids[i] >= full) return fail(FW_ERR_BAD_ARG, "pixel id out of range");
    for (uint32_t v = 0; v < n_views; v++) {
        const fw_camera_settings &c = cameras[v];
        const float f[] = {c.cam_pos.x, c.cam_pos.y, c.cam_pos.z, c.look_at.x, c.look_at.y, c.look_at.z, c.vfov, c.aperture, c.focus_dist};
        for (float x : f) if (!std::isfinite(x)) return fail(FW_ERR_BAD_ARG, "camera " + std::to_string(v) + " has a non-finite field");
    }
    if (p->rng_mode != FW_RNG_CTR) return fail(FW_ERR_UNSUPPORTED, "the HIP path implements FW_RNG_CTR only (FW_RNG_LCG is a sequential stream)");
    if (full > 0xffffffffull) return fail(FW_ERR_UNSUPPORTED, "image too large");
    const uint32_t N = p->pixel_ids ? p->n_pixels : (uint32_t)full;
    if ((uint64_t)n_views * N > 0xffffffffull) return fail(FW_ERR_UNSUPPORTED, "n_views x pixels must be below 2^32");

    const auto wall0 = std::chrono::steady_clock::now();
    HIPCHK(hipSetDevice(sc->device));
    Workspace *ws = workspace_for(sc->device);
    if (!ws) return fail(FW_ERR_OOM, "no workspace for this device");
    uint32_t budget = 0;
    {
        std::lock_guard<std::mutex> ws_guard(ws->mu);
        { const int irc = init_device_locked(ws, sc->device); if (irc) return irc; }
        if (int erc = ensure_env_dist(sc, p, ws)) return erc;
        budget = batch_budget(sc, p, options(), ws->arena.bytes).budget;
    }
    const uint32_t per_group = (uint32_t)std::max<uint64_t>(1, std::min<uint64_t>({(uint64_t)n_views, budget / N, VIEW_GROUP_MAX_PIXELS / N}));
    std::vector<fw::DCamera> cams(n_views);
    for (uint32_t v = 0; v < n_views; v++) cams[v] = make_camera(cameras[v], p->width, p->height);

    fw_stats total{};
    for (uint32_t v0 = 0; v0 < n_views; v0 += per_group) {
        const ViewGroup vg{cams.data() + v0, std::min(per_group, n_views - v0)};
        const size_t off = (size_t)v0 * N * 3;
        fw_stats gs{};
        if (int rc = render_impl(sc, p, rgb8 ? rgb8 + off : nullptr, gamma_rgb ? gamma_rgb + off : nullptr, linear_rgb ? linear_rgb + off : nullptr,
// ... 892 lines not shown
```

Before: 41770 Mrays/s.

## Add persistent megakernel path that traces whole paths with work-stealing refill

Adds a persistent one-wave-per-workgroup kernel that generates camera rays, intersects the room and deferred boxes, and shades in a loop. Dead lanes are refilled from atomic chunk counters spread across eight queues. This replaces per-segment raygen/extend/shade launches and the ray, state and hit buffers in HBM for the simple non-BVH scene case, and it factors the room scan and box tests into shared helpers. It costs lane divergence across bounce depths, register pressure from one fused kernel, and atomics on the work counters.

```diff
diff --git a/firework_amd/csrc/fw_device.h b/firework_amd/csrc/fw_device.h
--- a/firework_amd/csrc/fw_device.h
+++ b/firework_amd/csrc/fw_device.h
@@ -198,6 +198,10 @@
 void launch_extend_exact(const LaunchCfg &, const DScene &, const DFrame &, const DPaths &in, float2 *hits, int segment, bool use_bvh);
 void launch_shade(const LaunchCfg &, const DScene &, const DFrame &, DPaths in, DPaths out, const float2 *hits,
                   float4 *sample_rad, int segment);
+constexpr size_t PERSIST_CTR_WORDS = 128;
+bool persistent_tables_fit(const LaunchCfg &, const DScene &);
+void launch_path_persistent(const LaunchCfg &, const DScene &, const DCamera &, const DFrame &, float4 *sample_rad, uint32_t *ctr, uint32_t *totals,
+                            uint32_t n_paths);
 void launch_shade_ls(const LaunchCfg &, const DScene &, const DFrame &, DPaths in, DPaths out, const float2 *hits,
                      float4 *sample_rad, int segment, const DShadow &);
 void launch_shadow_resolve(const LaunchCfg &, const DScene &, const DShadow &, const float2 *hits, int segment);
diff --git a/firework_amd/csrc/fw_kernels.hip b/firework_amd/csrc/fw_kernels.hip
--- a/firework_amd/csrc/fw_kernels.hip
+++ b/firework_amd/csrc/fw_kernels.hip
@@ -1365,6 +1365,42 @@
     if (PARK && lane == 0) park_count[w] = park_n;
 }
 
+template <bool SIMPLE>
+__device__ __forceinline__ void room_scan(const DScene &sc, const Ray &r, uint32_t n_first, int segment, float &best_t, uint32_t &best_obj, uint32_t &best_prim) {
+    const float TMIN = 0.001f;
+    const RngKey nokey{0, 0, 0};
+    const float4 *op = sc.obj;
+    const Rcp rcx = make_rcp(r.d.x), rcy = make_rcp(r.d.y), rcz = make_rcp(r.d.z);
+    for (uint32_t k = 0; k < n_first; k++, op += OBJ_Q) {
+        const Obj o = load_obj(op, 0);
+        float t; uint32_t prim = 0; bool h;
+        const uint32_t kind = obj_kind(o);
+        if (kind >= 1u && kind <= 3u && !(obj_flags(o) & OF_ROTATED) && o.q4.y == 0.f) {
+            const Ray ro{r.o - mk(o.q0.w, o.q1.w, o.q2.w), r.d};
+            if (kind == 1u) h = hit_rect_rcp<0>(o.q3.x, o.q3.y, o.q3.z, o.q3.w, o.q4.x, ro, rcz, TMIN, best_t, t);
+            else if (kind == 2u) h = hit_rect_rcp<1>(o.q3.x, o.q3.y, o.q3.z, o.q3.w, o.q4.x, ro, rcy, TMIN, best_t, t);
+            else h = hit_rect_rcp<2>(o.q3.x, o.q3.y, o.q3.z, o.q3.w, o.q4.x, ro, rcx, TMIN, best_t, t);
+        } else h = hit_object<false, 0, false, SIMPLE>(sc, o, k, r, TMIN, best_t, nullptr, nokey, segment, t, prim);
+        if (h) { best_t = t; best_obj = k; best_prim = prim; }
+    }
+}
+__device__ __forceinline__ bool box_may_hit(const DScene &sc, uint32_t k, const Ray &r, V3 ainv, float eps, float best_t) {
+    const float4 lo = sc.obj_cull[2 * (size_t)k], hi = sc.obj_cull[2 * (size_t)k + 1];
+    const float m = eps + 1e-4f * (fmaxf(fmaxf(fabsf(lo.x), fabsf(lo.y)), fabsf(lo.z)) + fmaxf(fmaxf(fabsf(hi.x), fabsf(hi.y)), fabsf(hi.z))) + 1e-6f;
+    float t0 = (lo.x - m - r.o.x) * ainv.x, t1 = (hi.x + m - r.o.x) * ainv.x;
+    float tn = fminf(t0, t1), tf = fmaxf(t0, t1);
+    t0 = (lo.y - m - r.o.y) * ainv.y; t1 = (hi.y + m - r.o.y) * ainv.y;
+    tn = fmaxf(tn, fminf(t0, t1)); tf = fminf(tf, fmaxf(t0, t1));
+    t0 = (lo.z - m - r.o.z) * ainv.z; t1 = (hi.z + m - r.o.z) * ainv.z;
+    tn = fmaxf(tn, fminf(t0, t1)); tf = fminf(tf, fmaxf(t0, t1));
+    return !(tf < tn * (1.f - 1e-4f) - 1e-4f) && !(tf < 0.f) && !(tn * (1.f - 1e-4f) - 1e-4f > best_t);
+}
+__device__ __forceinline__ void box_exact(const DScene &sc, uint32_t k, const Ray &r, float &t, uint32_t &code) {
+    const float TMIN = 0.001f;
+    const Obj o = load_obj(sc.obj, k);
+    float tt; uint32_t prim;
+    if (hit_rect3d(o.q3, o.q4, to_object_space(o, r), TMIN, t, tt, prim)) { t = tt; code = (k << sc.prim_bits) | prim; }
+}
 constexpr uint32_t DEFER_FIELDS = 9;
 extern __shared__ uint32_t lds_defer[];
 template <bool SIMPLE>
@@ -1373,11 +1409,10 @@
     const uint32_t w = wave_index(), lane = threadIdx.x & 63u;
     if (w >= q.n_waves) return;
     const uint32_t n = q.wcount[(size_t)segment * q.n_waves + w], base = w * q.cap;
-    const float TMIN = 0.001f, TMAX = 2e9f;
+    const float TMAX = 2e9f;
     const uint32_t n_first = sc.n_objects - n_def;
     uint32_t *const L0 = lds_defer, *const L1 = lds_defer + DEFER_FIELDS * 64u;
     uint32_t cnt0 = 0, cnt1 = 0;
-    const RngKey nokey{0, 0, 0};
     auto write_final = [&](uint32_t slot, float t, uint32_t code) {
         if (f.hit4) reinterpret_cast<uint32_t *>(hits)[slot] = code; else qst(&hits[slot], make_float2(t, __uint_as_float(code)));
     };
@@ -1391,12 +1426,7 @@
         r.o = mk(__uint_as_float(L[192u + e]), __uint_as_float(L[256u + e]), __uint_as_float(L[320u + e]));
         r.d = mk(__uint_as_float(L[384u + e]), __uint_as_float(L[448u + e]), __uint_as_float(L[512u + e]));
     };
-    auto test = [&](uint32_t d, const Ray &r, float &t, uint32_t &code) {
-        const uint32_t k = n_first + d;
-        const Obj o = load_obj(sc.obj, k);
-        float tt; uint32_t prim;
-        if (hit_rect3d(o.q3, o.q4, to_object_space(o, r), TMIN, t, tt, prim)) { t = tt; code = (k << sc.prim_bits) | prim; }
-    };
+    auto test = [&](uint32_t d, const Ray &r, float &t, uint32_t &code) { box_exact(sc, n_first + d, r, t, code); };
     auto append = [&](uint32_t *L, uint32_t &cnt, bool want, uint32_t sb, float t, uint32_t code, const Ray &r) {
         const unsigned long long m = __ballot(want);
         if (!m) return;
@@ -1438,33 +1468,11 @@
         bool may0 = false, may1 = false;
         const Ray r = make_ray(ra, rb, f, segment);
         if (active) {
-            const float4 *op = sc.obj;
-            const Rcp rcx = make_rcp(r.d.x), rcy = make_rcp(r.d.y), rcz = make_rcp(r.d.z);
-            for (uint32_t k = 0; k < n_first; k++, op += OBJ_Q) {
-                const Obj o = load_obj(op, 0);
-                float t; uint32_t prim = 0; bool h;
-                const uint32_t kind = obj_kind(o);
-                if (kind >= 1u && kind <= 3u && !(obj_flags(o) & OF_ROTATED) && o.q4.y == 0.f) {
-                    const Ray ro{r.o - mk(o.q0.w, o.q1.w, o.q2.w), r.d};
-                    if (kind == 1u) h = hit_rect_rcp<0>(o.q3.x, o.q3.y, o.q3.z, o.q3.w, o.q4.x, ro, rcz, TMIN, best_t, t);
-                    else if (kind == 2u) h = hit_rect_rcp<1>(o.q3.x, o.q3.y, o.q3.z, o.q3.w, o.q4.x, ro, rcy, TMIN, best_t, t);
-                    else h = hit_rect_rcp<2>(o.q3.x, o.q3.y, o.q3.z, o.q3.w, o.q4.x, ro, rcx, TMIN, best_t, t);
-                } else h = hit_object<false, 0, false, SIMPLE>(sc, o, k, r, TMIN, best_t, nullptr, nokey, segment, t, prim);
-                if (h) { best_t = t; best_obj = k; best_prim = prim; }
-            }
+            room_scan<SIMPLE>(sc, r, n_first, segment, best_t, best_obj, best_prim);
             const V3 ainv = mk(__builtin_amdgcn_rcpf(r.d.x), __builtin_amdgcn_rcpf(r.d.y), __builtin_amdgcn_rcpf(r.d.z));
             const float eps = 1e-4f * (fabsf(r.o.x) + fabsf(r.o.y) + fabsf(r.o.z));
             for (uint32_t d = 0; d < n_def; d++) {
-                const uint32_t k = n_first + d;
-                const float4 lo = sc.obj_cull[2 * (size_t)k], hi = sc.obj_cull[2 * (size_t)k + 1];
-                const float m = eps + 1e-4f * (fmaxf(fmaxf(fabsf(lo.x), fabsf(lo.y)), fabsf(lo.z)) + fmaxf(fmaxf(fabsf(hi.x), fabsf(hi.y)), fabsf(hi.z))) + 1e-6f;
-                float t0 = (lo.x - m - r.o.x) * ainv.x, t1 = (hi.x + m - r.o.x) * ainv.x;
-                float tn = fminf(t0, t1), tf = fmaxf(t0, t1);
-                t0 = (lo.y - m - r.o.y) * ainv.y; t1 = (hi.y + m - r.o.y) * ainv.y;
-                tn = fmaxf(tn, fminf(t0, t1)); tf = fminf(tf, fmaxf(t0, t1));
-                t0 = (lo.z - m - r.o.z) * ainv.z; t1 = (hi.z + m - r.o.z) * ainv.z;
-                tn = fmaxf(tn, fminf(t0, t1)); tf = fminf(tf, fmaxf(t0, t1));
-                const bool maybe = !(tf < tn * (1.f - 1e-4f) - 1e-4f) && !(tf < 0.f) && !(tn * (1.f - 1e-4f) - 1e-4f > best_t);
+                const bool maybe = box_may_hit(sc, n_first + d, r, ainv, eps, best_t);
                 if (d == 0) may0 = maybe; else may1 = maybe;
             }
         }
@@ -2912,6 +2920,116 @@
     if (lane == 0) q.wcount[(size_t)(segment + 1) * q.n_waves + w] = out_n;
     PH_FLUSH(1);
 }
+#ifndef FW_PERSIST_WAVES
+#define FW_PERSIST_WAVES 4
+#endif
+constexpr uint32_t PERSIST_UNIT = 8;
+constexpr uint32_t PERSIST_CTRS = 8;
+constexpr uint32_t PERSIST_CTR_STRIDE = 16;
+__device__ __forceinline__ uint32_t home_of_linear(const DFrame &f, uint32_t linear, float inv_nw) {
+    const uint32_t cw = linear >> 6;
+    uint32_t c = (uint32_t)((float)cw * inv_nw);
+    int32_t w = (int32_t)(cw - c * f.q_n_waves);
+    if (w < 0) { c--; w += (int32_t)f.q_n_waves; }
+    else if ((uint32_t)w >= f.q_n_waves) { c++; w -= (int32_t)f.q_n_waves; }
+    return ((uint32_t)w << (f.q_shift + 6u)) | (c << 6) | (linear & 63u);
+}
+__attribute__((amdgpu_waves_per_eu(FW_PERSIST_WAVES, 8)))
+__global__ __launch_bounds__(WB) void k_path_persistent(DScene sc, DCamera cam, DFrame f, float4 *__restrict__ sample_rad, uint32_t *__restrict__ ctr,
+                                                        uint32_t *__restrict__ totals, uint32_t n_paths, uint32_t n_def, uint32_t n_mat, uint32_t n_tex) {
+    static_assert(WB == 64, "one wave per workgroup: the LDS counters below are the wave's own");
+    const uint32_t lane = threadIdx.x & 63u;
+    __shared__ uint32_t ends[MAX_SEGMENTS];
+    const uint32_t no = sc.n_objects * OBJ_Q, nm = 2 * n_mat, nt = 2 * n_tex;
+    for (uint32_t k = lane; k < no; k += WB) lds_tables[k] = sc.obj[k];
+    for (uint32_t k = lane; k < nm; k += WB) lds_tables[no + k] = sc.mat[k];
+    for (uint32_t k = lane; k < nt; k += WB) lds_tables[no + nm + k] = sc.tex[k];
+    if (lane < (uint32_t)MAX_SEGMENTS) ends[lane] = 0u;
+    __syncthreads();
+    const float4 *objp = lds_tables, *matp = lds_tables + no, *texp = lds_tables + no + nm;
+    PH_DECL;
+    const float TMAX = 2e9f;
+    const uint32_t n_first = sc.n_objects - n_def, n_chunks = (n_paths + 63u) / 64u;
+    const float inv_nw = 1.f / (float)f.q_n_waves;
+    const uint32_t x0 = blockIdx.x & (PERSIST_CTRS - 1u);
+    uint32_t xi = 0, nxt = 0, end = 0;
+    bool live = false;
+    Ray r{mk(0.f, 0.f, 0.f), mk(0.f, 0.f, 1.f)};
+    RngKey key{0u, 0u, f.seed32};
+    uint32_t chain = 0, home = 0;
+    int seg = 0;
+    for (;;) {
+        {
+            PH_T0;
+#pragma nounroll
+            for (int k = 0; k < 3; k++) {
+                const unsigned long long dead = __ballot(!live);
+                if (dead == 0ull) break;
+                if (nxt >= end) {
+                    bool got = false;
+                    while (xi < PERSIST_CTRS) {
+                        const uint32_t x = (x0 + xi) & (PERSIST_CTRS - 1u);
+                        const uint32_t lo = (uint32_t)((uint64_t)n_chunks * x / PERSIST_CTRS), hi = (uint32_t)((uint64_t)n_chunks * (x + 1u) / PERSIST_CTRS);
+                        uint32_t v = 0;
+                        if (lane == 0) v = atomicAdd(&ctr[x * PERSIST_CTR_STRIDE], 1u);
+                        v = (uint32_t)__builtin_amdgcn_readfirstlane((int)v);
+                        const uint64_t c = (uint64_t)lo + (uint64_t)v * PERSIST_UNIT;
+                        if (c < hi) {
+                            nxt = (uint32_t)c * 64u;
+                            end = min(min((uint32_t)c + PERSIST_UNIT, hi) * 64u, n_paths);
+                            got = true;
+                            break;
+                        }
+                        xi++;
+                    }
+                    if (!got) break;
+                }
+                const uint32_t rank = __builtin_amdgcn_mbcnt_hi((uint32_t)(dead >> 32), __builtin_amdgcn_mbcnt_lo((uint32_t)dead, 0u));
+                const uint32_t avail = end - nxt;
+                if (!live && rank < avail) {
+                    const uint32_t id = nxt + rank;
+                    key = key_of_linear(f, id);
+                    home = home_of_linear(f, id, inv_nw);
+                    r = camera_ray(cam, f, key);
+                    chain = 0u; seg = 0; live = true;
+                }
+                nxt += min((uint32_t)__popcll(dead), avail);
+            }
+            PH_ADD(15);
+        }
+        if (__ballot(live) == 0ull) break;
+        float best_t = TMAX; uint32_t best_obj = MISS, best_prim = 0;
+        if (live) { PH_T0; room_scan<true>(sc, r, n_first, seg, best_t, best_obj, best_prim); PH_ADD(13); }
+        uint32_t code = best_obj == MISS ? MISS : ((best_obj << sc.prim_bits) | best_prim);
+        {
+            PH_T0;
+            const V3 ainv = mk(__builtin_amdgcn_rcpf(r.d.x), __builtin_amdgcn_rcpf(r.d.y), __builtin_amdgcn_rcpf(r.d.z));
+            const float eps = 1e-4f * (fabsf(r.o.x) + fabsf(r.o.y) + fabsf(r.o.z));
+            for (uint32_t d = 0; d < n_def; d++) {
+                const uint32_t k = n_first + d;
+                const bool maybe = live && box_may_hit(sc, k, r, ainv, eps, best_t);
+                if (__ballot(maybe) == 0ull) continue;
+                if (maybe) box_exact(sc, k, r, best_t, code);
+            }
+            PH_ADD(14);
+        }
+        if (live) {
+            PH_T0;
+            Ray nr{mk(0.f, 0.f, 0.f), mk(0.f, 0.f, 0.f)}; V3 nbeta = mk(0.f, 0.f, 0.f); uint32_t nchain = 0;
+            const bool alive = shade_path<true, true>(sc, f, objp, matp, texp, r, nbeta, chain, home, best_t, code, seg, sample_rad, nr, nbeta, nchain PH_PASS, &key);
+            if (alive) { r = nr; chain = nchain; seg++; }
+            else { atomicAdd(&ends[seg], 1u); live = false; }
+            PH_ADD(0);
+        }
+    }
+    __syncthreads();
+    if (lane < (uint32_t)MAX_SEGMENTS) {
+        uint32_t acc = 0;
+        for (uint32_t s = lane; s < (uint32_t)MAX_SEGMENTS; s++) acc += ends[s];
+        if (acc) atomicAdd(&totals[lane], acc);
+    }
+    PH_FLUSH(1);
+}
 template <int LDS_TAB, int MODE>
 __attribute__((amdgpu_waves_per_eu(FW_SHADE_WAVES, 8)))
 __global__ __launch_bounds__(WB) void k_shade_ls(DScene sc, DFrame f, DPaths in, DPaths out, const float2 *__restrict__ hits,
@@ -3740,6 +3858,20 @@
 #undef FW_SHADE_C
 #undef FW_SHADE
 }
+static size_t persistent_tables(const LaunchCfg &c, const DScene &sc) { return ((size_t)sc.n_objects * OBJ_Q + 2 * (size_t)c.n_mat + 2 * (size_t)c.n_tex) * sizeof(float4); }
+bool persistent_tables_fit(const LaunchCfg &c, const DScene &sc) { return persistent_tables(c, sc) <= LDS_TABLE_LIMIT; }
+void launch_path_persistent(const LaunchCfg &c, const DScene &sc, const DCamera &cam, const DFrame &f, float4 *sample_rad, uint32_t *ctr, uint32_t *totals,
+                            uint32_t n_paths) {
+    static_assert(PERSIST_CTRS * PERSIST_CTR_STRIDE <= PERSIST_CTR_WORDS, "the host zeroes PERSIST_CTR_WORDS counter words per batch");
+    const size_t lds = persistent_tables(c, sc);
+    int per_cu = 0;
+    if (hipOccupancyMaxActiveBlocksPerMultiprocessor(&per_cu, reinterpret_cast<const void *>(k_path_persistent), WB, lds) != hipSuccess || per_cu < 1) {
+        (void)hipGetLastError();
+        per_cu = 1;
+    }
+    const uint32_t grid = std::max(1u, std::min<uint32_t>((uint32_t)c.n_cus * (uint32_t)per_cu, (n_paths + 63u) / 64u));
+    hipLaunchKernelGGL(k_path_persistent, dim3(grid), dim3(WB), lds, c.stream, sc, cam, f, sample_rad, ctr, totals, n_paths, c.n_defer, c.n_mat, c.n_tex);
+}
 void launch_shade_ls(const LaunchCfg &c, const DScene &sc, const DFrame &f, DPaths in, DPaths out, const float2 *hits,
                      float4 *sample_rad, int segment, const DShadow &sh) {
     const size_t tab = ((size_t)sc.n_objects * OBJ_Q + 2 * (size_t)c.n_mat + 2 * (size_t)c.n_tex) * sizeof(float4);
diff --git a/firework_amd/csrc/fw_runtime.cpp b/firework_amd/csrc/fw_runtime.cpp
--- a/firework_amd/csrc/fw_runtime.cpp
+++ b/firework_amd/csrc/fw_runtime.cpp
@@ -33,6 +33,7 @@
     int streams = 0;
     int graph = -1;
     int phase_lock = -1;
+    int persistent = -1;
     int soft_shear_log2 = 5, exact_shear_log2 = 10; double exact_far_x = 256.0;
     double wide_node_cost = 0.0005;
     int wide = -1;
@@ -46,7 +47,7 @@
 #endif
 };
 const char *const OPTION_NAMES[] = {"BVH", "NO_EXACT", "EXACT_ALL", "EXACT_FORM", "NO_DEFER", "NO_HIT4", "NO_HOIST", "NO_LDS_TABLES", "NO_LDS_TREES", "NO_LDS_TRIS",
-                                    "NO_SHORT_RAYS", "NO_TILE_ORDER", "NO_ZERO_SKIP", "DEP_PIXEL_MAJOR", "DEP_SLOT_MAJOR", "NO_CHAIN", "EXACT_PRODUCT", "PHASE_LOCK", "GRAPH", "SOFT_SHEAR_LOG2", "EXACT_SHEAR_LOG2", "EXACT_FAR_X", "WIDE_NODE_COST", "TRACE", "STREAMS", "WIDE", "BUILD", "WAVES",
+                                    "NO_SHORT_RAYS", "NO_TILE_ORDER", "NO_ZERO_SKIP", "DEP_PIXEL_MAJOR", "DEP_SLOT_MAJOR", "NO_CHAIN", "EXACT_PRODUCT", "PHASE_LOCK", "PERSISTENT", "GRAPH", "SOFT_SHEAR_LOG2", "EXACT_SHEAR_LOG2", "EXACT_FAR_X", "WIDE_NODE_COST", "TRACE", "STREAMS", "WIDE", "BUILD", "WAVES",
                                     "PATHS_PER_BATCH", "DUMP_PATH",
 #if FW_AB
                                     "FUSED", "TLAS_REFILL", "SHADE_LIST", "NO_SHADE_DEFER", "STAGGER", "DEBUG_WIDE_LEVELS",
@@ -75,6 +76,7 @@
     else if (n == "EXACT_PRODUCT") o.exact_product = v && atoi(v) != 0;
     else if (n == "PHASE_LOCK") o.phase_lock = v ? (atoi(v) != 0 ? 1 : 0) : -1;
     else if (n == "GRAPH") o.graph = v ? (atoi(v) != 0 ? 1 : 0) : -1;
+    else if (n == "PERSISTENT") o.persistent = v ? (atoi(v) != 0 ? 1 : 0) : -1;
     else if (n == "SOFT_SHEAR_LOG2") o.soft_shear_log2 = v ? (int)num() : 5;
     else if (n == "EXACT_SHEAR_LOG2") o.exact_shear_log2 = v ? (int)num() : 10;
     else if (n == "EXACT_FAR_X") o.exact_far_x = v ? atof(v) : 256.0;
@@ -1884,6 +1886,17 @@
                                                                                    : ((sc->ex.mode & 4u) && sc->d.has_mesh ? 4u : 0u)));
     const bool park_meshes = p->use_bvh && sc->d.has_mesh != 0 && tlas_refill;
     const bool stage_rays = ri && ri->per_sample && !ri->on_device;
+    bool persist = false;
+    {
+        fw::LaunchCfg pc{};
+        set_walk_cfg(pc, sc, O, q, p->use_bvh != 0, tlas_refill);
+        bool mode1 = !sc->has_expensive;
+#if FW_AB
+        mode1 = mode1 && !O.no_shade_defer;
+#endif
+        persist = O.persistent != 0 && !p->use_bvh && pc.n_defer > 0 && pc.simple_set && mode1 && sc->chain_bits != 0 && !O.no_chain && !fused_req &&
+                  !ls && !exact_mode && !ri && !vg && O.dump_path.empty() && fw::persistent_tables_fit(pc, sc->d);
+    }
     int rc = FW_OK;
     auto need = [&](DevBuf &b, size_t n) { if (!rc) rc = b.alloc(n); };
     auto layout = [&](uint8_t *arena_base) -> size_t {
@@ -1891,13 +1904,16 @@
         auto put = [&](void *&dst, size_t n) { dst = arena_base ? arena_base + off : nullptr; off += (n + 255) & ~(size_t)255; };
         for (int l = 0; l < n_lanes; l++) {
             Workspace::Lane &L = ws->lanes[l];
-            for (int k = 0; k < 2; k++) { put(L.ray_a[k], (size_t)cap * 16); put(L.ray_b[k], (size_t)cap * 8); put(L.state[k], (size_t)cap * 16); }
-            put(L.hits, (size_t)cap * 8);
+            if (persist) { for (int k = 0; k < 2; k++) L.ray_a[k] = L.ray_b[k] = L.state[k] = nullptr; L.hits = nullptr; }
+            else {
+                for (int k = 0; k < 2; k++) { put(L.ray_a[k], (size_t)cap * 16); put(L.ray_b[k], (size_t)cap * 8); put(L.state[k], (size_t)cap * 16); }
+                put(L.hits, (size_t)cap * 8);
+            }
             put(L.sample_rad, (size_t)cap * 16);
             put(L.dep_bits, ((size_t)cap + 31) / 32 * 4);
             if (exact_product && !fused_req) put(L.atten, (size_t)cap * (fw::MAX_SEGMENTS - 1) * fw::B_ATTEN); else L.atten = nullptr;
             if (exact_mode) put(L.exact_slots, 2 * (size_t)max_paths * 4 + 64);
-            put(L.wcount, (size_t)(fw::MAX_SEGMENTS + 1) * q.n_waves * 4);
+            put(L.wcount, std::max<size_t>((size_t)(fw::MAX_SEGMENTS + 1) * q.n_waves, fw::PERSIST_CTR_WORDS) * 4);
             if (stage_rays) put(L.rays, (size_t)max_paths * 24); else L.rays = nullptr;
             if (ls) {
                 put(L.s_ray_a, (size_t)cap * 16); put(L.s_ray_b, (size_t)cap * 8); put(L.s_state, (size_t)cap * 16); put(L.s_obj, (size_t)cap * 4);
@@ -2044,7 +2060,7 @@
     struct BatchCtx { fw::DFrame fr; fw::LaunchCfg cfg; fw::DPaths buf[2]; float2 *hits; float4 *srad; fw::DPark park; uint32_t *totals; uint32_t n_paths; int cur; int lane; hipStream_t ls;
                       fw::DShadow sh; fw::DEnvDist ed; };
     constexpr uint64_t PHASE_LOCK_MIN_CHUNKS = 3u << 19;
-    const bool phase_lock = n_lanes == 2 && !fused && (O.phase_lock == 1 || (O.phase_lock < 0 && !p->use_bvh && cfg.n_defer > 0 && chunks >= PHASE_LOCK_MIN_CHUNKS));
+    const bool phase_lock = n_lanes == 2 && !fused && !persist && (O.phase_lock == 1 || (O.phase_lock < 0 && !p->use_bvh && cfg.n_defer > 0 && chunks >= PHASE_LOCK_MIN_CHUNKS));
     std::vector<hipEvent_t> &pe = ws->phase_events;
     while (phase_lock && pe.size() < 2 * (size_t)fw::MAX_SEGMENTS) { hipEvent_t e; HIPCHK(hipEventCreateWithFlags(&e, hipEventDisableTiming)); pe.push_back(e); }
     float4 *const accum = rd ? rd->accum : (float4 *)ws->accum.p;
@@ -2059,6 +2075,7 @@
         c.fr.dep_bits = (uint32_t *)L.dep_bits;
         c.fr.atten = (c.fr.chain_bits == 0 && exact_product && !fused_req) ? (float4 *)L.atten : nullptr; c.fr.atten_stride = cap;
         if (c.fr.skip_zero_deposits) HIPCHK(hipMemsetAsync(c.fr.dep_bits, 0, ((size_t)cap + 31) / 32 * 4, c.ls));
+        if (persist) HIPCHK(hipMemsetAsync(c.cfg.q.wcount, 0, fw::PERSIST_CTR_WORDS * 4, c.ls));
         if (exact_mode) {
             c.fr.ex.slots[0] = (uint32_t *)L.exact_slots; c.fr.ex.slots[1] = c.fr.ex.slots[0] + max_paths;
             c.fr.ex.count = c.fr.ex.slots[1] + max_paths; c.fr.ex.cap = max_paths;
@@ -2091,6 +2108,10 @@
         if (timing) { (void)hipEventRecord(ws->lanes[c.lane].events[1 + ev_next[c.lane]], c.ls); ev_next[c.lane]++; ev_class[c.lane].push_back(cls); }
     };
     auto segment = [&](uint32_t b, BatchCtx &c, int seg, int which, int group_size) -> int {
+        if (persist) {
+            if (seg == 0) timed(c, 2, [&] { fw::launch_path_persistent(c.cfg, sc->d, cam, c.fr, c.srad, c.cfg.q.wcount, c.totals, c.n_paths); });
+            return FW_OK;
+        }
 #if FW_AB
         if (fused) { timed(c, 2, [&] { fw::launch_bounce(c.cfg, sc->d, c.fr, c.buf[c.cur], c.buf[c.cur ^ 1], c.srad, seg, use_bvh); }); c.cur ^= 1; return FW_OK; }
 #endif
@@ -2133,7 +2154,7 @@
         return FW_OK;
     };
     auto end_batch = [&](uint32_t b, BatchCtx &c) -> int {
-        timed(c, 3, [&] { fw::launch_queue_totals(c.cfg, c.totals, c.park.ptotal); });
+        if (!persist) timed(c, 3, [&] { fw::launch_queue_totals(c.cfg, c.totals, c.park.ptotal); });
         if (count_deposits) fw::launch_count_deposits(c.cfg, c.fr.dep_bits, c.totals + 12);
         if (n_lanes > 1 && b > 0) HIPCHK(hipStreamWaitEvent(c.ls, ws->events[3 + b - 1], 0));
         if (rd) timed(c, 3, [&] { fw::launch_accumulate_adaptive(c.cfg, c.fr, c.srad, accum, rd->moments); });
@@ -2165,7 +2186,7 @@
                 timed(ctx[g], 0, [&] { fw::launch_raygen_rays(ctx[g].cfg, src, ri->per_sample, (uint32_t *)ws->ray_err.p, ctx[g].fr, ctx[g].buf[0], ctx[g].n_paths); });
             }
             else if (vg) timed(ctx[g], 0, [&] { fw::launch_raygen_views(ctx[g].cfg, (const fw::DCamera *)ws->view_cams.p, n_view, ctx[g].fr, ctx[g].buf[0], ctx[g].srad, ctx[g].n_paths); });
-            else timed(ctx[g], 0, [&] { fw::launch_raygen(ctx[g].cfg, cam, ctx[g].fr, ctx[g].buf[0], ctx[g].srad, ctx[g].n_paths); });
+            else if (!persist) timed(ctx[g], 0, [&] { fw::launch_raygen(ctx[g].cfg, cam, ctx[g].fr, ctx[g].buf[0], ctx[g].srad, ctx[g].n_paths); });
         }
         for (int seg = 0; seg < fw::MAX_SEGMENTS; seg++)
             for (int g = 0; g < group; g++)
@@ -2188,7 +2209,7 @@
             fw::LaunchCfg kc = cfg; kc.stream = nullptr;
             mix(&cam, sizeof cam); mix(&fr, sizeof fr); mix(&kc, sizeof kc); mix(&sc->d, sizeof sc->d); mix(&q, sizeof q);
             const uint64_t scalars[] = {n_batches, (uint64_t)n_lanes, spp_b, first_sample, p->samples, n_pix, max_paths, cap, exact_mode, (uint64_t)park_meshes, (uint64_t)phase_lock,
-                                        (uint64_t)count_deposits, (uint64_t)exact_product, (uint64_t)use_bvh, (uint64_t)fused, (uint64_t)stagger, (uint64_t)(uintptr_t)accum, (uint64_t)(uintptr_t)ws->totals.p,
+                                        (uint64_t)count_deposits, (uint64_t)exact_product, (uint64_t)use_bvh, (uint64_t)fused, (uint64_t)stagger, (uint64_t)persist, (uint64_t)(uintptr_t)accum, (uint64_t)(uintptr_t)ws->totals.p,
                                         (uint64_t)(uintptr_t)ws->arena.p, (uint64_t)ws->arena.bytes};
             mix(scalars, sizeof scalars);
             for (int l = 0; l < n_lanes; l++) { const Workspace::Lane &L = ws->lanes[l]; const void *ptrs[] = {L.ray_a[0], L.ray_a[1], L.ray_b[0], L.ray_b[1], L.state[0], L.state[1], L.hits, L.sample_rad, L.wcount, L.park_a, L.park_b, L.park_m, L.pcount, L.dep_bits, L.exact_slots, L.atten}; mix(ptrs, sizeof ptrs); }
@@ -2304,7 +2325,10 @@
             const uint64_t medium = sc->d.has_medium ? later * 4 : 0;
             const uint64_t b_state = fr.chain_bits ? fw::B_STATE_CHAIN : fw::B_STATE;
             const uint64_t shade_in = rd_ray + later * b_state, shade_out = survivors * (fw::B_RAY + b_state + (fr.atten ? fw::B_ATTEN : 0u)) + stats->deposits * fw::B_DEPOSIT;
-            if (fused) { stats->bytes_extend = 0; stats->bytes_shade = shade_in + shade_out; }
+            if (persist) {
+                stats->bytes_raygen = fr.pixel_ids ? S * 4 : 0; stats->bytes_extend = 0; stats->bytes_shade = stats->deposits * fw::B_DEPOSIT;
+            }
+            else if (fused) { stats->bytes_extend = 0; stats->bytes_shade = shade_in + shade_out; }
             else {
                 stats->bytes_extend = rd_ray + medium + stats->rays * b_hit + stats->parked_rays * 2 * fw::B_PARK;
                 stats->bytes_shade = shade_in + stats->rays * b_hit + shade_out;
@@ -2329,7 +2353,7 @@
                 }
             stats->ms_raygen = acc[0]; stats->ms_extend = acc[1]; stats->ms_shade = acc[2]; stats->ms_accumulate = acc[3];
         }
-        stats->n_extend_launches = fused ? 0 : n_batches * fw::MAX_SEGMENTS; stats->n_shade_launches = n_batches * fw::MAX_SEGMENTS;
+        stats->n_extend_launches = (fused || persist) ? 0 : n_batches * fw::MAX_SEGMENTS; stats->n_shade_launches = persist ? n_batches : n_batches * fw::MAX_SEGMENTS;
         stats->n_batches = n_batches; stats->tlas_nodes = sc->tlas_nodes; stats->blas_nodes = sc->blas_nodes;
         stats->reserved = ((sc->tlas_depth & 0x7fffu) << 16) | (sc->blas_depth & 0xffffu) | (graph_replayed ? 0x80000000u : 0u);
     }
```

After: 36780 Mrays/s (median of 2 runs). -11.9%, worse.
